# c-zhou/oatk

Hardware: AMD Instinct MI355X
Metric: HiFi Gbases/s through syncasm (syncmer+syncerr) at k=1001 s=31 (higher is better)
Workload: dtype u64

## Files before the change

include/oatk_hip_ec.h:

```cpp
#ifndef OATK_HIP_EC_H
#define OATK_HIP_EC_H

#include "oatk_hip.h"

#ifdef __cplusplus
extern "C" {
#endif

typedef struct {
    uint64_t n_vtx, n_arc;
    const uint64_t *idx_p;
    const uint64_t *idx_n;
    const uint64_t *arc_v;
    const uint64_t *arc_w;
    const uint64_t *arc_ls;
    const uint32_t *arc_cov;
    const uint8_t *arc_del;
} oatk_ec_graph_t;

int oatk_hip_ec(oatk_hip_ctx *ctx, const oatk_ec_graph_t *g, double max_edist, uint32_t err_mer_c, uint32_t max_err_c,
                uint32_t err_arc_c, double max_arc_f);

int oatk_hip_ec_stats(oatk_hip_ctx *ctx, uint64_t *stats12);

int oatk_hip_debug_ec_tiers(oatk_hip_ctx *ctx, int cap_t0, int cap_t1);

int oatk_hip_debug_wf_ed(oatk_hip_ctx *ctx, uint64_t n_jobs, const uint8_t *t_codes, const uint64_t *t_off, const uint8_t *q_codes, const uint64_t *q_off,
                         const int32_t *bw, const int32_t *step_ql, const uint64_t *step_off, int32_t *out3);
int oatk_hip_debug_wf_ed_wg(oatk_hip_ctx *ctx, int R, uint64_t n_jobs, const uint8_t *t_codes, const uint64_t *t_off, const uint8_t *q_codes, const uint64_t *q_off,
                            const int32_t *bw, const int32_t *step_ql, const uint64_t *step_off, int32_t *out3);
int oatk_hip_debug_tables(oatk_hip_ctx *ctx, uint64_t n_jobs, const uint8_t *t_codes, const uint64_t *t_off, const uint8_t *s_codes, const uint64_t *s_off, int32_t *out, const uint64_t *out_off);

enum {
    OATK_BUF_EC_N_SCM = 100, OATK_BUF_EC_SCM_OFF, OATK_BUF_EC_KMER, OATK_BUF_EC_MPOS, OATK_BUF_EC_SMER,
    OATK_BUF_EC_SCM_COV, OATK_BUF_EC_SCM_DEL, OATK_BUF_EC_SCM_OCC_OFF, OATK_BUF_EC_SCM_OCC, OATK_BUF_EC_ERR_DEL,
    OATK_BUF_EC_SCM_FWD,
    OATK_BUF_EC_VTX_SRC,
    OATK_BUF_EC_BLOCK_WORK, OATK_BUF_EC_BLOCK_OUT,
    OATK_BUF_EC_CSEQ_LEN,
    OATK_BUF_EC_CSEQ_OFF,
    OATK_BUF_EC_CSEQ,
    OATK_BUF_EC_BLOCK_QEND
};

int oatk_hip_ec_keep_seq(oatk_hip_ctx *ctx, int on);
int oatk_hip_ec_corrected_reads(oatk_hip_ctx *ctx, uint64_t *n_bases);

int oatk_hip_ec_mark(oatk_hip_ctx *ctx, uint32_t err_mer_c, uint32_t max_err_c, uint32_t err_arc_c, double max_arc_f);
int oatk_hip_ec_correct(oatk_hip_ctx *ctx, double max_edist);

int oatk_hip_ec_graph(oatk_hip_ctx *ctx);
int oatk_hip_ec_graph_light(oatk_hip_ctx *ctx, uint32_t err_mer_c);

int oatk_hip_ec_set_global(oatk_hip_ctx *ctx, uint64_t n_global, const uint32_t *d_l2g, const uint32_t *d_cov, const uint64_t *d_s);
int oatk_hip_ec_pairs(oatk_hip_ctx *ctx, const void **d_keys, const void **d_dist, uint64_t *n_pairs);
int oatk_hip_ec_graph_from_pairs(oatk_hip_ctx *ctx, const uint64_t *d_keys, const uint32_t *d_dist, uint64_t n_pairs);
int oatk_hip_ec_graph_from_segments(oatk_hip_ctx *ctx, const uint64_t *d_keys, const uint64_t *d_val, uint64_t n_seg);
int oatk_hip_ec_export_kmers(oatk_hip_ctx *ctx, const uint32_t *d_ids, uint64_t n, uint8_t *d_out, uint32_t stride, uint8_t *d_rev);
int oatk_hip_ec_import_kmers(oatk_hip_ctx *ctx, const uint32_t *d_ids, const uint8_t *d_rev, const uint8_t *d_kmers, uint64_t n, uint32_t stride);
int oatk_hip_ec_reserve_import(oatk_hip_ctx *ctx, uint64_t bytes);

enum {
    OATK_BUF_EG_IDX_P = 120, OATK_BUF_EG_IDX_N, OATK_BUF_EG_ARC_V, OATK_BUF_EG_ARC_W, OATK_BUF_EG_ARC_LS, OATK_BUF_EG_ARC_COV,
    OATK_BUF_EG_ARC_COMP,
    OATK_BUF_EG_OTHER
};

#ifdef __cplusplus
}
#endif
#endif
```

oatk_amd/_lib.py:

```python
import ctypes as C
import os

HERE = os.path.dirname(os.path.abspath(__file__))
LIB_PATH = os.environ.get("OATK_HIP_LIB") or os.path.join(HERE, "lib", "liboatk_hip.so")
HOST_LIB_PATH = os.path.join(HERE, "lib", "liboatk_host.so")

OK, E_NODEV, E_ARG, E_STATE, E_SMER, E_SPLIT, E_NOMEM = range(7)
READ_ALIGN = 64
BUF = {name: i for i, name in enumerate([
    "HOCO_L", "N_SCM", "N_NN", "N_LRL", "HO_RL", "HOCO_S", "NN_KEY", "LRL_KEY", "LRL_VAL",
    "SCM_OFF", "POS_MPOS", "POS_SMER", "POS_HASH", "POS_KID",
    "SCM_H", "SCM_S", "SCM_COV", "SCM_OCC_OFF", "SCM_OCC"])}
BUF.update({name: 100 + i for i, name in enumerate([
    "EC_N_SCM", "EC_SCM_OFF", "EC_KMER", "EC_MPOS", "EC_SMER", "EC_SCM_COV", "EC_SCM_DEL", "EC_SCM_OCC_OFF", "EC_SCM_OCC", "EC_ERR_DEL",
    "EC_SCM_FWD", "EC_VTX_SRC", "EC_BLOCK_WORK", "EC_BLOCK_OUT", "EC_CSEQ_LEN", "EC_CSEQ_OFF", "EC_CSEQ", "EC_BLOCK_QEND"])})
BUF.update({name: 160 + i for i, name in enumerate(["INGEST_SEQ", "INGEST_OFF", "INGEST_LEN", "INGEST_HDR"])})
FMT_AUTO, FMT_FASTA, FMT_FASTQ = 0, 1, 2
BUF.update({name: 140 + i for i, name in enumerate(["CONS_SEL", "CONS_SLOT", "CONS_RL", "CONS_MSEQ", "CONS_FIRST", "CONS_TOT"])})
BUF.update({name: 200 + i for i, name in enumerate(["RA_ALN_SID", "RA_ALN_OFF", "RA_ALN_S", "RA_FRG_UID", "RA_FRG_UBEG", "RA_FRG_UEND", "RA_FRG_SBEG", "RA_FRG_SEND", "RA_SKIPPED"])})
BUF.update({name: 150 + i for i, name in enumerate(["OVL_KEY", "OVL_OFF", "OVL_DIST", "OVL_CNT", "OVL_TAIL"])})
BUF.update({name: 120 + i for i, name in enumerate([
    "EG_IDX_P", "EG_IDX_N", "EG_ARC_V", "EG_ARC_W", "EG_ARC_LS", "EG_ARC_COV", "EG_ARC_COMP", "EG_OTHER"])})
BUF.update({name: 180 + i for i, name in enumerate([
    "AG_SCM_DEL", "AG_VTX_SCM", "AG_VTX_COV", "AG_IDX_P", "AG_IDX_N", "AG_ARC_V", "AG_ARC_W", "AG_ARC_COV", "AG_ARC_COMP", "AG_ARC_LINK"])})
BUF.update({name: 220 + i for i, name in enumerate(["MG_H", "MG_S", "MG_COV", "MG_L2G", "MG_EC_COV", "MG_EC_DEL", "MG_LCOV"])})
BUF.update({name: 230 + i for i, name in enumerate(["MG_G_H", "MG_G_S", "MG_G_COV", "MG_G_DEL", "MG_G_OCC_OFF", "MG_G_OCC", "MG_POS_GKID"])})
TIMERS = ["hpc", "syncmer", "syncmer_n", "scan_post", "count_place", "count_sort", "count_group", "kmer_hash", "ec_graph", "ec_mark", "ec_solve", "ec_refresh"]

EXPORTS = [
    "oatk_hip_abi_version", "oatk_hip_device_count", "oatk_hip_create", "oatk_hip_destroy", "oatk_hip_last_error",
    "oatk_hip_stream", "oatk_hip_sync", "oatk_hip_max_k", "oatk_hip_scan", "oatk_hip_scan_host", "oatk_hip_count",
    "oatk_comm_unique_id", "oatk_comm_create", "oatk_comm_group_create", "oatk_comm_group_rank", "oatk_comm_group_destroy", "oatk_comm_destroy",
    "oatk_comm_rank", "oatk_comm_size", "oatk_comm_backend", "oatk_comm_traffic", "oatk_hip_merge_counts", "oatk_hip_multi_range", "oatk_hip_ec_sharded",
    "oatk_hip_gather_table", "oatk_hip_asm_graph_sharded", "oatk_hip_consensus_sharded", "oatk_hip_overlap_hist_sharded", "oatk_hip_stat_sharded",
    "oatk_hip_scan_begin", "oatk_hip_scan_reserve", "oatk_hip_scan_append", "oatk_hip_device", "oatk_hip_d2d", "oatk_hip_mem_pool",
    "oatk_hip_info", "oatk_hip_buffer", "oatk_hip_d2h", "oatk_hip_d2h_async", "oatk_hip_h2d_async", "oatk_hip_staging", "oatk_hip_ingest_text_buffer", "oatk_hip_set_timing", "oatk_hip_get_timing",
    "oatk_hip_debug_hash_mask", "oatk_hip_debug_force_general", "oatk_hip_debug_list_cap",
    "oatk_hip_ec_graph", "oatk_hip_ec_graph_light", "oatk_hip_ec", "oatk_hip_ec_stats", "oatk_hip_debug_ec_tiers", "oatk_hip_debug_wf_ed", "oatk_hip_debug_wf_ed_wg", "oatk_hip_ec_mark", "oatk_hip_ec_correct",
    "oatk_hip_ec_set_global", "oatk_hip_ec_pairs", "oatk_hip_ec_graph_from_pairs", "oatk_hip_ec_graph_from_segments", "oatk_hip_ec_export_kmers", "oatk_hip_ec_import_kmers",
    "oatk_hip_ec_reserve_import", "oatk_hip_consensus", "oatk_hip_consensus_ids", "oatk_hip_ingest", "oatk_hip_ingest_host", "oatk_hip_scan_ingested", "oatk_hip_stat", "oatk_hip_stat_keys", "oatk_hip_stat_from_keys",
    "oatk_hip_asm_graph", "oatk_hip_asm_pairs", "oatk_hip_asm_graph_from_pairs", "oatk_hip_overlap_hist", "oatk_hip_overlap_pairs", "oatk_hip_overlap_hist_from_pairs", "oatk_hip_read_alignment", "oatk_hip_debug_align_two_pass",
    "oatk_hip_ra_utg_coverage", "oatk_hip_ra_arc_coverage", "oatk_hip_debug_racov_cap", "oatk_hip_ra_utg_coverage_sharded", "oatk_hip_ra_arc_coverage_sharded",
    "oatk_hip_ra_triplet_scores", "oatk_hip_ra_triplet_scores_sharded",
    "oatk_hip_ec_keep_seq", "oatk_hip_ec_corrected_reads",
    "oatk_hip_inflate_bgzf", "oatk_hip_inflate_bgzf_host", "oatk_hip_inflate_last_byte", "oatk_hip_ingest_names",
    "oatk_hip_ingest_bam", "oatk_hip_ingest_bam_host", "oatk_hip_ingest_bam_stats", "oatk_hip_ingest_bam_times",
]

HOST_EXPORTS = ["oatk_multi_scg_ra_utg_coverage", "oatk_multi_scg_ra_arc_coverage", "oatk_scg_multiplex_plan", "oatk_multi_scg_multiplex_plan",
                "oatk_triplet_table_free", "oatk_multi_read_error_correction_fo", "oatk_bgzf_index", "oatk_host_set_device_inflate", "oatk_host_inflate_counts"]


def load_host():
    H = C.CDLL(HOST_LIB_PATH)
    vp = C.c_void_p
    H.oatk_sr_db_new.restype = vp
    H.oatk_sr_db_new.argtypes = [C.c_int, C.c_int]
    H.oatk_multi_create.restype = vp
    H.oatk_multi_create.argtypes = [C.POINTER(C.c_int), C.c_int]
    H.oatk_multi_destroy.argtypes = [vp]
    H.oatk_multi_ctx.restype = vp
    H.oatk_multi_ctx.argtypes = [vp, C.c_int]
    H.oatk_multi_last_error.restype = C.c_char_p
    H.oatk_multi_last_error.argtypes = [vp]
    H.oatk_multi_range.argtypes = [vp, C.c_int, C.POINTER(C.c_uint64), C.POINTER(C.c_uint64)]
    H.oatk_multi_sr_read_files.argtypes = [vp, vp, C.POINTER(C.c_char_p), C.c_int]
    H.oatk_multi_collect_syncmer_from_reads.restype = vp
    H.oatk_multi_collect_syncmer_from_reads.argtypes = [vp, vp, C.POINTER(C.c_int)]
    H.oatk_multi_read_error_correction.argtypes = [vp, vp, vp, C.c_double, C.c_uint32, C.c_uint32, C.c_uint32, C.c_double, vp]
    H.oatk_multi_read_error_correction_fo.argtypes = [vp, vp, vp, C.c_double, C.c_uint32, C.c_uint32, C.c_uint32, C.c_double, vp, vp]
    H.oatk_multi_make_syncmer_asmg.restype = vp
    H.oatk_multi_make_syncmer_asmg.argtypes = [vp, vp, C.c_uint32, C.c_double, C.POINTER(C.c_int)]
    H.oatk_multi_scg_read_alignment.argtypes = [vp, vp, vp, vp, C.c_int, C.POINTER(C.c_uint64)]
    H.oatk_multi_scg_ra_utg_coverage.argtypes = [vp, vp, vp, vp, C.c_int]
    H.oatk_multi_scg_ra_arc_coverage.argtypes = [vp, vp, vp, vp, C.c_int]
    H.oatk_scg_multiplex_plan.argtypes = [vp, vp, vp, C.c_uint, C.c_uint32, C.c_double, C.c_double, vp, C.POINTER(C.c_int), C.POINTER(TripletTable)]
    H.oatk_multi_scg_multiplex_plan.argtypes = [vp, vp, vp, C.c_uint32, C.c_double, C.c_double, vp, C.POINTER(C.c_int), C.POINTER(TripletTable)]
    H.oatk_triplet_table_free.restype = None
    H.oatk_triplet_table_free.argtypes = [C.POINTER(TripletTable)]
    H.oatk_host_debug_window.argtypes = [C.c_uint64]
    H.oatk_bgzf_index.argtypes = [vp, C.c_uint64, C.c_uint64, C.c_uint64, vp, C.POINTER(C.c_uint64), C.POINTER(C.c_uint64), C.POINTER(C.c_uint64)]
    return H


BGZF_MEMBER = [("in_off", "<u8"), ("in_len", "<u4"), ("out_len", "<u4"), ("out_off", "<u8"), ("crc", "<u4"), ("pad", "<u4")]
INF_OK, INF_STREAM, INF_LENGTH, INF_CRC = range(4)


class TripletTable(C.Structure):
    _fields_ = [("n", C.c_uint64), ("m", C.c_uint64), ("l_in", C.POINTER(C.c_uint64)), ("l_out", C.POINTER(C.c_uint64)), ("val", C.POINTER(C.c_double))]

# ... 60 lines not shown
    L.oatk_hip_last_error.argtypes = [vp]
    L.oatk_hip_stream.restype = vp
    L.oatk_hip_stream.argtypes = [vp]
    L.oatk_hip_sync.argtypes = [vp]
    L.oatk_hip_max_k.restype = C.c_int
    L.oatk_hip_scan.argtypes = [vp, vp, vp, vp, C.c_uint64, C.c_uint64, C.c_uint64, C.c_int, C.c_int]
    L.oatk_hip_scan_host.argtypes = [vp, vp, vp, vp, C.c_uint64, C.c_uint64, C.c_uint64, C.c_int, C.c_int]
    L.oatk_hip_count.argtypes = [vp]
    L.oatk_comm_unique_id.argtypes = [vp]
    L.oatk_comm_create.restype = vp
    L.oatk_comm_create.argtypes = [vp, C.c_int, C.c_int, C.c_int]
    L.oatk_comm_group_create.restype = vp
    L.oatk_comm_group_create.argtypes = [C.c_int]
    L.oatk_comm_group_rank.restype = vp
    L.oatk_comm_group_rank.argtypes = [vp, C.c_int]
    L.oatk_comm_group_destroy.argtypes = [vp]
    L.oatk_comm_destroy.argtypes = [vp]
    L.oatk_comm_rank.argtypes = [vp]
    L.oatk_comm_size.argtypes = [vp]
    L.oatk_comm_backend.restype = C.c_char_p
    L.oatk_comm_backend.argtypes = [vp]
    L.oatk_comm_traffic.restype = None
    L.oatk_comm_traffic.argtypes = [vp, C.POINTER(C.c_uint64), C.c_int]
    L.oatk_hip_merge_counts.argtypes = [vp, vp, C.POINTER(C.c_uint64)]
    L.oatk_hip_multi_range.argtypes = [vp, C.POINTER(C.c_uint64), C.POINTER(C.c_uint64), C.POINTER(C.c_uint64)]
    L.oatk_hip_ec_sharded.argtypes = [vp, vp, C.c_double, C.c_uint32, C.c_uint32, C.c_uint32, C.c_double, vp, C.POINTER(C.c_uint64)]
    L.oatk_hip_gather_table.argtypes = [vp, vp, C.c_int]
    L.oatk_hip_asm_graph_sharded.argtypes = [vp, vp, C.c_uint32, C.c_double, C.POINTER(C.c_uint64), C.POINTER(C.c_uint64)]
    L.oatk_hip_consensus_sharded.argtypes = [vp, vp, C.c_uint32]
    L.oatk_hip_overlap_hist_sharded.argtypes = [vp, vp, C.c_uint32, C.POINTER(C.c_uint64), C.POINTER(C.c_uint64)]
    L.oatk_hip_stat_sharded.argtypes = [vp, vp, C.POINTER(StatRaw)]
    L.oatk_hip_scan_begin.argtypes = [vp, C.c_uint64, C.c_int, C.c_int]
    L.oatk_hip_scan_reserve.argtypes = [vp, C.c_uint64, C.c_uint64, C.c_uint64]
    L.oatk_hip_scan_append.argtypes = [vp, vp]
    L.oatk_hip_device.argtypes = [vp]
    L.oatk_hip_mem_pool.argtypes = [vp, C.c_uint64]
    L.oatk_hip_d2d.argtypes = [vp, vp, vp, C.c_uint64]
    L.oatk_hip_info.argtypes = [vp, C.POINTER(Info)]
    L.oatk_hip_buffer.argtypes = [vp, C.c_int, C.POINTER(vp), C.POINTER(C.c_uint64)]
    L.oatk_hip_d2h.argtypes = [vp, vp, vp, C.c_uint64]
    L.oatk_hip_staging.restype = vp
    L.oatk_hip_staging.argtypes = [vp, C.c_uint64]
    L.oatk_hip_set_timing.argtypes = [vp, C.c_int]
    L.oatk_hip_get_timing.argtypes = [vp, C.POINTER(C.c_float), C.c_int]
    L.oatk_hip_debug_hash_mask.argtypes = [vp, C.c_uint64]
    L.oatk_hip_debug_force_general.argtypes = [vp, C.c_int]
    L.oatk_hip_debug_list_cap.argtypes = [vp, C.c_int]
    L.oatk_hip_ec_graph.argtypes = [vp]
    L.oatk_hip_ec_graph_light.argtypes = [vp, C.c_uint32]
    L.oatk_hip_ec.argtypes = [vp, C.POINTER(EcGraph), C.c_double, C.c_uint32, C.c_uint32, C.c_uint32, C.c_double]
    L.oatk_hip_ec_stats.argtypes = [vp, vp]
    L.oatk_hip_debug_ec_tiers.argtypes = [vp, C.c_int, C.c_int]
    L.oatk_hip_debug_wf_ed.argtypes = [vp, C.c_uint64, vp, vp, vp, vp, vp, vp, vp, vp]
    if hasattr(L, "oatk_hip_debug_wf_ed_wg"):
        L.oatk_hip_debug_wf_ed_wg.argtypes = [vp, C.c_int, C.c_uint64, vp, vp, vp, vp, vp, vp, vp, vp]
    if hasattr(L, "oatk_hip_debug_ed_ab"):
        L.oatk_hip_debug_ed_ab.argtypes = [vp, C.c_int, C.c_uint64, vp, vp, vp, vp, vp, vp, C.POINTER(C.c_float)]
    L.oatk_hip_ec_mark.argtypes = [vp, C.c_uint32, C.c_uint32, C.c_uint32, C.c_double]
    L.oatk_hip_ec_correct.argtypes = [vp, C.c_double]
    L.oatk_hip_ec_keep_seq.argtypes = [vp, C.c_int]
    L.oatk_hip_ec_corrected_reads.argtypes = [vp, C.POINTER(C.c_uint64)]
    L.oatk_hip_ec_set_global.argtypes = [vp, C.c_uint64, vp, vp, vp]
    L.oatk_hip_ec_pairs.argtypes = [vp, C.POINTER(vp), C.POINTER(vp), C.POINTER(C.c_uint64)]
    L.oatk_hip_ec_graph_from_pairs.argtypes = [vp, vp, vp, C.c_uint64]
    L.oatk_hip_ec_graph_from_segments.argtypes = [vp, vp, vp, C.c_uint64]
    L.oatk_hip_ec_export_kmers.argtypes = [vp, vp, C.c_uint64, vp, C.c_uint32, vp]
    L.oatk_hip_ec_import_kmers.argtypes = [vp, vp, vp, vp, C.c_uint64, C.c_uint32]
    L.oatk_hip_ec_reserve_import.argtypes = [vp, C.c_uint64]
    L.oatk_hip_consensus.argtypes = [vp, C.c_uint32]
    L.oatk_hip_consensus_ids.argtypes = [vp, vp, C.c_uint64]
    L.oatk_hip_ingest.argtypes = [vp, vp, C.c_uint64, C.c_int, C.c_int, C.POINTER(C.c_uint64), C.POINTER(C.c_uint64)]
    L.oatk_hip_ingest_host.argtypes = [vp, vp, C.c_uint64, C.c_int, C.c_int, C.POINTER(C.c_uint64), C.POINTER(C.c_uint64)]
    L.oatk_hip_scan_ingested.argtypes = [vp, C.c_uint64, C.c_int, C.c_int]
    L.oatk_hip_ingest_text_buffer.argtypes = [vp, C.c_uint64, C.POINTER(vp)]
    L.oatk_hip_inflate_bgzf.argtypes = [vp, vp, C.c_uint64, vp, C.c_uint64, vp, C.c_uint64, C.POINTER(C.c_uint64), vp]
    L.oatk_hip_inflate_bgzf_host.argtypes = [vp, vp, C.c_uint64, vp, C.c_uint64, vp, C.c_uint64, C.POINTER(C.c_uint64), vp]
    L.oatk_hip_inflate_last_byte.argtypes = [vp]
    L.oatk_hip_ingest_names.argtypes = [vp, vp, C.c_uint64, C.POINTER(vp), C.POINTER(vp), C.POINTER(C.c_uint64)]
    L.oatk_hip_ingest_bam.argtypes = [vp, vp, C.c_uint64, C.c_int, C.c_int, C.POINTER(C.c_uint64), C.POINTER(C.c_uint64)]
    L.oatk_hip_ingest_bam_host.argtypes = [vp, vp, C.c_uint64, C.c_int, C.c_int, C.POINTER(C.c_uint64), C.POINTER(C.c_uint64)]
    L.oatk_hip_ingest_bam_stats.argtypes = [vp, C.POINTER(C.c_uint64)]
    L.oatk_hip_ingest_bam_times.argtypes = [vp, C.POINTER(C.c_float)]
    L.oatk_hip_stat.argtypes = [vp, C.POINTER(StatRaw)]
    L.oatk_hip_stat_keys.argtypes = [vp, C.POINTER(vp), C.POINTER(vp), C.POINTER(C.c_uint64), vp]
    L.oatk_hip_stat_from_keys.argtypes = [vp, vp, vp, C.c_uint64, vp, C.POINTER(StatRaw)]
    L.oatk_hip_debug_align_two_pass.argtypes = [vp, C.c_int]
    L.oatk_hip_read_alignment.argtypes = [vp, C.POINTER(RaGraph), vp, C.POINTER(C.c_uint64), C.POINTER(C.c_uint64), vp]
    L.oatk_hip_ra_utg_coverage.argtypes = [vp, C.POINTER(RacovGraph), C.POINTER(RacovReads), C.POINTER(RacovAln), C.c_int, vp, C.POINTER(C.c_uint64)]
    L.oatk_hip_ra_arc_coverage.argtypes = [vp, C.POINTER(RacovGraph), C.POINTER(RacovAln), vp]
    L.oatk_hip_debug_racov_cap.argtypes = [vp, C.c_uint64]
    L.oatk_hip_ra_utg_coverage_sharded.argtypes = [vp, vp, C.POINTER(RacovGraph), C.POINTER(RacovReads), C.POINTER(RacovAln), C.c_int, vp, C.POINTER(C.c_uint64)]
    L.oatk_hip_ra_arc_coverage_sharded.argtypes = [vp, vp, C.POINTER(RacovGraph), C.POINTER(RacovAln), vp]
    u64p = C.POINTER(C.c_uint64)
    L.oatk_hip_ra_triplet_scores.argtypes = [vp, C.POINTER(RacovGraph), C.POINTER(RacovAln), vp, C.c_uint64, u64p, vp, vp, vp, vp]
    L.oatk_hip_ra_triplet_scores_sharded.argtypes = [vp, vp, C.POINTER(RacovGraph), C.POINTER(RacovAln), vp, C.c_uint64, u64p, vp, vp, vp, vp]
    L.oatk_hip_overlap_pairs.argtypes = [vp, C.POINTER(vp), C.POINTER(vp), C.POINTER(C.c_uint64)]
    L.oatk_hip_overlap_hist_from_pairs.argtypes = [vp, vp, vp, C.c_uint64, C.POINTER(C.c_uint64), C.POINTER(C.c_uint64)]
    L.oatk_hip_overlap_hist.argtypes = [vp, C.POINTER(C.c_uint64), C.POINTER(C.c_uint64)]
    L.oatk_hip_asm_graph.argtypes = [vp, C.c_uint32, C.c_double, C.POINTER(C.c_uint64), C.POINTER(C.c_uint64)]
    L.oatk_hip_asm_pairs.argtypes = [vp, C.POINTER(vp), C.POINTER(C.c_uint64)]
    L.oatk_hip_asm_graph_from_pairs.argtypes = [vp, vp, C.c_uint64, C.c_uint64, vp, vp, C.c_uint32, C.c_double, C.POINTER(C.c_uint64), C.POINTER(C.c_uint64)]
    _lib = L
    return L
```

oatk_amd/csrc/api_ec.inc:

```
#include "../../include/oatk_hip_ec.h"
#include "ec.hpp"
#include "ec_wave.hpp"
#include "ec_heavy.hpp"
#include "ec_fused.hpp"
#include "ecgraph.hpp"
#include "ec_seq.hpp"
#include <rocprim/iterator/counting_iterator.hpp>

struct EcState {
    DevBuf idx_p, idx_n, arc_v, arc_w, arc_ls, arc_cov, arc_del, conv;
    DevBuf scm_del, err_del, vtx_hs_off, vtx_mpos;
    DevBuf copy_n, seg, keep_all, n_blocks, n_blocks64, blk_off, work, out, path_pool, cursor, todo, todo2, slabs, big_slabs, os_slabs;
    DevBuf qkey, qidx, qtmp[4];
    uint64_t n_live = 0, q_used = 0, qk_used = 0;
    DevBuf hyb_slabs[16];
    hipStream_t aux[5] = {nullptr, nullptr, nullptr, nullptr, nullptr};
    hipEvent_t aux_ev[5] = {nullptr, nullptr, nullptr, nullptr, nullptr}, fork_ev = nullptr;
    DevBuf new_n, new_n64, new_off, new_k, new_m, new_s, stats;
    DevBuf live32, live64, live_off, larc, lidx_p, lidx_n;
    DevBuf cov, fwd, key_id, key_sorted, val_occ, occ, occ_off, cov64;
    uint64_t n_vtx = 0, new_tot = 0;
    uint64_t stats_h[12] = {0};
    uint64_t n_work = 0;
    uint32_t staged_over = 0;
// ... 51 lines not shown
        if (which == OATK_BUF_EC_VTX_SRC) *d_ptr = e->vtx_hs_off.p, *bytes = e->n_vtx * 8;
        else *d_ptr = e->err_del.p, *bytes = e->n_vtx;
        return OATK_OK;
    }
    if (!e || !e->done) { ctx->err = "unknown buffer id, or error-correction results requested before oatk_hip_ec"; return OATK_E_STATE; }
    if (which == OATK_BUF_EC_BLOCK_WORK) { *d_ptr = e->work.p, *bytes = e->n_work * sizeof(oatk::EcWork); return OATK_OK; }
    if (which == OATK_BUF_EC_BLOCK_OUT) { *d_ptr = e->out.p, *bytes = e->n_work * sizeof(oatk::EcBlockOut); return OATK_OK; }
    if (which == OATK_BUF_EC_BLOCK_QEND) {
        if (!e->seq_kept) { ctx->err = "EC_BLOCK_QEND: the resident correction was made without oatk_hip_ec_keep_seq"; return OATK_E_STATE; }
        *d_ptr = e->qend.p, *bytes = e->n_work * 4;
        return OATK_OK;
    }
    if (which >= OATK_BUF_EC_CSEQ_LEN && which <= OATK_BUF_EC_CSEQ) {
        if (!e->seq_kept || !e->cseq_done) { ctx->err = "corrected sequences requested before oatk_hip_ec_corrected_reads"; return OATK_E_STATE; }
        if (which == OATK_BUF_EC_CSEQ_LEN) *d_ptr = e->clen.p, *bytes = ctx->n_reads * 4;
        else if (which == OATK_BUF_EC_CSEQ_OFF) *d_ptr = e->coff.p, *bytes = (ctx->n_reads + 1) * 8;
        else *d_ptr = e->cseq.p, *bytes = e->cseq_bytes;
        return OATK_OK;
    }
    const uint64_t n = ctx->n_reads, ns = e->n_vtx, tot = e->new_tot;
    switch (which) {
        case OATK_BUF_EC_N_SCM: *d_ptr = e->new_n.p, *bytes = n * 4; break;
        case OATK_BUF_EC_SCM_OFF: *d_ptr = e->new_off.p, *bytes = (n + 1) * 8; break;
        case OATK_BUF_EC_KMER: *d_ptr = e->new_k.p, *bytes = tot * 8; break;
        case OATK_BUF_EC_MPOS: *d_ptr = e->new_m.p, *bytes = tot * 4; break;
        case OATK_BUF_EC_SMER: *d_ptr = e->new_s.p, *bytes = tot * 8; break;
        case OATK_BUF_EC_SCM_COV: *d_ptr = e->cov.p, *bytes = ns * 4; break;
        case OATK_BUF_EC_SCM_DEL: *d_ptr = e->scm_del.p, *bytes = ns; break;
        case OATK_BUF_EC_SCM_OCC_OFF: *d_ptr = e->occ_off.p, *bytes = (ns + 1) * 8; break;
        case OATK_BUF_EC_SCM_OCC: *d_ptr = e->occ.p, *bytes = tot * 8; break;
        case OATK_BUF_EC_ERR_DEL: *d_ptr = e->err_del.p, *bytes = ns; break;
        case OATK_BUF_EC_SCM_FWD: *d_ptr = e->fwd.p, *bytes = ns * 4; break;
        default: ctx->err = "unknown buffer id"; return OATK_E_ARG;
    }
    return OATK_OK;
}

__global__ void ec_narrow_kernel(const uint64_t *in, uint32_t *out, uint64_t n)
{
    uint64_t i = (uint64_t) blockIdx.x * blockDim.x + threadIdx.x;
    if (i < n) out[i] = (uint32_t) in[i];
}
#define EENSURE(buf, bytes, ...) ENSURE_IN(e, "ec.", buf, bytes, ##__VA_ARGS__)

extern "C" int oatk_hip_debug_ec_tiers(oatk_hip_ctx *ctx, int cap_t0, int cap_t1)
{
    if (!ctx) return OATK_E_NODEV;
    if (cap_t0 < 0 || cap_t1 < 0 || (cap_t0 && cap_t1 && cap_t1 < cap_t0)) { ctx->err = "oatk_hip_debug_ec_tiers: 0 <= cap_t0 <= cap_t1"; return OATK_E_ARG; }
    ctx->ec_cap_t0 = cap_t0, ctx->ec_cap_t1 = cap_t1;
    return OATK_OK;
}

static int debug_ed_impl(oatk_hip_ctx *ctx, uint64_t n_jobs, const uint8_t *t_codes, const uint64_t *t_off, const uint8_t *q_codes, const uint64_t *q_off,
                         const int32_t *bw, const int32_t *step_ql, const uint64_t *step_off, int32_t *out3, bool myers, float *kernel_ms, int wg_R = 0)
{
    using namespace oatk;
    if (!ctx) return OATK_E_NODEV;
    if (n_jobs == 0) return OATK_OK;
    if (n_jobs >= 0x7FFFFFFFULL) { ctx->err = "oatk_hip_debug_wf_ed: too many jobs"; return OATK_E_ARG; }
    CK(hipSetDevice(ctx->device));
    std::vector<uint64_t> tw_off(n_jobs + 1, 0), qw_off(n_jobs + 1, 0), k_off(n_jobs + 1, 0);
    std::vector<int32_t> tl(n_jobs);
    for (uint64_t j = 0; j < n_jobs; ++j) {
        const uint64_t t = t_off[j + 1] - t_off[j], q = q_off[j + 1] - q_off[j];
        if (t == 0 || q == 0 || t > 0x3FFFFFFF || q > 0x3FFFFFFF) { ctx->err = "oatk_hip_debug_wf_ed: empty or oversized string (wf_ed asserts tl > 0 && ql > 0)"; return OATK_E_ARG; }
        for (uint64_t s = step_off[j]; s < step_off[j + 1]; ++s)
            if (step_ql[s] < 1 || (uint64_t) step_ql[s] > q || (s > step_off[j] && step_ql[s] < step_ql[s - 1])) { ctx->err = "oatk_hip_debug_wf_ed: query lengths must ascend within the query"; return OATK_E_ARG; }
        tl[j] = (int32_t) t;
        if (wg_R && (bw[j] >= 0? (uint64_t) 2 * (uint64_t) bw[j] + 3 : t + q + 3) > (wg_R == ECF_NW? (uint64_t) ECF_NW * ECF_OWN : (uint64_t) 64 * ECH_NW * (uint64_t) wg_R)) { ctx->err = "oatk_hip_debug_wf_ed_wg: a job's diagonals do not fit the registers of this variant"; return OATK_E_ARG; }
        tw_off[j + 1] = tw_off[j] + ecw_words((int32_t) t), qw_off[j + 1] = qw_off[j] + ecw_words((int32_t) q);
        k_off[j + 1] = k_off[j] + 2 * (t + q + 8);
    }
    auto pack = [](const uint8_t *codes, const uint64_t *off, const std::vector<uint64_t> &woff, uint64_t n) {
        std::vector<uint32_t> w(woff[n], 0u);
        for (uint64_t j = 0; j < n; ++j)
            for (uint64_t p = 0, len = off[j + 1] - off[j]; p < len; ++p)
                w[woff[j] + (p >> 4)] |= (uint32_t) (codes[off[j] + p] & 3u) << ((p & 15u) << 1);
        return w;
    };
    const std::vector<uint32_t> tw = pack(t_codes, t_off, tw_off, n_jobs), qw = pack(q_codes, q_off, qw_off, n_jobs);
    const uint64_t n_steps = step_off[n_jobs];
    DevBuf d_tw, d_qw, d_two, d_qwo, d_tl, d_bw, d_sq, d_so, d_k, d_ko, d_out, d_slab;
    hipEvent_t ev0 = nullptr, ev1 = nullptr;
    if (kernel_ms) { *kernel_ms = 0.f; (void) hipEventCreate(&ev0); (void) hipEventCreate(&ev1); }
    int32_t max_t = 0;
    for (uint64_t j = 0; j < n_jobs; ++j) if (tl[j] > max_t) max_t = tl[j];
    const uint64_t n_waves = (n_jobs + 63) / 64, slab_words = (uint64_t) 6 * 64 * (uint64_t) ((max_t + 63) / 64 + 1);
    std::vector<int32_t> ql_last(n_jobs);
    for (uint64_t j = 0; j < n_jobs; ++j) ql_last[j] = step_off[j + 1] > step_off[j]? step_ql[step_off[j + 1] - 1] : (int32_t) (q_off[j + 1] - q_off[j]);
    int rc = OATK_OK;
    hipError_t he = hipSuccess;
    auto up = [&](DevBuf &b, const void *src, size_t bytes) {
        if (rc) return;
        if (!b.ensure(bytes + 16, ctx->stream)) { rc = OATK_E_NOMEM; return; }
        if (bytes && (he = hipMemcpyAsync(b.p, src, bytes, hipMemcpyHostToDevice, ctx->stream)) != hipSuccess) rc = OATK_E_NODEV;
    };
    up(d_tw, tw.data(), tw.size() * 4); up(d_qw, qw.data(), qw.size() * 4);
    up(d_two, tw_off.data(), (n_jobs + 1) * 8); up(d_qwo, qw_off.data(), (n_jobs + 1) * 8); up(d_ko, k_off.data(), (n_jobs + 1) * 8);
    up(d_tl, tl.data(), n_jobs * 4); up(d_bw, bw, n_jobs * 4); up(d_sq, step_ql, n_steps * 4); up(d_so, step_off, (n_jobs + 1) * 8);
    if (!rc && (!d_k.ensure(k_off[n_jobs] * 4 + 16, ctx->stream) || !d_out.ensure(n_steps * 12 + 16, ctx->stream))) rc = OATK_E_NOMEM;
    if (!rc && myers) {
        if (!d_slab.ensure(n_waves * slab_words * 8 + 64, ctx->stream) || !d_out.ensure(n_jobs * 12 + 16, ctx->stream)) rc = OATK_E_NOMEM;
        up(d_sq, ql_last.data(), n_jobs * 4);
    }
    if (!rc) {
        if (ev0) (void) hipEventRecord(ev0, ctx->stream);
#ifdef OATK_EXPERIMENTS
        if (myers)
            hipLaunchKernelGGL(myers_ed_kernel, dim3((unsigned) n_waves), dim3(64), 0, ctx->stream, n_jobs, d_tw.as<uint32_t>(), d_two.as<uint64_t>(), d_tl.as<int32_t>(),
                               d_qw.as<uint32_t>(), d_qwo.as<uint64_t>(), d_sq.as<int32_t>(), d_bw.as<int32_t>(), d_slab.as<uint64_t>(), slab_words, d_out.as<int32_t>());
        else
#endif
        if (wg_R) {
            uint64_t cap_words = 0;
            for (uint64_t j = 0; j < n_jobs; ++j) { if (tw_off[j + 1] - tw_off[j] > cap_words) cap_words = tw_off[j + 1] - tw_off[j]; if (qw_off[j + 1] - qw_off[j] > cap_words) cap_words = qw_off[j + 1] - qw_off[j]; }
            const uint64_t lds = ((uint64_t) ech_misc_words(wg_R) + 2 * cap_words) * 4;
            if (lds > 64 * 1024 || (wg_R != 1 && wg_R != 2 && wg_R != 6 && wg_R != ECF_NW)) { ctx->err = "oatk_hip_debug_wf_ed_wg: strings too long for LDS, or no such variant (1, 2, 6, 16)"; rc = OATK_E_ARG; }
            else if (wg_R == ECF_NW) hipLaunchKernelGGL((ecf_wf_ed_kernel<ECF_NW>), dim3((unsigned) n_jobs), dim3(64 * ECF_NW), (unsigned) (((uint64_t) ecf_misc_words(ECF_NW) + 2 * cap_words) * 4), ctx->stream, d_tw.as<uint32_t>(), d_two.as<uint64_t>(), d_tl.as<int32_t>(),
                                                         d_qw.as<uint32_t>(), d_qwo.as<uint64_t>(), d_bw.as<int32_t>(), d_sq.as<int32_t>(), d_so.as<uint64_t>(), d_out.as<int32_t>(), (int32_t) cap_words);
            else if (wg_R == 1) hipLaunchKernelGGL((ech_wf_ed_kernel<ECH_NW, 1>), dim3((unsigned) n_jobs), dim3(64 * ECH_NW), (unsigned) lds, ctx->stream, d_tw.as<uint32_t>(), d_two.as<uint64_t>(), d_tl.as<int32_t>(),
                                                    d_qw.as<uint32_t>(), d_qwo.as<uint64_t>(), d_bw.as<int32_t>(), d_sq.as<int32_t>(), d_so.as<uint64_t>(), d_out.as<int32_t>(), (int32_t) cap_words);
            else if (wg_R == 2) hipLaunchKernelGGL((ech_wf_ed_kernel<ECH_NW, 2>), dim3((unsigned) n_jobs), dim3(64 * ECH_NW), (unsigned) lds, ctx->stream, d_tw.as<uint32_t>(), d_two.as<uint64_t>(), d_tl.as<int32_t>(),
                                                    d_qw.as<uint32_t>(), d_qwo.as<uint64_t>(), d_bw.as<int32_t>(), d_sq.as<int32_t>(), d_so.as<uint64_t>(), d_out.as<int32_t>(), (int32_t) cap_words);
            else hipLaunchKernelGGL((ech_wf_ed_kernel<ECH_NW, 6>), dim3((unsigned) n_jobs), dim3(64 * ECH_NW), (unsigned) lds, ctx->stream, d_tw.as<uint32_t>(), d_two.as<uint64_t>(), d_tl.as<int32_t>(),
                                    d_qw.as<uint32_t>(), d_qwo.as<uint64_t>(), d_bw.as<int32_t>(), d_sq.as<int32_t>(), d_so.as<uint64_t>(), d_out.as<int32_t>(), (int32_t) cap_words);
        } else
        hipLaunchKernelGGL(ecw_wf_ed_kernel, dim3((unsigned) n_jobs), dim3(64), 0, ctx->stream, d_tw.as<uint32_t>(), d_two.as<uint64_t>(), d_tl.as<int32_t>(),
                           d_qw.as<uint32_t>(), d_qwo.as<uint64_t>(), d_bw.as<int32_t>(), d_sq.as<int32_t>(), d_so.as<uint64_t>(), d_k.as<int32_t>(),
                           d_ko.as<uint64_t>(), d_out.as<int32_t>());
        if (ev1) (void) hipEventRecord(ev1, ctx->stream);
        const uint64_t n_out = myers? n_jobs : n_steps;
        if (n_out && (he = hipMemcpyAsync(out3, d_out.p, n_out * 12, hipMemcpyDeviceToHost, ctx->stream)) != hipSuccess) rc = OATK_E_NODEV;
        if ((he = hipStreamSynchronize(ctx->stream)) != hipSuccess) rc = OATK_E_NODEV;
        if (!rc && (he = hipGetLastError()) != hipSuccess) rc = OATK_E_NODEV;
    }
    (void) hipStreamSynchronize(ctx->stream);
    if (ev0 && ev1 && !rc) (void) hipEventElapsedTime(kernel_ms, ev0, ev1);
    if (ev0) (void) hipEventDestroy(ev0);
    if (ev1) (void) hipEventDestroy(ev1);
    if (rc == OATK_E_NODEV) ctx->err = std::string("oatk_hip_debug_wf_ed: ") + hipGetErrorString(he);
    if (rc == OATK_E_NOMEM) ctx->err = "oatk_hip_debug_wf_ed: hipMalloc failed";
    return rc;
}

extern "C" int oatk_hip_debug_wf_ed(oatk_hip_ctx *ctx, uint64_t n_jobs, const uint8_t *t_codes, const uint64_t *t_off, const uint8_t *q_codes, const uint64_t *q_off,
                                    const int32_t *bw, const int32_t *step_ql, const uint64_t *step_off, int32_t *out3)
{
    float ms = 0.f;
    const bool timed = getenv("OATK_DEBUG_ED_TIME") != nullptr;
    const int rc = debug_ed_impl(ctx, n_jobs, t_codes, t_off, q_codes, q_off, bw, step_ql, step_off, out3, false, timed? &ms : nullptr);
    if (timed) fprintf(stderr, "[wf_ed_wg] R 0: %llu jobs, kernel %.3f ms\n", (unsigned long long) n_jobs, ms);
    return rc;
}

extern "C" int oatk_hip_debug_tables(oatk_hip_ctx *ctx, uint64_t n_jobs, const uint8_t *t_codes, const uint64_t *t_off, const uint8_t *s_codes, const uint64_t *s_off, int32_t *out, const uint64_t *out_off)
{
    using namespace oatk;
    if (!ctx) return OATK_E_NODEV;
    if (n_jobs == 0) return OATK_OK;
    if (n_jobs >= 0x7FFFFFFFULL) { ctx->err = "oatk_hip_debug_tables: too many jobs"; return OATK_E_ARG; }
    CK(hipSetDevice(ctx->device));
    std::vector<uint64_t> tw_off(n_jobs + 1, 0), qw_off(n_jobs + 1, 0);
    std::vector<int32_t> tl(n_jobs), ql(n_jobs);
    uint64_t cap_words = 0;
    for (uint64_t j = 0; j < n_jobs; ++j) {
        const uint64_t t = t_off[j + 1] - t_off[j], q = s_off[j + 1] - s_off[j];
        if (t == 0 || q == 0 || t > 0x3FFFFFFF || q > 1024) { ctx->err = "oatk_hip_debug_tables: an empty string, or one of more than 1024 bases"; return OATK_E_ARG; }
        if (out_off[j + 1] - out_off[j] < 2 * (t + 1)) { ctx->err = "oatk_hip_debug_tables: a job's output holds 2 (tl + 1) numbers"; return OATK_E_ARG; }
        tl[j] = (int32_t) t, ql[j] = (int32_t) q;
        tw_off[j + 1] = tw_off[j] + ecw_words((int32_t) t), qw_off[j + 1] = qw_off[j] + ecw_words((int32_t) q);
        if (tw_off[j + 1] - tw_off[j] > cap_words) cap_words = tw_off[j + 1] - tw_off[j];
        if (qw_off[j + 1] - qw_off[j] > cap_words) cap_words = qw_off[j + 1] - qw_off[j];
    }
    if (2 * cap_words * 4 > 64 * 1024) { ctx->err = "oatk_hip_debug_tables: strings too long for LDS"; return OATK_E_ARG; }
    auto pack = [](const uint8_t *codes, const uint64_t *off, const std::vector<uint64_t> &woff, uint64_t n) {
        std::vector<uint32_t> w(woff[n], 0u);
        for (uint64_t j = 0; j < n; ++j)
            for (uint64_t p = 0, len = off[j + 1] - off[j]; p < len; ++p)
                w[woff[j] + (p >> 4)] |= (uint32_t) (codes[off[j] + p] & 3u) << ((p & 15u) << 1);
        return w;
    };
    const std::vector<uint32_t> tw = pack(t_codes, t_off, tw_off, n_jobs), qw = pack(s_codes, s_off, qw_off, n_jobs);
    DevBuf d_tw, d_qw, d_two, d_qwo, d_tl, d_ql, d_oo, d_out;
    int rc = OATK_OK;
    hipError_t he = hipSuccess;
    auto up = [&](DevBuf &b, const void *src, size_t bytes) {
        if (rc) return;
        if (!b.ensure(bytes + 16, ctx->stream)) { rc = OATK_E_NOMEM; return; }
        if (bytes && (he = hipMemcpyAsync(b.p, src, bytes, hipMemcpyHostToDevice, ctx->stream)) != hipSuccess) rc = OATK_E_NODEV;
    };
    up(d_tw, tw.data(), tw.size() * 4); up(d_qw, qw.data(), qw.size() * 4);
    up(d_two, tw_off.data(), (n_jobs + 1) * 8); up(d_qwo, qw_off.data(), (n_jobs + 1) * 8);
    up(d_tl, tl.data(), n_jobs * 4); up(d_ql, ql.data(), n_jobs * 4); up(d_oo, out_off, (n_jobs + 1) * 8);
    const uint64_t n_out = out_off[n_jobs];
    if (!rc && !d_out.ensure(n_out * 4 + 16, ctx->stream)) rc = OATK_E_NOMEM;
    if (!rc) {
        int seg_nw = 1, seg_cut = 0;
        { const char *ev = getenv("OATK_DEBUG_TABLES_SEG"); if (ev && sscanf(ev, "%d:%d", &seg_nw, &seg_cut) != 2) seg_nw = 1, seg_cut = 0; }
        if (n_out && (he = hipMemsetAsync(d_out.p, 0xFF, n_out * 4, ctx->stream)) != hipSuccess) rc = OATK_E_NODEV;
#define OATK_TABLES_LAUNCH(NW) hipLaunchKernelGGL((ecb_tables_kernel<NW>), dim3((unsigned) n_jobs), dim3(64 * NW), (unsigned) (2 * cap_words * 4), ctx->stream, d_tw.as<uint32_t>(), d_two.as<uint64_t>(), d_tl.as<int32_t>(), \
                           d_qw.as<uint32_t>(), d_qwo.as<uint64_t>(), d_ql.as<int32_t>(), d_out.as<int32_t>(), d_oo.as<uint64_t>(), (int32_t) cap_words, (int32_t) seg_cut)
        if (seg_nw == 2) OATK_TABLES_LAUNCH(2); else if (seg_nw == 4) OATK_TABLES_LAUNCH(4); else if (seg_nw == 8) OATK_TABLES_LAUNCH(8); else if (seg_nw == 16) OATK_TABLES_LAUNCH(16); else OATK_TABLES_LAUNCH(1);
#undef OATK_TABLES_LAUNCH
        if (n_out && (he = hipMemcpyAsync(out, d_out.p, n_out * 4, hipMemcpyDeviceToHost, ctx->stream)) != hipSuccess) rc = OATK_E_NODEV;
        if ((he = hipStreamSynchronize(ctx->stream)) != hipSuccess) rc = OATK_E_NODEV;
// ... 313 lines not shown
    CK(hipSetDevice(ctx->device));
    EcState *e = ctx->ec;
    if (n) hipLaunchKernelGGL(ecw_export_kmer_kernel, dim3((unsigned) n), dim3(64), 0, ctx->stream, n, d_ids, e->vtx_hs_off.as<uint64_t>(), e->vtx_mpos.as<uint32_t>(),
                              ctx->hoco_s.as<uint8_t>(), ctx->K, stride, d_out, d_rev);
    CK(hipStreamSynchronize(ctx->stream));
    CK(hipGetLastError());
    return OATK_OK;
}

extern "C" int oatk_hip_ec_import_kmers(oatk_hip_ctx *ctx, const uint32_t *d_ids, const uint8_t *d_rev, const uint8_t *d_kmers, uint64_t n, uint32_t stride)
{
    using namespace oatk;
    if (!ctx) return OATK_E_NODEV;
    if (!ctx->ec || !ctx->ec->marked) { ctx->err = "oatk_hip_ec_import_kmers needs oatk_hip_ec_mark"; return OATK_E_STATE; }
    if (stride % 16 || stride < (uint32_t) ((ctx->K + 3) / 4 + 8)) { ctx->err = "k-mer stride must be a multiple of 16 and hold the k-mer + 8 bytes"; return OATK_E_ARG; }
    CK(hipSetDevice(ctx->device));
    EcState *e = ctx->ec;
    if (n && !ctx->hoco_s.p) { ctx->err = "oatk_hip_ec_import_kmers: this batch has no hoco strings to put k-mers behind"; return OATK_E_STATE; }
    const uint64_t base = ((ctx->seq_bytes / 4 + 128) + 15) & ~15ULL;
    if (e->imp_used + n * stride > ctx->import_reserve) { ctx->err = "imported k-mers exceed the reserve behind the hoco strings (oatk_hip_ec_reserve_import before the scan)"; return OATK_E_NOMEM; }
    if (n) {
        CK(hipMemcpyAsync(ctx->hoco_s.as<uint8_t>() + base + e->imp_used, d_kmers, n * stride, hipMemcpyDeviceToDevice, ctx->stream));
        hipLaunchKernelGGL(ecw_import_kmer_kernel, dim3((unsigned) ((n + 255) / 256)), dim3(256), 0, ctx->stream, n, d_ids, d_rev, base + e->imp_used, stride,
                           e->vtx_hs_off.as<uint64_t>(), e->vtx_mpos.as<uint32_t>());
        e->imp_used += n * stride;
    }
    CK(hipStreamSynchronize(ctx->stream));
    CK(hipGetLastError());
    return OATK_OK;
}

extern "C" int oatk_hip_ec_reserve_import(oatk_hip_ctx *ctx, uint64_t bytes)
{
    if (!ctx) return OATK_E_NODEV;
    ctx->import_reserve = bytes < (1u << 20)? (1u << 20) : (bytes + 15) & ~15ULL;
    return OATK_OK;
}

struct EcKnobs {
    int heavy = -1;
    bool stages = false;
    bool serial_tiers = false;
    int32_t step_budget = 1000;
    int32_t min_nw = 0;
    int32_t heavy_cap2 = 0;
    int32_t heavy_fl = 0;
    int32_t waves = 32;
    bool assemble_walk = false;
    int memo = 2;
    bool queue_sort = true;
    bool list_walk = false;
    bool light_packed = true;
    bool light_pairs = true;
    bool light_wide = false;
};
static EcKnobs ec_knobs_read()
{
    EcKnobs k;
    auto num = [](const char *n, int32_t lo, int32_t dflt) { const char *e = getenv(n); return e && atoi(e) >= lo? (int32_t) atoi(e) : dflt; };
    { const char *e = getenv("OATK_DEBUG_EC_HEAVY"); k.heavy = e && (e[0] == '0' || e[0] == '1') && !e[1]? e[0] - '0' : -1; }
    k.stages = getenv("OATK_DEBUG_EC_STAGES") != nullptr;
    { const char *e = getenv("OATK_DEBUG_EC_SERIAL_TIERS"); k.serial_tiers = e && e[0] == '1'; }
    k.step_budget = num("OATK_DEBUG_EC_STEP_BUDGET", 1, 1000);
    k.min_nw = num("OATK_DEBUG_EC_FUSED_MIN_NW", 2, 0);
    k.heavy_cap2 = num("OATK_DEBUG_EC_HEAVY_CAP2", 1, 0), k.heavy_fl = num("OATK_DEBUG_EC_HEAVY_FL", 64, 0) & ~7;
    k.waves = num("OATK_DEBUG_EC_WAVES", 1, 32);
    { const char *e = getenv("OATK_DEBUG_EC_ASSEMBLE_WALK"); k.assemble_walk = e && e[0] == '1'; }
    { const char *e = getenv("OATK_DEBUG_EC_LIST_WALK"); k.list_walk = e && e[0] == '1'; }
    { const char *e = getenv("OATK_DEBUG_EC_MEMO"); k.memo = e && (e[0] == '0' || e[0] == '1') && !e[1]? e[0] - '0' : 2; }
    { const char *e = getenv("OATK_DEBUG_EC_QUEUE_SORT"); k.queue_sort = !(e && e[0] == '0' && !e[1]); }
    { const char *e = getenv("OATK_DEBUG_EC_LIGHT_PACKED"); k.light_packed = !(e && e[0] == '0' && !e[1]); }
    { const char *e = getenv("OATK_DEBUG_EC_LIGHT_PAIRS"); k.light_pairs = !(e && e[0] == '0' && !e[1]); }
    { const char *e = getenv("OATK_DEBUG_EC_LIGHT_KEYBITS"); k.light_wide = e && !strcmp(e, "64"); }
    return k;
}

static int ec_light_packed(oatk_hip_ctx *ctx, uint32_t c, bool pairs_old, bool force_wide)
{
    using namespace oatk;
    EcState *e = ctx->ec;
    const uint64_t nv = ec_n_vtx(ctx), nr = ctx->n_reads, n = ctx->n_occ, nw = (nv + 63) / 64, nwg = (nr + 255) / 256;
    if (n >= 0xFFFFFFFFULL) { ctx->err = "more than 2^32 adjacent pairs"; return OATK_E_ARG; }
    if (nv >= 0x7FFFFFFFULL) { ctx->err = "too many syncmers for 32-bit oriented vertex ids"; return OATK_E_ARG; }
    EENSURE(g_other, 2 * nv + 8); EENSURE(g_cbits, (nw + 1) * 8); EENSURE(g_wcnt, (nw + 1) * 4); EENSURE(g_wpre, (nw + 1) * 4);
    EENSURE(g_gcnt, (nwg + 1) * 4); EENSURE(g_gpre, (nwg + 1) * 4); EENSURE(g_nruns, 64);
    t_begin(ctx, OATK_T_EC_GRAPH);
    CK(hipMemsetAsync(e->g_other.p, 0, 2 * nv + 8, ctx->stream));
    uint32_t n_cand = 0, nk32 = 0;
    uint64_t nk = 0;
    EgrPacked pk = {nullptr, 1, force_wide, nullptr};
    int rc;
    if (n && nv) {
        const uint64_t *bits = e->g_cbits.as<uint64_t>();
        const uint32_t *wpre = e->g_wpre.as<uint32_t>();
        const uint64_t *scm_off = ctx->scm_off.as<uint64_t>(), *chains = ec_chains(ctx);
        const uint32_t *mpos = ctx->pos_mpos.as<uint32_t>();
        hipLaunchKernelGGL(egr_cand_flag_kernel, grid256(nv), dim3(256), 0, ctx->stream, nv, nw, ctx->scm_cov.as<uint32_t>(), c, e->g_cbits.as<uint64_t>(), e->g_wcnt.as<uint32_t>());
        PRIM(rocprim::exclusive_scan, e->g_wcnt.as<const uint32_t>(), e->g_wpre.as<uint32_t>(), 0u, nw + 1, rocprim::plus<uint32_t>(), ctx->stream);
        CK(hipMemcpyAsync(&n_cand, e->g_wpre.as<uint32_t>() + nw, 4, hipMemcpyDeviceToHost, ctx->stream));
        if (pairs_old) {
            EENSURE(g_keys, (n + 1) * 8); EENSURE(g_dist, (n + 1) * 4); EENSURE(g_keep, n + 8); EENSURE(g_keys2, (n + 1) * 8);
            hipLaunchKernelGGL(egr_pair_light_wave_kernel, dim3((unsigned) ((nr + 3) / 4)), dim3(256), 0, ctx->stream, nr, scm_off, chains, mpos, ctx->scm_cov.as<uint32_t>(), c,
                               e->g_keys.as<uint64_t>(), e->g_dist.as<uint32_t>(), e->g_keep.as<uint8_t>(), e->g_other.as<uint8_t>());
            auto flags = rocprim::make_transform_iterator(e->g_keep.as<uint8_t>(), [] __device__(uint8_t f) -> uint32_t { return f; });
            PRIM(rocprim::exclusive_scan, flags, e->g_keys2.as<uint32_t>(), 0u, n, rocprim::plus<uint32_t>(), ctx->stream);
        } else {
            hipLaunchKernelGGL((egr_pair_entry_kernel<uint32_t, false>), dim3((unsigned) nwg), dim3(256), 0, ctx->stream, nr, scm_off, chains, mpos, bits, wpre, 0u,
                               e->g_gcnt.as<uint32_t>(), (const uint32_t *) nullptr, (uint32_t *) nullptr, (uint32_t *) nullptr, (uint8_t *) nullptr);
            PRIM(rocprim::exclusive_scan, e->g_gcnt.as<const uint32_t>(), e->g_gpre.as<uint32_t>(), 0u, nwg + 1, rocprim::plus<uint32_t>(), ctx->stream);
            CK(hipMemcpyAsync(&nk32, e->g_gpre.as<uint32_t>() + nwg, 4, hipMemcpyDeviceToHost, ctx->stream));
        }
        CK(hipStreamSynchronize(ctx->stream));
        while ((1ULL << pk.B) < 2 * (uint64_t) n_cand) ++pk.B;
        if (2 * pk.B > 64) { ctx->err = "light EC graph: a pair of candidate ranks does not fit a 64-bit key"; return OATK_E_ARG; }
        pk.wide = force_wide || 2 * pk.B > 32;
        const uint64_t cap = pairs_old? n : (uint64_t) nk32;
        EENSURE(g_lkeys, (cap + 1) * (pk.wide? 8 : 4)); EENSURE(g_ldist, (cap + 1) * 4); EENSURE(g_candid, ((uint64_t) n_cand + 1) * 4);
        pk.keys = e->g_lkeys.p, pk.cand_id = e->g_candid.as<uint32_t>();
        if (n_cand) hipLaunchKernelGGL(egr_cand_id_kernel, grid256(nv), dim3(256), 0, ctx->stream, nv, bits, wpre, e->g_candid.as<uint32_t>());
        if (pairs_old) {
            uint64_t *d_cnt = e->g_nruns.as<uint64_t>() + 2;
            if (pk.wide) hipLaunchKernelGGL(egr_compact_pack_kernel<uint64_t>, grid256(n), dim3(256), 0, ctx->stream, n, e->g_keep.as<uint8_t>(), e->g_keys2.as<uint32_t>(), e->g_keys.as<uint64_t>(),
                                            e->g_dist.as<uint32_t>(), bits, wpre, pk.B, e->g_lkeys.as<uint64_t>(), e->g_ldist.as<uint32_t>(), d_cnt);
            else hipLaunchKernelGGL(egr_compact_pack_kernel<uint32_t>, grid256(n), dim3(256), 0, ctx->stream, n, e->g_keep.as<uint8_t>(), e->g_keys2.as<uint32_t>(), e->g_keys.as<uint64_t>(),
                                    e->g_dist.as<uint32_t>(), bits, wpre, pk.B, e->g_lkeys.as<uint32_t>(), e->g_ldist.as<uint32_t>(), d_cnt);
// ... 127 lines not shown
{
    if (!e->aux[0]) {
        int pr_least = 0, pr_greatest = 0;
        CK(hipDeviceGetStreamPriorityRange(&pr_least, &pr_greatest));
        for (int i = 0; i < 5; ++i) { CK(hipStreamCreateWithPriority(&e->aux[i], hipStreamNonBlocking, i < 4? pr_greatest : pr_least)); CK(hipEventCreateWithFlags(&e->aux_ev[i], hipEventDisableTiming)); }
        CK(hipEventCreateWithFlags(&e->fork_ev, hipEventDisableTiming));
    }
    CK(hipEventRecord(e->fork_ev, ctx->stream));
    return OATK_OK;
}

static int ec_route(oatk_hip_ctx *ctx, EcState *e, uint64_t n_work, const EcRoute &rt, unsigned long long *routed, size_t bytes)
{
    hipLaunchKernelGGL(ec_route_kernel, dim3((unsigned) ((n_work + 256 * ECW_ROUTE_ITEMS - 1) / (256 * ECW_ROUTE_ITEMS))), dim3(256), 0, ctx->stream, e->work.as<EcWork>(), n_work, rt);
    CK(hipMemcpyAsync(routed, rt.cnt[0], bytes, hipMemcpyDeviceToHost, ctx->stream));
    CK(hipStreamSynchronize(ctx->stream));
    return OATK_OK;
}

static int ec_sort_longest_first(oatk_hip_ctx *ctx, EcState *e, uint32_t *list, uint64_t n)
{
    uint32_t *k_in = e->todo2.as<uint32_t>(), *k_out = k_in + (n + 1), *v_out = k_out + (n + 1);
    hipLaunchKernelGGL(ec_route_keys_kernel, dim3((unsigned) ((n + 255) / 256)), dim3(256), 0, ctx->stream, e->work.as<EcWork>(), list, n, k_in);
    PRIM(rocprim::radix_sort_pairs, k_in, k_out, list, v_out, n, 0, 32, ctx->stream);
    CK(hipMemcpyAsync(list, v_out, n * 4, hipMemcpyDeviceToDevice, ctx->stream));
    return OATK_OK;
}

static int ec_queue_room(oatk_hip_ctx *ctx, EcState *e, uint64_t n_work)
{
    e->q_used = e->qk_used = 0;
    EENSURE(qkey, (4 * (n_work + 1) + 64) * 4); EENSURE(qidx, 2 * (n_work + 1) * 4);
    return OATK_OK;
}
static int ec_queue_sort(oatk_hip_ctx *ctx, EcState *e, const uint32_t *list, uint64_t n, hipStream_t st, DevBuf &tmp, const uint32_t **sorted)
{
    auto bits = [](uint64_t v) { int b = 1; while (b < 64 && (v >> b)) ++b; return b; };
    const uint64_t end_max = 2 * e->g_n_vtx;
    const uint32_t lp_max = (uint32_t) e->n_live;
    const int lb = bits(lp_max), total = lb + 8 >= 32? 32 : (lb + 8 + 7) & ~7;
    const int eb = bits(end_max) < total - lb? bits(end_max) : total - lb;
    if (e->q_used + n > e->qidx.cap / 4 || e->qk_used + 2 * (n + 1) > e->qkey.cap / 4) { ctx->err = "EC solver: more sorted queues than room for them (internal)"; return OATK_E_STATE; }
    uint32_t *v_out = e->qidx.as<uint32_t>() + e->q_used, *k_in = e->qkey.as<uint32_t>() + e->qk_used, *k_out = k_in + (n + 1);
    e->q_used += n, e->qk_used += 2 * (n + 1);
    hipLaunchKernelGGL(ec_queue_keys_kernel, dim3((unsigned) ((n + 255) / 256)), dim3(256), 0, st, e->work.as<EcWork>(), list, n, lp_max, end_max, eb, k_in);
    if (list) PRIM_IN(tmp, st, "hipMalloc failed (EC queue sort)", rocprim::radix_sort_pairs, k_in, k_out, list, v_out, n, 0, (unsigned) (eb + lb), st);
    else {
        rocprim::counting_iterator<uint32_t> iota(0);
        PRIM_IN(tmp, st, "hipMalloc failed (EC queue sort)", rocprim::radix_sort_pairs, k_in, k_out, iota, v_out, n, 0, (unsigned) (eb + lb), st);
    }
    *sorted = v_out;
    return OATK_OK;
}
static int32_t ec_routed_batch(uint64_t n_todo, uint64_t waves)
{
    const uint64_t b = waves? n_todo / (16 * waves) : 1;
    return (int32_t) (b < 1? 1 : (b > ECW_BATCH? ECW_BATCH : b));
}
struct EcMemoLog { int tier; unsigned long long n; int32_t batch; int slot; };
static int ec_memo_report(oatk_hip_ctx *ctx, EcState *e, const std::vector<EcMemoLog> &log)
{
    if (log.empty()) return OATK_OK;
    unsigned long long c[128];
    CK(hipMemcpyAsync(c, (unsigned long long *) e->cursor.p + 64, sizeof(c), hipMemcpyDeviceToHost, ctx->stream));
    CK(hipStreamSynchronize(ctx->stream));
    for (const EcMemoLog &l : log)
        fprintf(stderr, "[ec stages] wave solver, tier %d, %llu blocks: batch %d, %llu levels reused, %llu blocks started at their sink\n", l.tier, l.n, (int) l.batch, c[2 * l.slot], c[2 * l.slot + 1]);
    return OATK_OK;
}

static int ec_launch_slab_tier(oatk_hip_ctx *ctx, EcState *e, const EcwArgs &base, uint32_t &max_hl, const uint32_t *todo, uint64_t n_todo,
                               unsigned long long *queue, hipStream_t st)
{
    if (max_hl == 0) {
        std::vector<uint32_t> hl(ctx->n_reads);
        CK(hipMemcpy(hl.data(), ctx->hoco_l.p, ctx->n_reads * 4, hipMemcpyDeviceToHost));
        for (uint64_t i = 0; i < ctx->n_reads; ++i) if (hl[i] > max_hl) max_hl = hl[i];
    }
    EcwArgs a = base;
    a.cap_t = (int32_t) max_hl + 64, a.cap_c = ec_cap_c(a.cap_t, ctx->K);
    a.cap_w = 2 * ((int32_t) (max_hl * base.max_edist) + 16) + 16, a.cap_path = ec_cap_c((int32_t) max_hl, ctx->K), a.cap_f = 1 << 22;
    a.todo = todo, a.n_todo = n_todo, a.next = queue, a.skip_l = 0x7FFFFFFF, a.batch = 1;
    a.todo_out = e->todo2.as<uint32_t>(), a.todo_cnt = base.pool_cursor + 63;
    a.slab_bytes = ((uint64_t) ecw_scratch_words(a.cap_t, a.cap_c, a.cap_w, a.cap_path, a.cap_f) * 4 + 63) & ~63ULL;
    uint64_t waves = todo? n_todo : base.n_work;
    if (waves > 1024) waves = 1024;
    if (!waves) return OATK_OK;
    EENSURE(big_slabs, waves * a.slab_bytes);
    a.slabs = e->big_slabs.as<uint8_t>();
    ec_wave_launch<1, 1>(waves, 0, st, a);
    return OATK_OK;
}

static int ec_second_stage(oatk_hip_ctx *ctx, EcState *e, const EcKnobs &kn, const EcwArgs &base, uint32_t *todo, uint64_t nh, uint32_t *todo_out,
                           int &qslot, int &hyb_k, unsigned long long &left)
{
    unsigned long long *cur = base.pool_cursor;
    struct timespec ts0, ts1;
    if (kn.stages) clock_gettime(CLOCK_MONOTONIC, &ts0);
    if (nh > 1 && nh <= (4u << 20)) {
        if (3 * (nh + 1) > base.n_work + 1) EENSURE(todo2, 3 * (nh + 1) * 4);
        int rc = ec_sort_longest_first(ctx, e, todo, nh); if (rc) return rc;
    }
    const int NCLS = 5;
    const int NWS[NCLS] = {16, 8, 4, 2, 1};
    EcwArgs fa[NCLS];
    uint64_t lds[NCLS];
    for (int i = 0; i < NCLS; ++i) {
        const int NW = NWS[i];
        EcwArgs &a = fa[i];
        a = base;
        a.cap_t = ec_band_cap(((NW == 1? 64 : NW * ECF_OWN) - 3) / 2, base.max_edist);
        a.cap_c = ec_cap_c(a.cap_t, ctx->K), a.cap_w = 0, a.cap_path = a.cap_c;
        a.cap_f = kn.heavy_fl? kn.heavy_fl : (NW == 16? 32768 : (NW == 8? 24576 : (NW == 4? 16384 : (NW == 2? 12288 : 8192))));
        a.os_words = 1 << 20;
        lds[i] = (uint64_t) (NW == 1? ech_lds_words(a.cap_t, a.cap_c, a.cap_f, 1) : ecf_lds_words(a.cap_t, a.cap_c, a.cap_f, NW)) * 4;
    }
    int narrowest = NCLS - 1;
    if (kn.min_nw >= 2) narrowest = kn.min_nw >= 16? 0 : (kn.min_nw >= 8? 1 : (kn.min_nw >= 4? 2 : 3));
    while (narrowest > 0 && lds[narrowest] > 64 * 1024) --narrowest;
// ... 94 lines not shown
    const uint64_t t0_waves = T0.usable? ec_tier_waves(T0, kn.waves, ctx->n_cu) : 0;
    EENSURE(os_slabs, (t0_waves + ECW_WPB) * ec_os_words(T0.cap_c) * 4 + 64);
    EENSURE(todo, 4 * (n_work + 1) * 4); EENSURE(todo2, (n_work + 1) * 4);
    uint32_t *list[5] = {nullptr, e->todo.as<uint32_t>(), e->todo.as<uint32_t>() + (n_work + 1), e->todo.as<uint32_t>() + 2 * (n_work + 1), e->todo.as<uint32_t>() + 3 * (n_work + 1)};
    int qslot = 5, hyb_k = 0;
    auto launch_class = [&](int c, const uint32_t *todo, uint64_t n_todo, hipStream_t st) -> int {
        if (!n_todo) return OATK_OK;
        if (qslot >= 60) { ctx->err = "EC solver: more launches than work-queue counters (internal)"; return OATK_E_STATE; }
        const EcClass &h = H[c];
        EcwArgs a = base;
        a.cap_t = h.cap_t, a.cap_c = h.cap_c, a.cap_w = kn.step_budget, a.cap_path = h.cap_c, a.cap_f = h.cap_fl, a.os_words = (uint64_t) h.cap_fh;
        a.todo = todo, a.n_todo = n_todo, a.next = cur + qslot++, a.skip_l = 0x7FFFFFFF, a.batch = 1;
        a.todo_out = list[4], a.todo_cnt = cur + 4;
        uint64_t wgs = (uint64_t) ctx->n_cu * (c < 3? ec_wg_per_cu(h.lds) : 8);
        if (wgs > n_todo) wgs = n_todo;
        while (wgs > (uint64_t) ctx->n_cu && wgs * h.slab > (3ULL << 30)) wgs -= (uint64_t) ctx->n_cu;
        void *p = nullptr;
        { int rc = ec_slab_buf(ctx, e, hyb_k, wgs * h.slab + 64, st, "the workgroup solver", "slabs", &p); if (rc) return rc; }
        a.slabs = (uint8_t *) p, a.slab_bytes = h.slab;
        if (c == 1) ec_heavy_launch<1, 4>(wgs, h.lds, st, a);
        else if (c == 2) ec_heavy_launch<1, 8>(wgs, h.lds, st, a);
        else ec_heavy_launch<ECH_NW, 6>(wgs, h.lds, st, a);
        return OATK_OK;
    };
    EcRoute rt;
    for (int c = 0; c < 4; ++c) rt.list[c] = list[c], rt.cnt[c] = cur + c;
    for (int c = 1; c < 4; ++c) if (!H[c].usable) rt.list[c] = list[4], rt.cnt[c] = cur + 4;
    rt.cap[0] = T0.usable? T0.cap_t : -1, rt.cap[1] = H[1].routes? H[1].cap_t : 0, rt.cap[2] = H[2].routes? H[2].cap_t : 0, rt.cap[3] = 0x7FFFFFFF;
    unsigned long long routed[5] = {0, 0, 0, 0, 0}, cnts[5] = {0, 0, 0, 0, 0};
    if (n_work) { int rc = ec_route(ctx, e, n_work, rt, routed, sizeof(routed)); if (rc) return rc; }
    { int rc = ec_fork_side_streams(ctx, e); if (rc) return rc; }
    {
        unsigned long long mx = routed[1] > routed[2]? routed[1] : routed[2];
        mx = routed[3] > mx? routed[3] : mx;
        if (mx <= (4u << 20) && 3 * (mx + 1) > n_work + 1) EENSURE(todo2, 3 * (mx + 1) * 4);
    }
    int used_aux = 0;
    for (int c = 3; c >= 1; --c) {
        if (!routed[c]) continue;
        if (routed[c] > 1 && routed[c] <= (64u << 10)) {
            int rc = ec_sort_longest_first(ctx, e, list[c], routed[c]); if (rc) return rc;
            CK(hipEventRecord(e->fork_ev, ctx->stream));
        }
        hipStream_t st = e->aux[used_aux];
        CK(hipStreamWaitEvent(st, e->fork_ev, 0));
        { int rc = launch_class(c, list[c], routed[c], st); if (rc) return rc; }
        CK(hipEventRecord(e->aux_ev[used_aux], st));
        ++used_aux;
    }
    std::vector<EcMemoLog> mlog;
    if (T0.usable && n_work) {
        EcwArgs a = base;
        ec_set_caps(a, T0);
        a.todo = nullptr, a.n_todo = 0, a.next = cur + qslot++, a.skip_l = T0.cap_t, a.batch = ECW_BATCH;
        if (kn.queue_sort && n_work > 1) {
            { int rc = ec_queue_room(ctx, e, n_work); if (rc) return rc; }
            { int rc = ec_queue_sort(ctx, e, nullptr, n_work, ctx->stream, ctx->tmp, &a.todo); if (rc) return rc; }
            a.n_todo = n_work;
        }
        if (kn.stages) a.memo_stat = cur + 64 + 2 * mlog.size(), mlog.push_back(EcMemoLog{0, (unsigned long long) n_work, a.batch, (int) mlog.size()});
        a.arc_budget = EC_ARC_BUDGET;
        a.todo_out = list[1], a.todo_cnt = cur + 1;
        a.os_words = ec_os_words(T0.cap_c), a.os_slabs = e->os_slabs.as<uint32_t>();
        uint64_t waves = t0_waves;
        const uint64_t groups = (n_work + (uint64_t) a.batch - 1) / (uint64_t) a.batch;
        if (waves > groups) waves = groups;
        ec_launch_lds_tier(T0, waves, ctx->stream, a);
    }
    CK(hipMemcpyAsync(cnts, cur, sizeof(cnts), hipMemcpyDeviceToHost, ctx->stream));
    CK(hipStreamSynchronize(ctx->stream));
    if (kn.stages) { int rc = ec_memo_report(ctx, e, mlog); if (rc) return rc; }
    if (cnts[1] > routed[1]) { int rc = launch_class(1, list[1] + routed[1], cnts[1] - routed[1], ctx->stream); if (rc) return rc; }
    n_big = cnts[1] + routed[2] + routed[3] + routed[4];
    for (int i = 0; i < used_aux; ++i) CK(hipStreamWaitEvent(ctx->stream, e->aux_ev[i], 0));
    CK(hipMemcpyAsync(cnts, cur, sizeof(cnts), hipMemcpyDeviceToHost, ctx->stream));
    CK(hipStreamSynchronize(ctx->stream));
    if (kn.stages) fprintf(stderr, "[ec stages] first stage done: %llu blocks go on (classes got %llu + %llu + %llu; %llu past a class that does not fit LDS)\n", cnts[4], cnts[1], routed[2], routed[3], routed[4]);
    if (!cnts[4]) return OATK_OK;
    unsigned long long left = 0;
    { int rc = ec_second_stage(ctx, e, kn, base, list[4], cnts[4], list[1], qslot, hyb_k, left); if (rc) return rc; }
    if (!left) return OATK_OK;
    return ec_launch_slab_tier(ctx, e, base, max_hl, list[1], left, cur + qslot++, ctx->stream);
}

static int ec_solve_tiers(oatk_hip_ctx *ctx, EcState *e, const EcKnobs &kn, const EcwArgs &base, uint32_t &max_hl, uint64_t &n_big)
{
    const int LAST = 3;
    const uint64_t n_work = base.n_work;
    unsigned long long *cur = base.pool_cursor;
    const int32_t t_lo = ctx->ec_cap_t0 > 0? ctx->ec_cap_t0 : EC_CAP_T0, t_hi = ctx->ec_cap_t1 > 0? ctx->ec_cap_t1 : EC_CAP_T1;
    EcTier T[LAST + 1];
    T[0] = ec_lds_tier(t_lo, 32, 2048, false, base.max_edist, ctx->K);
    T[1] = ec_lds_tier(2 * t_lo < t_hi? 2 * t_lo : t_hi, 64, 4096, false, base.max_edist, ctx->K);
    T[2] = ec_lds_tier(t_hi, 0, 0, true, base.max_edist, ctx->K);
    T[LAST] = EcTier{}, T[LAST].usable = true;
    uint64_t os_total = 0, os_next = 0;
    for (int t = 0; t < LAST; ++t) if (T[t].usable) os_total += 3 * (ec_tier_waves(T[t], kn.waves, ctx->n_cu) + ECW_WPB) * ec_os_words(T[t].cap_c);
    EENSURE(os_slabs, os_total * 4 + 64);
    EENSURE(todo, 3 * (n_work + 1) * 4); EENSURE(todo2, (n_work + 1) * 4);
    uint32_t *list[4] = {nullptr, e->todo.as<uint32_t>(), e->todo.as<uint32_t>() + (n_work + 1), e->todo.as<uint32_t>() + 2 * (n_work + 1)};
    int qslot = 4, hyb_k = 0;
    std::vector<EcMemoLog> mlog;
    if (kn.queue_sort) { int rc = ec_queue_room(ctx, e, n_work); if (rc) return rc; }
    auto next_usable = [&](int t) { int u = t + 1; while (u < LAST && !T[u].usable) ++u; return u; };
    auto launch = [&](int tier, const uint32_t *todo, uint64_t n_todo, hipStream_t st, bool routed, uint64_t max_waves = 0) -> int {
        if (qslot >= 60) { ctx->err = "EC solver: more rounds of left-overs than queue counters (internal)"; return OATK_E_STATE; }
        unsigned long long *queue = cur + qslot++;
        if (kn.stages) fprintf(stderr, "[ec stages] tier %d: %llu blocks%s\n", tier, (unsigned long long) (todo? n_todo : n_work), todo? (routed? " routed by length" : " left over") : "");
        if (tier == LAST) return ec_launch_slab_tier(ctx, e, base, max_hl, todo, n_todo, queue, st);
        const EcTier &t = T[tier];
        EcwArgs a = base;
        ec_set_caps(a, t);
        a.todo = todo, a.n_todo = n_todo, a.next = queue;
        a.skip_l = routed && tier == 0? t.cap_t : 0x7FFFFFFF;
        a.batch = ECW_BATCH;
        const int nx = tier < LAST - 1 && T[LAST - 1].usable? LAST - 1 : next_usable(tier);
        a.todo_out = list[nx], a.todo_cnt = cur + nx;
        uint64_t waves = ec_tier_waves(t, kn.waves, ctx->n_cu);
        a.os_words = ec_os_words(t.cap_c);
        if ((os_next + waves * a.os_words) * 4 > e->os_slabs.cap) { ctx->err = "EC solver: more launches than optimum-consensus slabs (internal)"; return OATK_E_STATE; }
        a.os_slabs = e->os_slabs.as<uint32_t>() + os_next;
        os_next += waves * a.os_words;
        const uint64_t n_items = todo? n_todo : n_work;
        if (tier > 0) {
            uint64_t w1 = waves < n_items? waves : n_items;
            if (max_waves && w1 > max_waves) w1 = max_waves;
            a.batch = ec_routed_batch(n_items, w1);
        }
        if (kn.queue_sort && (todo? routed : true) && n_items > 1 && a.batch > 1) {
            DevBuf *tmp = &ctx->tmp;
            for (int i = 0; i < 4; ++i) if (st == e->aux[i]) tmp = &e->qtmp[i];
            { int rc = ec_queue_sort(ctx, e, todo, n_items, st, *tmp, &a.todo); if (rc) return rc; }
            a.n_todo = n_items;
        }
        const uint64_t groups = (n_items + (uint64_t) a.batch - 1) / (uint64_t) a.batch;
        if (waves > groups) waves = groups;
        if (max_waves && waves > max_waves) waves = max_waves;
        if (!waves) return OATK_OK;
        if (kn.stages && mlog.size() < 64) a.memo_stat = cur + 64 + 2 * mlog.size(), mlog.push_back(EcMemoLog{tier, (unsigned long long) n_items, a.batch, (int) mlog.size()});
        if (t.hybrid) {
            void *p = nullptr;
            int rc = ec_slab_buf(ctx, e, hyb_k, (waves + ECW_WPB) * t.slab + 64, st, "the hybrid tier", "slabs", &p); if (rc) return rc;
            a.slabs = (uint8_t *) p, a.slab_bytes = t.slab;
        }
        ec_launch_lds_tier(t, waves, st, a);
        return OATK_OK;
    };
    EcRoute rt;
    for (int t = 0; t <= LAST; ++t) rt.cap[t] = T[t].usable? T[t].cap_t : 0, rt.list[t] = list[t], rt.cnt[t] = cur + t;
    rt.cap[LAST] = 0x7FFFFFFF;
    const bool side_by_side = T[0].usable && !kn.serial_tiers && n_work;
    unsigned long long routed[4] = {0, 0, 0, 0}, done[4] = {0, 0, 0, 0}, cnts[4] = {0, 0, 0, 0};
    int used_aux = 0;
    if (side_by_side) {
        { int rc = ec_route(ctx, e, n_work, rt, routed, sizeof(routed)); if (rc) return rc; }
        { int rc = ec_fork_side_streams(ctx, e); if (rc) return rc; }
        for (int tier = LAST - 1; tier >= 1; --tier) {
            if (!T[tier].usable || !routed[tier]) continue;
            hipStream_t st = e->aux[used_aux];
            CK(hipStreamWaitEvent(st, e->fork_ev, 0));
            { int rc = launch(tier, list[tier], routed[tier], st, true, tier == 1? 2 * (uint64_t) ctx->n_cu : 0); if (rc) return rc; }
            CK(hipEventRecord(e->aux_ev[used_aux], st));
            ++used_aux;
            done[tier] = routed[tier];
        }
    }
    const int first_tier = side_by_side || T[0].usable? 0 : next_usable(0);
    { int rc = launch(first_tier, nullptr, 0, ctx->stream, side_by_side); if (rc) return rc; }
    bool waited_aux = used_aux == 0;
    for (int round = 0; ; ++round) {
        CK(hipMemcpyAsync(cnts, cur, sizeof(cnts), hipMemcpyDeviceToHost, ctx->stream));
        CK(hipStreamSynchronize(ctx->stream));
        if (round == 0) n_big = cnts[1] + cnts[2] + routed[3];
        bool any = false;
        for (int tier = first_tier + 1; tier <= LAST; ++tier) {
            if (!T[tier].usable || cnts[tier] <= done[tier]) continue;
            { int rc = launch(tier, list[tier] + done[tier], cnts[tier] - done[tier], ctx->stream, false); if (rc) return rc; }
            done[tier] = cnts[tier];
            any = true;
        }
        if (!any && waited_aux) break;
        if (!waited_aux) { for (int i = 0; i < used_aux; ++i) CK(hipStreamWaitEvent(ctx->stream, e->aux_ev[i], 0)); waited_aux = true; }
    }
    if (kn.stages) { int rc = ec_memo_report(ctx, e, mlog); if (rc) return rc; }
    return OATK_OK;
}

}

extern "C" int oatk_hip_ec_correct(oatk_hip_ctx *ctx, double max_edist)
{
    using namespace oatk;
// ... 16 lines not shown
        if (na) hipLaunchKernelGGL(ec_live_flag_kernel, grid256(na), dim3(256), 0, ctx->stream, na, (const uint8_t *) e->arc_del.p, e->live32.as<uint32_t>());
        { int rc = prim_scan_total_u32(ctx, e->live32, e->live64, e->live_off, na, &n_live); if (rc) return rc; }
        if (n_live >= 0xFFFFFFFFULL) { ctx->err = "error correction: more than 2^32 live arcs"; return OATK_E_ARG; }
        EENSURE(larc, (n_live + 1) * sizeof(EcLiveArc));
        e->n_live = n_live;
        hipLaunchKernelGGL(ec_live_idx_kernel, grid256(2 * nv), dim3(256), 0, ctx->stream, 2 * nv, e->idx_p.as<uint64_t>(), e->idx_n.as<uint32_t>(),
                           e->live_off.as<uint64_t>(), e->lidx_p.as<uint32_t>(), e->lidx_n.as<uint32_t>(), e->g_flags.as<uint32_t>() + 9);
        if (na) hipLaunchKernelGGL(ec_live_arc_kernel, grid256(na), dim3(256), 0, ctx->stream, na, (const uint8_t *) e->arc_del.p, e->live_off.as<uint64_t>(),
                                   e->arc_w.as<uint64_t>(), e->arc_ls.as<uint32_t>(), e->vtx_hs_off.as<uint64_t>(), e->vtx_mpos.as<uint32_t>(),
                                   e->lidx_p.as<uint32_t>(), e->lidx_n.as<uint32_t>(), e->larc.as<EcLiveArc>(), e->g_flags.as<uint32_t>() + 8);
        uint32_t fl[2] = {0, 0};
        CK(hipMemcpyAsync(fl, e->g_flags.as<uint32_t>() + 8, 8, hipMemcpyDeviceToHost, ctx->stream));
        CK(hipStreamSynchronize(ctx->stream));
        const uint32_t no_src = fl[0];
        graph_branches = fl[1] != 0;
        if (no_src && ctx->n_occ) { ctx->err = "error correction: a live vertex has no k-mer on this shard (import it: oatk_hip_ec_import_kmers)"; return OATK_E_STATE; }
        lv.idx_p = e->lidx_p.as<uint32_t>(), lv.idx_n = e->lidx_n.as<uint32_t>(), lv.arc = e->larc.as<EcLiveArc>();
    }

    EENSURE(n_blocks, (nr + 1) * 4);
    const dim3 rblocks((unsigned) ((nr + ECR_READS_PER_BLOCK - 1) / ECR_READS_PER_BLOCK > 0? (nr + ECR_READS_PER_BLOCK - 1) / ECR_READS_PER_BLOCK : 1));
    EENSURE(new_n, (nr + 1) * 4); EENSURE(copy_n, (nr + 1) * 4); EENSURE(keep_all, nr + 1);
    const uint64_t stage_cap = nocc + nr + 1;
    e->staged_over = 0;
    if (kn.list_walk) hipLaunchKernelGGL(ec_count_blocks_wave_kernel, rblocks, dim3(256), 0, ctx->stream, rd, (const uint8_t *) e->scm_del.p, e->n_blocks.as<uint32_t>());
    else {
        static_assert(sizeof(EcSeg) == 8, "a staging entry is one val_occ entry");
        EENSURE(val_occ, stage_cap * sizeof(EcSeg));
        hipLaunchKernelGGL(ec_stage_blocks_wave_kernel, rblocks, dim3(256), 0, ctx->stream, rd, (const uint8_t *) e->scm_del.p, e->n_blocks.as<uint32_t>(), e->copy_n.as<uint32_t>(),
                           e->keep_all.as<uint8_t>(), e->val_occ.as<EcSeg>(), stage_cap, e->g_flags.as<uint32_t>() + 10);
        CK(hipMemcpyAsync(&e->staged_over, e->g_flags.as<uint32_t>() + 10, 4, hipMemcpyDeviceToHost, ctx->stream));
    }
    uint64_t n_work = 0;
    { int rc = prim_scan_total_u32(ctx, e->n_blocks, e->n_blocks64, e->blk_off, nr, &n_work); if (rc) return rc; }
    if (e->staged_over) { ctx->err = "error correction: a read has more error blocks than syncmers + 1 (the block walk's staging array)"; return OATK_E_STATE; }
    EENSURE(work, (n_work + 1) * sizeof(EcWork)); EENSURE(out, (n_work + 1) * sizeof(EcBlockOut));
    e->n_work = n_work;
    EENSURE(seg, (n_work + 1) * sizeof(EcSeg));
    if (kn.list_walk) hipLaunchKernelGGL(ec_list_blocks_wave_kernel, rblocks, dim3(256), 0, ctx->stream, rd, lv, (const uint8_t *) e->scm_del.p, e->blk_off.as<uint64_t>(), e->work.as<EcWork>(),
                                         e->copy_n.as<uint32_t>(), e->seg.as<EcSeg>(), e->keep_all.as<uint8_t>());
    else hipLaunchKernelGGL(ec_fill_work_kernel, grid256(nr), dim3(256), 0, ctx->stream, rd, lv, e->blk_off.as<uint64_t>(), (const EcSeg *) e->val_occ.as<EcSeg>(), e->work.as<EcWork>(), e->seg.as<EcSeg>());
    if (keep_seq) {
        uint64_t slot_words = 0;
        EENSURE(slot_w, (n_work + 1) * 4); EENSURE(qend, (n_work + 1) * 4);
        if (n_work) hipLaunchKernelGGL(ec_slot_words_kernel, grid256(n_work), dim3(256), 0, ctx->stream, e->work.as<EcWork>(), n_work, max_edist, e->slot_w.as<uint32_t>());
        { int rc = prim_scan_total_u32(ctx, e->slot_w, e->slot_w64, e->slot_off, n_work, &slot_words); if (rc) return rc; }
        EENSURE(slots, (slot_words + 4) * 4);
    }
    t_end(ctx, OATK_T_EC_MARK);
    t_begin(ctx, OATK_T_EC_SOLVE);

    const bool heavy = kn.heavy < 0? graph_branches : kn.heavy != 0;
    uint64_t pool_cap = 2 * nocc + (uint64_t) 16384 * ECW_POOL_CHUNK + 4096;
    EENSURE(cursor, 512 + 128 * 8); EENSURE(stats, 16 * 8);
    uint64_t n_big = 0;
    uint32_t max_hl = 0;
    for (;;) {
        EENSURE(path_pool, pool_cap * 8);
        CK(hipMemsetAsync(e->cursor.p, 0, 512 + 128 * 8, ctx->stream));
        EcwArgs base = {};
        base.lv = lv, base.rd = rd, base.work = e->work.as<EcWork>(), base.n_work = n_work, base.max_edist = max_edist;
        base.out = e->out.as<EcBlockOut>(), base.path_pool = e->path_pool.as<uint64_t>(), base.pool_cap = pool_cap;
        base.memo = kn.memo;
        base.pool_cursor = (unsigned long long *) e->cursor.p;
        if (keep_seq) {
            CK(hipMemsetAsync(e->qend.p, 0, (n_work + 1) * 4, ctx->stream));
            base.seq_qend = e->qend.as<uint32_t>(), base.seq_slots = e->slots.as<uint32_t>(), base.seq_slot_off = e->slot_off.as<uint64_t>();
        }
        if (kn.stages) fprintf(stderr, "[ec stages] the live graph %s: %s\n", graph_branches? "branches" : "does not branch", heavy? "classes with budgets, second stage" : "round 4's tiers");
        { int rc = heavy? ec_solve_classes(ctx, e, kn, base, max_hl, n_big) : ec_solve_tiers(ctx, e, kn, base, max_hl, n_big); if (rc) return rc; }
        unsigned long long fin = 0, used = 0;
        CK(hipMemcpyAsync(&fin, base.pool_cursor + 63, 8, hipMemcpyDeviceToHost, ctx->stream));
        CK(hipStreamSynchronize(ctx->stream));
        if (fin) { ctx->err = "error correction: a block outgrew the large scratch slab (DFS deeper than 4 MiB of frames)"; return OATK_E_NOMEM; }
        CK(hipMemcpyAsync(&used, e->cursor.p, 8, hipMemcpyDeviceToHost, ctx->stream));
        CK(hipStreamSynchronize(ctx->stream));
        if (used <= pool_cap) break;
        pool_cap = used + used / 4 + 4096;
    }

    t_end(ctx, OATK_T_EC_SOLVE);
    t_begin(ctx, OATK_T_EC_REFRESH);
    EENSURE(new_n, (nr + 1) * 4);
    CK(hipMemsetAsync(e->stats.p, 0, 16 * 8, ctx->stream));
    EcAssembleArgs aa;
    aa.rd = rd, aa.scm_del = (const uint8_t *) e->scm_del.p, aa.scm_s = g.scm_s, aa.blk_off = e->blk_off.as<uint64_t>();
    aa.out = e->out.as<EcBlockOut>(), aa.path_pool = e->path_pool.as<uint64_t>(), aa.new_n = e->new_n.as<uint32_t>(), aa.new_off = nullptr;
    aa.new_k_mer = nullptr, aa.new_s_mer = nullptr, aa.new_m_pos = nullptr, aa.old_s_mer = ctx->pos_smer.as<uint64_t>();
    aa.stats = (unsigned long long *) e->stats.p, aa.pass = 1, aa.seg = e->seg.as<EcSeg>(), aa.keep_all = e->keep_all.as<uint8_t>();
    if (n_work) hipLaunchKernelGGL(ec_block_stats_kernel, dim3((unsigned) (n_work / 256 + 1 < 512? n_work / 256 + 1 : 512)), dim3(256), 0, ctx->stream, e->work.as<EcWork>(),
                                   e->out.as<EcBlockOut>(), n_work, (unsigned long long *) e->stats.p);
    if (kn.assemble_walk) hipLaunchKernelGGL(ec_new_n_kernel, grid256(nr), dim3(256), 0, ctx->stream, nr, e->copy_n.as<uint32_t>(), e->blk_off.as<uint64_t>(), e->work.as<EcWork>(), e->out.as<EcBlockOut>(), e->new_n.as<uint32_t>());
    else hipLaunchKernelGGL(ec_new_n_seg_kernel, grid256(nr), dim3(256), 0, ctx->stream, nr, e->copy_n.as<uint32_t>(), e->blk_off.as<uint64_t>(), e->seg.as<EcSeg>(), e->out.as<EcBlockOut>(), e->new_n.as<uint32_t>());
    uint64_t tot = 0;
    { int rc = prim_scan_total_u32(ctx, e->new_n, e->new_n64, e->new_off, nr, &tot); if (rc) return rc; }
    e->new_tot = tot;
    EENSURE(new_k, (tot + 1) * 8); EENSURE(new_m, (tot + 1) * 4); EENSURE(new_s, (tot + 1) * 8);
    EENSURE(key_id, (tot + 1) * 4); EENSURE(key_sorted, (tot + 1) * 4); EENSURE(val_occ, (tot + 1) * 8); EENSURE(occ, (tot + 1) * 8);
    aa.new_off = e->new_off.as<uint64_t>(), aa.new_k_mer = e->new_k.as<uint64_t>(), aa.new_m_pos = e->new_m.as<uint32_t>(), aa.new_s_mer = e->new_s.as<uint64_t>();
    aa.key_id = e->key_id.as<uint32_t>(), aa.val_occ = e->val_occ.as<uint64_t>(), aa.sid0 = ctx->sid0;
    if (kn.assemble_walk) hipLaunchKernelGGL(ec_assemble_wave_kernel<1>, rblocks, dim3(256), 0, ctx->stream, aa);
    else hipLaunchKernelGGL(ec_assemble_seg_kernel, rblocks, dim3(256), 0, ctx->stream, aa);

    EENSURE(cov, (nv + 1) * 4); EENSURE(fwd, (nv + 1) * 4);
    CK(hipMemsetAsync(e->cov.p, 0, (nv + 1) * 4, ctx->stream));
    CK(hipMemsetAsync(e->fwd.p, 0, (nv + 1) * 4, ctx->stream));
    if (tot) {
        unsigned id_bits = 1;
        while (id_bits < 32 && (nv - 1) >> id_bits) ++id_bits;
        PRIM(rocprim::radix_sort_pairs, e->key_id.as<uint32_t>(), e->key_sorted.as<uint32_t>(), e->val_occ.as<uint64_t>(), e->occ.as<uint64_t>(), tot, 0, id_bits, ctx->stream);
        hipLaunchKernelGGL(ec_fwd_flag_kernel, grid256(tot), dim3(256), 0, ctx->stream, tot, e->occ.as<uint64_t>(), e->key_id.as<uint32_t>());
        PRIM(rocprim::inclusive_scan, e->key_id.as<uint32_t>(), e->key_id.as<uint32_t>(), tot, rocprim::plus<uint32_t>(), ctx->stream);
        hipLaunchKernelGGL(ec_cov_sorted_kernel, grid256(tot), dim3(256), 0, ctx->stream, tot, e->key_sorted.as<uint32_t>(), e->key_id.as<uint32_t>(),
                           e->cov.as<uint32_t>(), e->fwd.as<uint32_t>());
    }
    hipLaunchKernelGGL(ec_del_kernel, grid256(nv), dim3(256), 0, ctx->stream, nv, e->fwd.as<uint32_t>(), e->scm_del.as<uint8_t>());
    uint64_t chk = 0;
    { int rc = prim_scan_total_u32(ctx, e->cov, e->cov64, e->occ_off, nv, &chk); if (rc) return rc; }
    unsigned long long st[16];
    CK(hipMemcpyAsync(st, e->stats.p, sizeof(st), hipMemcpyDeviceToHost, ctx->stream));
    t_end(ctx, OATK_T_EC_REFRESH);
    CK(hipStreamSynchronize(ctx->stream));
    CK(hipGetLastError());
    t_collect(ctx, OATK_T_EC_MARK, OATK_T_EC_REFRESH);
    for (int i = 0; i < 11; ++i) e->stats_h[i] = st[i];
    e->stats_h[11] = n_big;
    if (chk != tot) { ctx->err = "error correction: coverage does not add up"; return OATK_E_STATE; }
    e->done = true, e->seq_kept = keep_seq, e->seq_global = e->global;
    return OATK_OK;
}

extern "C" int oatk_hip_ec_keep_seq(oatk_hip_ctx *ctx, int on)
{
    if (!ctx) return OATK_E_NODEV;
    if (!ctx->ec) ctx->ec = new EcState();
    ctx->ec->keep_seq = on != 0;
    return OATK_OK;
}

extern "C" int oatk_hip_ec_corrected_reads(oatk_hip_ctx *ctx, uint64_t *n_bases)
{
    using namespace oatk;
    if (!ctx) return OATK_E_NODEV;
    EcState *e = ctx->ec;
    if (e && e->seq_kept && e->seq_global != e->global) {
        ctx->err = e->global? "oatk_hip_ec_corrected_reads: the resident correction was made on one handle's ids and the handle is sharded now (correct again: oatk_hip_ec_sharded)"
                            : "oatk_hip_ec_corrected_reads: the resident correction was made on sharded reads (global ids) and the handle is not sharded any more (correct again)";
        return OATK_E_STATE;
    }
    if (!e || !e->done || !e->seq_kept || !ctx->scanned) { ctx->err = "oatk_hip_ec_corrected_reads needs a correction of the resident batch made with oatk_hip_ec_keep_seq"; return OATK_E_STATE; }
    CK(hipSetDevice(ctx->device));
    e->cseq_done = false;
    EC_VIEWS();
    (void) g;
    const uint64_t n_work = e->n_work;
    const bool stages = getenv("OATK_DEBUG_EC_STAGES") != nullptr;
    hipEvent_t ev[3] = {nullptr, nullptr, nullptr};
    if (stages) for (int i = 0; i < 3; ++i) CK(hipEventCreate(&ev[i]));
    EENSURE(sblk, (n_work + nr + 1) * sizeof(EcSeqBlk)); EENSURE(clen, (nr + 1) * 4); EENSURE(cbytes, (nr + 1) * 4);
    if (stages) CK(hipEventRecord(ev[0], ctx->stream));
    if (nr) hipLaunchKernelGGL(ec_cseq_len_kernel, grid256(nr), dim3(256), 0, ctx->stream, rd, e->blk_off.as<uint64_t>(), e->work.as<EcWork>(), e->out.as<EcBlockOut>(), e->qend.as<uint32_t>(),
                               e->sblk.as<EcSeqBlk>(), e->clen.as<uint32_t>(), e->cbytes.as<uint32_t>());
    uint64_t bytes = 0;
    { int rc = prim_scan_total_u32(ctx, e->cbytes, e->cbytes64, e->coff, nr, &bytes); if (rc) return rc; }
    EENSURE(cseq, bytes + 16);
    if (stages) CK(hipEventRecord(ev[1], ctx->stream));
    EcSeqArgs sa;
// ... 58 lines not shown
```

oatk_amd/csrc/ec.hpp:

```cpp
#pragma once
#include "common.hpp"

namespace oatk {

#define EC_FAILURE 0
#define EC_SUCCESS 1
#define EC_AMBISNQ 2
#define EC_AMBISEQ 3
#define EC_MAX_DFS_PATH 10000
#define EC_MIN_ERR_SEQ_LEN 10
#define EC_MIN_ERR_BASE 6
#define EC_NONE 0xFFFFFFFFFFFFFFFFULL

struct EcGraph {
    uint64_t n_vtx, n_arc;
    const uint64_t *idx_p;
    const uint32_t *idx_n;
    const uint64_t *arc_v, *arc_w;
    const uint32_t *arc_ls, *arc_cov;
    uint8_t *arc_del;
    uint8_t *scm_del;
    const uint32_t *scm_cov;
    const uint64_t *scm_s;
    const uint64_t *vtx_hs_off;
// ... 605 lines not shown
                    int32_t c;
                    if (b.r) c = np >= 1? np - 1 : 0;
                    else c = (np >= 2? np - 2 : 0) + (b.end_utg == EC_NONE && np > 1? 1 : 0);
                    if (PASS) {
                        for (int32_t t = lane; t < c; t += 64) {
                            const uint64_t p = b.r? path[np - 1 - t] : path[1 + t];
                            const uint64_t kk = (p & ~1ULL) | 1ULL;
                            write(wpos + (uint32_t) t, kk, b.r? 0xFFFFFFFFu ^ (uint32_t) (p & 1ULL) : 0xFFFFFFFEu | (uint32_t) (p & 1ULL), a.scm_s[kk >> 1]);
                        }
                    }
                    wpos += (uint32_t) c;
                } else if (b.r) {
                    copy(0, b.beg);
                } else if (b.beg + 1 < n) {
                    copy(b.beg + 1, b.end < n? b.end : n);
                }
            },
            copy);
        if (nb < 0) {
            wpos = w0;
            if (PASS && lane < n) write(w0 + (uint32_t) lane, km, mp, my_s);
            wpos += (uint32_t) n;
        }
        if (!PASS && lane == 0) a.new_n[x.r] = (uint32_t) (wpos - w0);
    }
}

__global__ __launch_bounds__(256) void ec_new_n_seg_kernel(uint64_t n_reads, const uint32_t *copy_n, const uint64_t *blk_off, const EcSeg *seg, const EcBlockOut *out, uint32_t *new_n)
{
    const uint64_t r = (uint64_t) blockIdx.x * blockDim.x + threadIdx.x;
    if (r >= n_reads) return;
    const uint64_t b0 = blk_off[r], b1 = blk_off[r + 1];
    if (b0 == b1) { new_n[r] = copy_n[r]; return; }
    uint32_t s = 0, prev_end = 0;
    for (uint64_t i = b0; i < b1; ++i) {
        const EcSeg d = seg[i];
        s += ec_seg_front(d, prev_end) + ec_seg_body(d, out[i].status, out[i].np);
        prev_end = d.end_fl >> 2;
    }
    new_n[r] = s;
}

__device__ __forceinline__ uint32_t ecr_incl_sum(uint32_t v)
{
    v += (uint32_t) __builtin_amdgcn_update_dpp(0, (int32_t) v, 0x111, 0xf, 0xf, false);
    v += (uint32_t) __builtin_amdgcn_update_dpp(0, (int32_t) v, 0x112, 0xf, 0xf, false);
    v += (uint32_t) __builtin_amdgcn_update_dpp(0, (int32_t) v, 0x114, 0xf, 0xf, false);
    v += (uint32_t) __builtin_amdgcn_update_dpp(0, (int32_t) v, 0x118, 0xf, 0xf, false);
    v += (uint32_t) __builtin_amdgcn_update_dpp(0, (int32_t) v, 0x142, 0xa, 0xf, false);
    v += (uint32_t) __builtin_amdgcn_update_dpp(0, (int32_t) v, 0x143, 0xc, 0xf, false);
    return v;
}

__global__ __launch_bounds__(256) void ec_assemble_seg_kernel(EcAssembleArgs a)
{
    const uint64_t r0 = ((uint64_t) blockIdx.x * 4 + (threadIdx.x >> 6)) * ECR_RPW;
    const int lane = threadIdx.x & 63;
    if (r0 >= a.rd.n_reads) return;
#pragma unroll
    for (int k = 0; k < ECR_RPW; ++k) {
        const uint64_t r = r0 + k;
        if (r >= a.rd.n_reads) break;
        const uint64_t o = a.rd.scm_off[r], b0 = a.blk_off[r], w0 = a.new_off[r];
        const int32_t n = ecr_s((int32_t) (a.rd.scm_off[r + 1] - o));
        const uint64_t nb64 = a.blk_off[r + 1] - b0;
        const int32_t nb = ecr_s(nb64 > 64? 65 : (int32_t) nb64);
        const uint32_t room = (uint32_t) ecr_s((int32_t) (uint32_t) (a.new_off[r + 1] - w0));
        const bool keep_all = ecr_s((int32_t) a.keep_all[r]) != 0;
        if (n > 64 || nb > 64 || (nb == 0 && !keep_all)) {
            if (lane == 0) ec_assemble_read_serial(a, r);
            continue;
        }
        const bool in = lane < n;
        const uint64_t km = in? a.rd.k_mer[o + lane] : 0;
        const uint32_t mp = in? a.rd.m_pos[o + lane] : 0;
        const uint64_t my_s = in? a.old_s_mer[o + lane] : 0;
        const uint64_t sid = (a.sid0 + r) << 32;
        auto write = [&](uint32_t idx, uint64_t kk, uint32_t m, uint64_t sv) {
            if (idx >= room) return;
            const uint64_t w = w0 + idx;
            a.new_k_mer[w] = kk, a.new_m_pos[w] = m, a.new_s_mer[w] = sv;
            a.key_id[w] = (uint32_t) (kk >> 1), a.val_occ[w] = sid | (uint64_t) idx << 1 | (m & 1u);
        };
        if (nb == 0) {
            if (in) write((uint32_t) lane, km, mp, my_s);
            continue;
        }
        const bool isb = lane < nb;
        EcSeg d;
        d.beg = 0, d.end_fl = 0;
        uint32_t status = EC_FAILURE, np = 0;
        uint64_t path_off = 0;
        if (isb) d = a.seg[b0 + lane], status = a.out[b0 + lane].status, np = a.out[b0 + lane].np, path_off = a.out[b0 + lane].path_off;
        const uint32_t end = d.end_fl >> 2, prev = wave_prev(end), prev_end = lane == 0? 0u : prev;
        const bool solved = isb && status == EC_SUCCESS;
        const uint32_t front = isb? ec_seg_front(d, prev_end) : 0u, body = isb? ec_seg_body(d, status, np) : 0u, pc = solved? body : 0u;
        const uint32_t at_incl = ecr_incl_sum(front + body), pt_incl = ecr_incl_sum(pc);
        const uint32_t at = at_incl - (front + body), pt = pt_incl - pc;
        const uint32_t n_path = ecr_u32(pt_incl, 63);
        {
            const uint32_t meta = d.beg | (d.end_fl & EC_SEG_R) << 8 | (uint32_t) solved << 9;
            const uint32_t base = at - prev_end;
            uint32_t my_meta = 0, my_base = 0;
            for (int32_t i = 0; i < nb; ++i) {
                const uint32_t pe = ecr_u32(prev_end, i), mi = ecr_u32(meta, i), bi = ecr_u32(base, i);
                if ((uint32_t) lane >= pe) my_meta = mi, my_base = bi;
            }
            const bool stays = !(my_meta >> 9 & 1u) || (!(my_meta >> 8 & 1u) && (uint32_t) lane <= (my_meta & 0xFFu));
            if (in && stays) write(my_base + (uint32_t) lane, km, mp, my_s);
        }
        for (uint32_t t0 = 0; t0 < n_path; t0 += 64) {
            const uint32_t t = t0 + (uint32_t) lane;
            int32_t bi = 0;
            for (int32_t i = 0; i < nb; ++i) if (t >= ecr_u32(pt, i)) bi = i;
            const uint32_t q = t - (uint32_t) __shfl((int32_t) pt, bi), dst = (uint32_t) __shfl((int32_t) (at + front), bi);
            const int32_t bnp = __shfl((int32_t) np, bi);
            const bool br = __shfl((int32_t) (d.end_fl & EC_SEG_R), bi) != 0;
            const uint64_t poff = (uint64_t) (uint32_t) __shfl((int32_t) (uint32_t) (path_off >> 32), bi) << 32 | (uint32_t) __shfl((int32_t) (uint32_t) path_off, bi);
            if (t < n_path) {
                const uint64_t p = br? a.path_pool[poff + (uint32_t) (bnp - 1) - q] : a.path_pool[poff + 1 + q];
                const uint64_t kk = (p & ~1ULL) | 1ULL;
                write(dst + q, kk, br? 0xFFFFFFFFu ^ (uint32_t) (p & 1ULL) : 0xFFFFFFFEu | (uint32_t) (p & 1ULL), a.scm_s[kk >> 1]);
            }
        }
    }
}

__global__ void ec_fwd_flag_kernel(uint64_t tot, const uint64_t *occ, uint32_t *flag)
{
    uint64_t i = (uint64_t) blockIdx.x * blockDim.x + threadIdx.x;
    if (i < tot) flag[i] = !(occ[i] & 1ULL);
}
__global__ void ec_cov_sorted_kernel(uint64_t tot, const uint32_t *key_sorted, const uint32_t *fwd_incl, uint32_t *cov, uint32_t *fwd)
{
    uint64_t i = (uint64_t) blockIdx.x * blockDim.x + threadIdx.x;
    if (i >= tot) return;
    const uint32_t k = key_sorted[i];
    if (i + 1 < tot && key_sorted[i + 1] == k) return;
    uint64_t lo = 0, hi = i;
    while (lo < hi) {
        const uint64_t mid = (lo + hi) >> 1;
        if (key_sorted[mid] < k) lo = mid + 1; else hi = mid;
    }
    cov[k] = (uint32_t) (i - lo + 1);
    fwd[k] = fwd_incl[i] - (lo? fwd_incl[lo - 1] : 0u);
}

__global__ void ec_del_kernel(uint64_t n, const uint32_t *fwd, uint8_t *del)
{
    uint64_t i = (uint64_t) blockIdx.x * blockDim.x + threadIdx.x;
    if (i < n) del[i] = !fwd[i];
}

}
```

oatk_amd/csrc/ec_wave.hpp:

```cpp
#pragma once
#include <type_traits>
#include "ec.hpp"

namespace oatk {

__device__ __forceinline__ uint32_t ecw_rev_in_bytes(uint32_t x)
{
    x = ((x >> 2) & 0x33333333u) | ((x & 0x33333333u) << 2);
    return ((x >> 4) & 0x0F0F0F0Fu) | ((x & 0x0F0F0F0Fu) << 4);
}
__device__ __forceinline__ uint32_t ecw_rev16(uint32_t x)
{
    x = __builtin_bitreverse32(x);
    return ((x >> 1) & 0x55555555u) | ((x & 0x55555555u) << 1);
}
__device__ __forceinline__ uint32_t ecw_src16(const uint8_t *hs, uint32_t p)
{
    const uint32_t *w = (const uint32_t *) hs + (p >> 4);
    const uint64_t v = (uint64_t) ecw_rev_in_bytes(w[1]) << 32 | ecw_rev_in_bytes(w[0]);
    return (uint32_t) (v >> ((p & 15u) << 1));
}
__device__ __forceinline__ uint32_t ecw_gather16(const uint8_t *hs, int64_t start, bool desc)
{
    if (!desc) return start >= 0? ecw_src16(hs, (uint32_t) start) : ecw_src16(hs, 0) << ((uint32_t) (-start) << 1);
// ... 10 lines not shown
    const uint64_t v = (uint64_t) ecw_rev_in_bytes(w1) << 32 | ecw_rev_in_bytes(w0);
    const uint32_t x = (uint32_t) (v >> ((p & 15u) << 1));
    if (!desc) return start >= 0? x : x << ((uint32_t) (-start) << 1);
    const int64_t lo = start - 15;
    return ~(lo >= 0? ecw_rev16(x) : ecw_rev16(x) >> ((uint32_t) (-lo) << 1));
}
__device__ __forceinline__ uint32_t ecw_win16(const uint32_t *W, int32_t p)
{
    const int32_t i = p >> 4;
    return (uint32_t) (((uint64_t) W[i + 1] << 32 | W[i]) >> ((p & 15) << 1));
}
__device__ __forceinline__ void ecw_sync()
{
    __builtin_amdgcn_fence(__ATOMIC_RELEASE, "workgroup");
    __builtin_amdgcn_wave_barrier();
    __builtin_amdgcn_fence(__ATOMIC_ACQUIRE, "workgroup");
}
__device__ __forceinline__ int32_t ecw_uni(int32_t v) { return __builtin_amdgcn_readfirstlane(v); }
__device__ __forceinline__ uint32_t ecw_uniu(uint32_t v) { return (uint32_t) __builtin_amdgcn_readfirstlane((int32_t) v); }
__device__ __forceinline__ uint32_t ecw_lane(uint32_t v, int l) { return (uint32_t) __builtin_amdgcn_readlane((int32_t) v, l); }
__device__ __forceinline__ uint64_t ecw_uni64(uint64_t v) { return (uint64_t) ecw_uniu((uint32_t) (v >> 32)) << 32 | ecw_uniu((uint32_t) v); }

__global__ __launch_bounds__(64) void ecw_export_kmer_kernel(uint64_t n, const uint32_t *ids, const uint64_t *vtx_hs_off, const uint32_t *vtx_mpos,
                                                             const uint8_t *hoco_s, int K, uint32_t stride, uint8_t *out, uint8_t *rev)
{
    const uint64_t i = blockIdx.x;
    if (i >= n) return;
    const uint32_t v = ids[i];
    const uint64_t src = vtx_hs_off[v];
    uint32_t *o = (uint32_t *) (out + i * stride);
    const uint32_t mp = vtx_mpos[v];
    for (uint32_t wi = threadIdx.x; wi < stride / 4; wi += 64)
        o[wi] = src != EC_NO_SRC && (int) (wi << 4) < K? ecw_rev_in_bytes(ecw_src16(hoco_s + src, (mp >> 1) + (wi << 4))) : 0u;
    if (threadIdx.x == 0) rev[i] = src != EC_NO_SRC? (uint8_t) (mp & 1u) : (uint8_t) 0xFF;
}
__global__ void ecw_import_kmer_kernel(uint64_t n, const uint32_t *ids, const uint8_t *rev, uint64_t base_off, uint32_t stride, uint64_t *vtx_hs_off, uint32_t *vtx_mpos)
{
    uint64_t i = (uint64_t) blockIdx.x * blockDim.x + threadIdx.x;
    if (i >= n) return;
    vtx_hs_off[ids[i]] = base_off + i * stride;
    vtx_mpos[ids[i]] = rev[i] & 1u;
}

#define ECW_LIKELY(x) __builtin_expect(!!(x), 1)
#define ECW_RARE(x) __builtin_expect(!!(x), 0)

struct EcwScratch {
    uint32_t *ts, *cs, *os;
    int32_t *ka, *kb;
    uint64_t *c_path, *o_path;
    uint8_t *frames;
    int32_t cap_t, cap_c, cap_w, cap_path, cap_f;
    int32_t arc_budget;
};

struct EcwFrame {
    uint32_t arc_i, arc_end;
    int32_t l0, score, t_end, q_end, n, d0, prev_off, depth;
};

struct EcwWave {
    int32_t *k, *spare;
    int32_t n, d0;
};

__device__ int ecw_step(const uint32_t *ts, int32_t tl, const uint32_t *qs, int32_t ql, int32_t bw, EcwWave &wv, int32_t *buf_a, int32_t *buf_b,
                        int32_t &t_end, int32_t &q_end)
{
    const int lane = threadIdx.x & 63;
    const int32_t n = wv.n, d0 = wv.d0;
    int32_t *k = wv.k;
    t_end = q_end = -1;
    int lg = 0;
    if (n <= 32) lg = n <= 1? 6 : __builtin_clz((uint32_t) (n - 1)) - 26;
    const int G = 1 << lg, c = lane & (G - 1), gbase = lane & ~(G - 1);
    const uint64_t gmask = G == 64? ~0ULL : (1ULL << G) - 1ULL;
    if (n > 64) {
        for (int32_t base = 0; base < n; base += 256) {
            int32_t kk[4], dd[4], lim[4];
            bool a0[4], act[4];
#pragma unroll
            for (int u = 0; u < 4; ++u) {
                const int32_t j = base + 64 * u + lane;
                const bool valid = j < n;
                kk[u] = valid? k[j] : 0, dd[u] = valid? d0 + j : 0;
                a0[u] = valid && !(kk[u] >= tl || kk[u] + dd[u] >= ql);
                act[u] = a0[u];
                lim[u] = (ql - dd[u] < tl? ql - dd[u] : tl) - 1;
            }
            while (__ballot(act[0] | act[1] | act[2] | act[3])) {
#pragma unroll
                for (int u = 0; u < 4; ++u) {
                    const int32_t r = lim[u] - kk[u];
                    const uint32_t x = ecw_win16(ts, kk[u] + 1) ^ ecw_win16(qs, kk[u] + dd[u] + 1);
                    int32_t m = x? __builtin_ctz(x) >> 1 : 16;
                    m = m < r? m : r;
                    m = act[u] && r > 0? m : 0;
                    kk[u] += m;
                    act[u] = act[u] && m == 16;
                }
            }
#pragma unroll
            for (int u = 0; u < 4; ++u) {
                const int32_t j = base + 64 * u + lane;
                const bool reached = a0[u] && (kk[u] + dd[u] == ql - 1 || kk[u] == tl - 1);
                const uint64_t rmask = __ballot(reached);
                if (rmask) {
                    const int fl = __builtin_ctzll(rmask);
                    if (a0[u] && lane < fl) k[j] = kk[u];
                    t_end = (int32_t) ecw_lane((uint32_t) kk[u], fl);
                    q_end = t_end + d0 + base + 64 * u + fl;
                    ecw_sync();
                    return 1;
                }
                if (a0[u]) k[j] = kk[u];
            }
        }
    } else
    for (int32_t base = 0; base < n; base += 64) {
        const int32_t j = base + (lane >> lg);
        const bool valid = j < n;
        int32_t kk = valid? k[j] : 0;
        const int32_t dd = valid? d0 + j : 0;
        const bool act0 = valid && !(kk >= tl || kk + dd >= ql);
        bool act = act0;
        const int32_t lim = (ql - dd < tl? ql - dd : tl) - 1;
        if (__ballot(act)) {
            const int32_t o = c << 4;
            for (;;) {
                const int32_t r = lim - kk - o;
                const int32_t oo = r > 0? o : 0;
                const uint32_t x = ecw_win16(ts, kk + 1 + oo) ^ ecw_win16(qs, kk + dd + 1 + oo);
                int32_t m = x? __builtin_ctz(x) >> 1 : 16;
                m = m < r? m : r;
                m = act && r > 0? m : 0;
                const uint64_t gb = (__ballot(m != 16) >> gbase) & gmask;
                const int first = gb? __builtin_ctzll(gb) : 0;
                const int32_t mm = __shfl(m, gbase + first);
                const int32_t adv = gb? (first << 4) + mm : G << 4;
                kk += act? adv : 0;
                act = act && gb == 0;
                if (!__ballot(act)) break;
            }
        }
        const bool reached = act0 && (kk + dd == ql - 1 || kk == tl - 1);
        const uint64_t rmask = __ballot(reached && c == 0);
        if (rmask) {
            const int fl = __builtin_ctzll(rmask);
            const int32_t jf = base + (fl >> lg);
            if (act0 && c == 0 && j < jf) k[j] = kk;
            t_end = (int32_t) ecw_lane((uint32_t) kk, fl);
            q_end = t_end + d0 + jf;
            ecw_sync();
            return 1;
        }
        if (act0 && c == 0) k[j] = kk;
    }
    ecw_sync();
    int32_t *__restrict__ nk = wv.spare;
#pragma unroll 4
    for (int32_t ib = 0; ib < n + 2; ib += 64) {
        const int32_t i = ib + lane, jj = i - 1;
        const int32_t ja = jj - 1 < 0? 0 : (jj - 1 < n? jj - 1 : n - 1), jb = jj < 0? 0 : (jj < n? jj : n - 1), jc = jj + 1 < n? jj + 1 : n - 1;
        const int32_t ka = k[ja], kb = k[jb], kc = k[jc];
        int32_t v = jj - 1 >= 0? ka : INT32_MIN;
        const int32_t ub = kb + 1, uc = kc + 1;
        v = jj >= 0 && jj < n && ub > v? ub : v;
        v = jj + 1 < n && uc > v? uc : v;
        if (i < n + 2) nk[i] = v;
    }
    int32_t st = 0, en = n + 2;
    const int32_t nd0 = d0 - 1;
    if (ECW_LIKELY(bw < 0 || n < 2 * bw + 1)) {
        if (nd0 < -tl) ++st;
        if (nd0 + n + 1 > ql) --en;
    } else {
        const int32_t lo = -bw > -tl? -bw : -tl, hi = bw > ql? bw : ql;
        while (nd0 + st < lo) ++st;
        while (nd0 + en - 1 > hi) --en;
    }
    wv.n = en - st, wv.d0 = nd0 + st;
    wv.k = nk + st;
    wv.spare = nk == buf_a? buf_b : buf_a;
    ecw_sync();
    return 0;
}

__global__ __launch_bounds__(64) void ecw_wf_ed_kernel(const uint32_t *tw, const uint64_t *tw_off, const int32_t *tl, const uint32_t *qw, const uint64_t *qw_off,
                                                       const int32_t *bw, const int32_t *step_ql, const uint64_t *step_off, int32_t *kbuf, const uint64_t *k_off,
                                                       int32_t *out3)
{
    const uint64_t j = blockIdx.x;
    const uint32_t *ts = tw + tw_off[j], *qs = qw + qw_off[j];
    int32_t *ka = kbuf + k_off[j], *kb = ka + (k_off[j + 1] - k_off[j]) / 2;
    const int32_t tlen = tl[j], band = bw[j];
    EcwWave wv;
    wv.k = ka, wv.spare = kb, wv.n = 1, wv.d0 = 0;
    if (threadIdx.x == 0) ka[0] = -1;
    ecw_sync();
    int32_t score = 0, t_end = -1, q_end = -1;
    for (uint64_t s = step_off[j]; s < step_off[j + 1]; ++s) {
        const int32_t ql = step_ql[s];
        for (;;) {
            if (ecw_step(ts, tlen, qs, ql, band, wv, ka, kb, t_end, q_end)) break;
            ++score;
            if (band >= 0 && score > band) break;
        }
        if (threadIdx.x == 0) out3[3 * s] = score, out3[3 * s + 1] = t_end + 1, out3[3 * s + 2] = q_end + 1;
    }
}

#ifdef OATK_EXPERIMENTS
__global__ __launch_bounds__(64) void myers_ed_kernel(uint64_t n_jobs, const uint32_t *tw, const uint64_t *tw_off, const int32_t *tl, const uint32_t *qw, const uint64_t *qw_off,
                                                      const int32_t *ql_, const int32_t *bw, uint64_t *slab, uint64_t slab_words, int32_t *out3)
{
    const uint64_t j = (uint64_t) blockIdx.x * 64 + threadIdx.x;
    if (j >= n_jobs) return;
    const uint32_t lane = threadIdx.x;
    const uint32_t *ts = tw + tw_off[j], *qs = qw + qw_off[j];
    const int32_t T = tl[j], Q = ql_[j], nw = (T + 63) >> 6;
    uint64_t *S = slab + (uint64_t) blockIdx.x * slab_words;
    auto at = [&](int32_t plane, int32_t w) -> uint64_t & { return S[((uint64_t) plane * (uint64_t) (slab_words / (6 * 64)) + (uint64_t) w) * 64 + lane]; };
    for (int32_t w = 0; w < nw; ++w) {
        uint64_t eq[4] = {0, 0, 0, 0};
        for (int32_t b = 0; b < 64 && 64 * w + b < T; ++b) {
            const int32_t p = 64 * w + b;
            eq[(ts[p >> 4] >> ((p & 15) << 1)) & 3u] |= 1ULL << b;
        }
        for (int c = 0; c < 4; ++c) at(c, w) = eq[c];
        at(4, w) = ~0ULL, at(5, w) = 0ULL;
    }
    const int32_t lastw = nw - 1;
    const uint64_t lastbit = 1ULL << ((T - 1) & 63);
    int32_t score = T, best = T, bi = T, bj = 0;
    for (int32_t col = 0; col < Q; ++col) {
        const uint32_t c = (qs[col >> 4] >> ((col & 15) << 1)) & 3u;
        int hin = 1;
        for (int32_t w = 0; w < nw; ++w) {
            uint64_t Eq = at((int32_t) c, w), Pv = at(4, w), Mv = at(5, w);
            const uint64_t Xv = Eq | Mv;
            if (hin < 0) Eq |= 1ULL;
            const uint64_t Xh = (((Eq & Pv) + Pv) ^ Pv) | Eq;
            uint64_t Ph = Mv | ~(Xh | Pv), Mh = Pv & Xh;
            const uint64_t top = w == lastw? lastbit : 1ULL << 63;
            const int hout = (Ph & top? 1 : 0) - (Mh & top? 1 : 0);
            Ph <<= 1, Mh <<= 1;
            if (hin < 0) Mh |= 1ULL; else if (hin > 0) Ph |= 1ULL;
            at(4, w) = Mh | ~(Xv | Ph);
            at(5, w) = Ph & Xv;
            hin = hout;
        }
        score += hin;
        if (score < best) best = score, bi = T, bj = col + 1;
    }
    int32_t v = score;
    for (int32_t i = T - 1; i >= 0; --i) {
        const uint64_t bit = 1ULL << (i & 63);
        v -= (at(4, i >> 6) & bit? 1 : 0) - (at(5, i >> 6) & bit? 1 : 0);
        if (v < best) best = v, bi = i, bj = Q;
    }
    const int32_t band = bw[j];
    if (band >= 0 && best > band) best = band + 1, bi = 0, bj = 0;
    out3[3 * j] = best, out3[3 * j + 1] = bi, out3[3 * j + 2] = bj;
}
#endif


struct EcwArcRegs {
    uint4 a;
    uint2 b;
};
__device__ __forceinline__ EcwArcRegs ecw_arc_load(const EcLiveArc *arc, uint32_t i)
{
    EcwArcRegs r;
    const uint4 *q = (const uint4 *) (arc + i);
    r.a = q[0];
    r.b = *(const uint2 *) (q + 1);
    return r;
}

struct EcwMemo {
    uint64_t src, ff_end;
    int32_t depth;
    int32_t ff_d;
    uint32_t ff_arc;
    int32_t ff_cl0, ff_clp;
    int32_t mode;
    uint32_t n_reuse, n_ff;
    __device__ __forceinline__ void reset() { src = ff_end = EC_NONE, depth = 0, ff_d = 0, ff_arc = 0, ff_cl0 = ff_clp = 0; }
};

template <bool KEEP = false>
__device__ bool ecw_solve_block(const EcLive &lv, const EcReads &rd, const EcWork &wk, const EcwScratch &s, double max_edist, EcwMemo &mm,
                                uint32_t &status_out, uint32_t &np_out, uint32_t &tried_out, uint32_t &n_path_out, uint32_t &wf_steps_out, uint32_t &wf_diag_out, uint32_t &olen_out)
{
    const int lane = threadIdx.x & 63;
    const int K = rd.K;
    const int32_t tl = wk.l;
    int32_t bw = (int32_t) ceil((double) tl * max_edist);
    if (bw < EC_MIN_ERR_BASE) bw = EC_MIN_ERR_BASE;
    if (ECW_RARE(tl > s.cap_t || 2 * bw + 8 > s.cap_w)) return false;
    bool m_live = false;
    if (mm.mode) {
        if (ECW_LIKELY(wk.ln == 1)) {
            if (wk.beg_utg != mm.src) mm.reset(), mm.src = wk.beg_utg;
            m_live = true;
        } else mm.reset();
    }
    const bool ff = mm.mode > 1 && m_live && mm.ff_d > 0 && wk.end_utg == mm.ff_end && mm.depth >= mm.ff_d && mm.ff_cl0 >= bw + 3 && mm.ff_clp - K <= tl + bw;
    bool ff_walk = mm.mode > 1 && m_live && wk.end_utg != EC_NONE;
    int32_t cl0 = ff? mm.ff_cl0 : 0;
    const uint32_t arc0 = ff? mm.ff_arc : wk.lp;
    EcwArcRegs pre;
    pre.a = make_uint4(0, 0, 0, 0), pre.b = make_uint2(0, 0);
    uint32_t pre_idx = 0xFFFFFFFFu;
    if (wk.ln) pre = ecw_arc_load(lv.arc, arc0), pre_idx = arc0;
    const uint8_t *hs = rd.hoco_s + ((uint64_t) wk.hs16 << 4);
    auto gather_target = [&](auto nwin, auto rev, int32_t wb) __attribute__((always_inline)) {
        constexpr int NW = decltype(nwin)::value;
        constexpr bool R = decltype(rev)::value;
        uint32_t w0[NW], w1[NW], pp[NW];
#pragma unroll
        for (int u = 0; u < NW; ++u) {
            const int32_t wi = wb + lane + 64 * u;
            const int64_t start = R? (int64_t) wk.beg_pos + tl - 1 - (wi << 4) : (int64_t) wk.beg_pos + (wi << 4);
            pp[u] = ecw_gather16_at(start, R);
            w0[u] = w1[u] = 0;
            if ((wi << 4) < tl) { const uint32_t *q = (const uint32_t *) hs + (pp[u] >> 4); w0[u] = q[0], w1[u] = q[1]; }
        }
#pragma unroll
        for (int u = 0; u < NW; ++u) {
            const int32_t wi = wb + lane + 64 * u;
            const int64_t start = R? (int64_t) wk.beg_pos + tl - 1 - (wi << 4) : (int64_t) wk.beg_pos + (wi << 4);
            if ((wi << 4) < tl) s.ts[wi] = ecw_gather16_fin(w0[u], w1[u], pp[u], start, R);
        }
    };
    auto gather_all = [&](auto rev) __attribute__((always_inline)) {
        if (tl <= 1024) gather_target(std::integral_constant<int, 1>(), rev, 0);
        else if (tl <= 2048) gather_target(std::integral_constant<int, 2>(), rev, 0);
        else for (int32_t wb = 0; (wb << 4) < tl; wb += 256) gather_target(std::integral_constant<int, 4>(), rev, wb);
    };
// ... 53 lines not shown
                continue;
            }
            if (lane == 0) f->arc_i = a + 1;
            depth = ecw_uni(f->depth);
            c_len = ecw_uni(f->l0), score = ecw_uni(f->score), t_end = ecw_uni(f->t_end), q_end = ecw_uni(f->q_end);
            wv.n = ecw_uni(f->n), wv.d0 = ecw_uni(f->d0), wv.k = s.ka, wv.spare = s.kb;
            const int32_t *sv = (const int32_t *) (f + 1);
            for (int32_t j = lane; j < wv.n; j += 64) s.ka[j] = sv[j];
        }
        ++tried;
        if (ECW_RARE(s.arc_budget > 0 && (tried > (uint32_t) s.arc_budget || wf_steps > 2u * (uint32_t) s.arc_budget))) return false;
        if (ECW_RARE(pre_idx != a)) pre = ecw_arc_load(lv.arc, a);
        const uint64_t w = ecw_uniu(pre.a.x);
        const int32_t ls = (int32_t) ecw_uniu(pre.a.y), ext = K - ls;
        const uint32_t w_hs16 = ecw_uniu(pre.a.z), w_mpos = ecw_uniu(pre.a.w), w_lp = ecw_uniu(pre.b.x), w_ln = ecw_uniu(pre.b.y);
        const int32_t t_end0 = t_end;
        if (ECW_RARE(depth + 2 > s.cap_path || c_len + ext > s.cap_c)) return false;
        if (lane == 0) s.c_path[depth + 1] = w;
        int32_t cn = depth + 2;
        pre_idx = 0xFFFFFFFFu;
        if (ECW_LIKELY(w_ln)) pre = ecw_arc_load(lv.arc, w_lp), pre_idx = w_lp;
        if (ECW_LIKELY(m_live && depth < mm.depth)) {
            c_len += ext;
            ++mm.n_reuse;
        } else {
            const uint8_t *vs = rd.hoco_s + ((uint64_t) w_hs16 << 4);
            const uint32_t pos = w_mpos >> 1;
            const bool asc = (uint32_t) (w & 1ULL) == (w_mpos & 1u);
            const int32_t w0 = c_len >> 4, w1 = (c_len + ext - 1) >> 4;
            for (int32_t wb = w0; wb <= w1; wb += 64) {
                const int32_t wi = wb + lane;
                if (wi > w1) continue;
                const int32_t t0 = (wi << 4) - c_len;
                uint32_t x = asc? ecw_gather16(vs, (int64_t) pos + ls + t0, false) : ecw_gather16(vs, (int64_t) pos + K - 1 - ls - t0, true);
                if (t0 < 0) {
                    const uint32_t keep = (1u << ((uint32_t) (-t0) << 1)) - 1u;
                    x = (s.cs[wi] & keep) | (x & ~keep);
                }
                s.cs[wi] = x;
            }
            c_len += ext;
            if (m_live && depth == mm.depth) ++mm.depth;
            ecw_sync();
        }
        if (depth == 0) cl0 = c_len;
        if (ff_walk && w == wk.end_utg && depth > 0) mm.ff_end = wk.end_utg, mm.ff_d = depth, mm.ff_arc = a, mm.ff_cl0 = cl0, mm.ff_clp = c_len - ext;
        if (edist == INT32_MAX && wk.end_utg != EC_NONE && wk.end_utg != w && w_ln == 1 && n_path < EC_MAX_DFS_PATH && c_len - K <= tl + bw && c_len >= bw + 3) {
            vpend = true, v_arc = w_lp, v_depth = depth + 1;
            continue;
        }
        ff_walk = false;
        for (;;) {
            ++wf_steps, wf_diag += (uint64_t) wv.n;
            if (ecw_step(s.ts, tl, s.cs, c_len, bw, wv, s.ka, s.kb, t_end, q_end)) break;
            ++score;
            if (ECW_RARE(score > bw)) break;
        }
        t_end += 1, q_end += 1;
        const int32_t ql = c_len;
        const int32_t sc = score + tl - t_end;
        bool new_opt = false;
        if (sc <= bw && (wk.end_utg == EC_NONE || wk.end_utg == w)) {
            status = EC_SUCCESS;
            if (sc <= edist) {
                if (t_end > t_end0) s_edist = edist;
                edist = sc;
                if (wk.end_utg == EC_NONE && q_end < ql) --cn;
                if (ECW_RARE(edist == s_edist)) {
                    bool diff = q_end != o_len;
                    if (!diff) {
                        bool d = false;
                        const int32_t nw = (q_end + 15) >> 4;
                        for (int32_t wi = lane; wi < nw; wi += 64) {
                            uint32_t x = s.cs[wi] ^ s.os[wi];
                            if (wi == nw - 1 && (q_end & 15)) x &= (1u << ((q_end & 15) << 1)) - 1u;
                            d |= x != 0;
                        }
                        diff = __ballot(d) != 0;
                    }
                    if (diff) status = EC_AMBISEQ;
                    if (status == EC_SUCCESS) {
                        bool pd = cn != np;
                        if (!pd) {
                            bool d = false;
                            for (int32_t i = lane; i < cn; i += 64) d |= s.c_path[i] != s.o_path[i];
                            pd = __ballot(d) != 0;
                        }
                        if (pd) status = EC_AMBISNQ;
                    }
                }
                ecw_sync();
                new_opt = true;
                o_len = q_end;
                for (int32_t i = lane; i < cn; i += 64) s.o_path[i] = s.c_path[i];
                np = cn;
            } else if (sc < s_edist) {
                s_edist = sc;
            }
        }
        if (score <= bw && ql - K <= tl + bw && ((wk.end_utg != EC_NONE && wk.end_utg != w) || t_end < tl)) {
            if (n_path < EC_MAX_DFS_PATH) {
                if (ECW_LIKELY(w_ln == 1)) vpend = true, v_arc = w_lp, v_depth = depth + 1;
                else if (w_ln > 1 && !push_frame(w_lp, w_ln, depth + 1)) return false;
            }
        } else {
            ++n_path;
        }
        if (new_opt && (KEEP || nfr > 0 || vpend)) {
            for (int32_t wi = lane; wi < ((o_len + 15) >> 4); wi += 64) s.os[wi] = s.cs[wi];
        }
    }
    ecw_sync();
    if (KEEP) olen_out = (uint32_t) o_len;
    status_out = (uint32_t) status, np_out = (uint32_t) np, tried_out = tried, n_path_out = (uint32_t) n_path, wf_steps_out = wf_steps, wf_diag_out = (uint32_t) (wf_diag >> 6);
    return true;
}

#ifndef ECW_WPB
#define ECW_WPB 2
#endif
#ifndef ECW_BATCH
#define ECW_BATCH 16
#endif
#define ECW_POOL_CHUNK 512

struct EcwArgs {
    EcLive lv;
    EcReads rd;
    const EcWork *work;
    uint64_t n_work;
    const uint32_t *todo;
    uint64_t n_todo;
    double max_edist;
    uint8_t *slabs;
    uint64_t slab_bytes;
    uint32_t *os_slabs;
    uint64_t os_words;
    int32_t cap_t, cap_c, cap_w, cap_path, cap_f;
    EcBlockOut *out;
    uint64_t *path_pool;
    uint64_t pool_cap;
    unsigned long long *pool_cursor;
    unsigned long long *next;
    uint32_t *todo_out;
    unsigned long long *todo_cnt;
    int32_t skip_l;
    int32_t batch;
    int32_t arc_budget;
    int32_t memo;
    unsigned long long *memo_stat;
    uint32_t *seq_qend;
    uint32_t *seq_slots;
    const uint64_t *seq_slot_off;
};

__host__ __device__ inline uint32_t ec_slot_words(int32_t l, double max_edist)
{
    if (l < EC_MIN_ERR_SEQ_LEN) return 0u;
    int32_t bw = (int32_t) ceil((double) l * max_edist);
    if (bw < EC_MIN_ERR_BASE) bw = EC_MIN_ERR_BASE;
    return (uint32_t) ((l + bw + 15) / 16);
}
__device__ __forceinline__ void ec_keep_seq(const EcwArgs &a, uint64_t wi, uint32_t status, uint32_t o_len, const uint32_t *os, int t, int T)
{
    if (status != EC_SUCCESS && status != EC_AMBISNQ) return;
    const uint64_t s0 = a.seq_slot_off[wi];
    uint32_t nw = (o_len + 15u) >> 4;
    const uint32_t room = (uint32_t) (a.seq_slot_off[wi + 1] - s0);
    if (nw > room) nw = room;
    for (uint32_t j = (uint32_t) t; j < nw; j += (uint32_t) T) a.seq_slots[s0 + j] = os[j];
    if (t == 0) a.seq_qend[wi] = o_len;
}

struct EcRoute {
    int32_t cap[4];
    uint32_t *list[4];
    unsigned long long *cnt[4];
};
#define ECW_ROUTE_ITEMS 8
__global__ void ec_route_keys_kernel(const EcWork *work, const uint32_t *list, uint64_t n, uint32_t *keys)
{
    const uint64_t i = (uint64_t) blockIdx.x * blockDim.x + threadIdx.x;
    if (i < n) keys[i] = ~(uint32_t) work[list[i]].l;
}
__global__ void ec_queue_keys_kernel(const EcWork *work, const uint32_t *list, uint64_t n, uint32_t lp_max, uint64_t end_max, int eb, uint32_t *keys)
{
    const uint64_t i = (uint64_t) blockIdx.x * blockDim.x + threadIdx.x;
    if (i >= n) return;
    const EcWork *w = work + (list? list[i] : i);
    const uint32_t lp = w->lp < lp_max? w->lp : lp_max;
    const uint64_t en = w->end_utg < end_max? w->end_utg : end_max;
    keys[i] = (uint32_t) ((uint64_t) lp << eb | (en & ((1ULL << eb) - 1ULL)));
}
__global__ void ec_route_longer_kernel(const EcWork *work, const uint32_t *list, uint64_t n, int32_t cap, unsigned long long *cnt)
{
    const uint64_t i = (uint64_t) blockIdx.x * blockDim.x + threadIdx.x;
    const uint64_t b = __ballot(i < n && work[list[i]].l > cap);
    if ((threadIdx.x & 63) == 0 && b) atomicAdd(cnt, (unsigned long long) __builtin_popcountll(b));
}
__global__ __launch_bounds__(256) void ec_route_kernel(const EcWork *work, uint64_t n_work, EcRoute rt)
{
    __shared__ uint32_t cnt[4], base_lo[4], base_hi[4];
    __shared__ uint32_t stage[4][256 * ECW_ROUTE_ITEMS / 2];
    constexpr uint32_t CAP = 256 * ECW_ROUTE_ITEMS / 2;
    if (threadIdx.x < 4) cnt[threadIdx.x] = 0;
    __syncthreads();
    const uint64_t i0 = (uint64_t) blockIdx.x * (256 * ECW_ROUTE_ITEMS);
#pragma unroll
    for (int k = 0; k < ECW_ROUTE_ITEMS; ++k) {
        const uint64_t i = i0 + (uint64_t) k * 256 + threadIdx.x;
        if (i >= n_work) continue;
        const int32_t l = work[i].l;
        int t = 0;
        while (t < 3 && l > rt.cap[t]) ++t;
        if (t == 0) continue;
        const uint32_t at = atomicAdd(&cnt[t], 1u);
        if (at < CAP) stage[t][at] = (uint32_t) i;
        else rt.list[t][atomicAdd(rt.cnt[t], 1ULL)] = (uint32_t) i;
    }
    __syncthreads();
    if (threadIdx.x >= 1 && threadIdx.x <= 3) {
        const uint32_t n = cnt[threadIdx.x] < CAP? cnt[threadIdx.x] : CAP;
        const unsigned long long b = n? atomicAdd(rt.cnt[threadIdx.x], (unsigned long long) n) : 0ULL;
        base_lo[threadIdx.x] = (uint32_t) b, base_hi[threadIdx.x] = (uint32_t) (b >> 32);
    }
    __syncthreads();
    for (int t = 1; t <= 3; ++t) {
        const uint32_t n = cnt[t] < CAP? cnt[t] : CAP;
        const uint64_t b = (uint64_t) base_hi[t] << 32 | base_lo[t];
        for (uint32_t j = threadIdx.x; j < n; j += 256) rt.list[t][b + j] = stage[t][j];
    }
}

__host__ __device__ inline uint32_t ecw_words(int32_t bases) { return (uint32_t) ((bases + 15) / 16 + 2); }
__host__ __device__ inline uint32_t ecw_lds_words_hybrid(int32_t cap_t, int32_t cap_c, int32_t cap_w)
{
    return (ecw_words(cap_t) + ecw_words(cap_c) + 2u * (uint32_t) (cap_w + 2) + 1u) & ~1u;
}
__host__ __device__ inline uint64_t ecw_slab_bytes_hybrid(int32_t cap_path, int32_t cap_f) { return ((uint64_t) 16 * (uint64_t) cap_path + (uint64_t) cap_f + 63) & ~63ULL; }
__host__ __device__ inline uint32_t ecw_scratch_words(int32_t cap_t, int32_t cap_c, int32_t cap_w, int32_t cap_path, int32_t cap_f, bool os_too = true)
{
    return ((ecw_words(cap_t) + (os_too? 2u : 1u) * ecw_words(cap_c) + 2u * (uint32_t) (cap_w + 2) + 1u) & ~1u) + 4u * (uint32_t) cap_path + (uint32_t) cap_f / 4u;
}

template <int MODE, int WPB = 1, bool KEEP = false>
__global__ __launch_bounds__(64 * WPB) void ec_wave_kernel(EcwArgs a)
{
    constexpr bool BIG = MODE == 1;
    extern __shared__ uint32_t ecw_lds[];
    const int lane = threadIdx.x & 63;
    const uint32_t wave = blockIdx.x * (uint32_t) WPB + ecw_uniu(threadIdx.x >> 6);
    EcwScratch s;
    s.cap_t = a.cap_t, s.cap_c = a.cap_c, s.cap_w = a.cap_w, s.cap_path = a.cap_path, s.cap_f = a.cap_f;
    s.arc_budget = MODE == 0? a.arc_budget : 0;
    uint32_t *const p0 = BIG? (uint32_t *) (a.slabs + (uint64_t) wave * a.slab_bytes)
                            : ecw_lds + (WPB > 1? ecw_uniu(threadIdx.x >> 6) * (MODE == 2? ecw_lds_words_hybrid(a.cap_t, a.cap_c, a.cap_w)
                                                                                                      : ecw_scratch_words(a.cap_t, a.cap_c, a.cap_w, a.cap_path, a.cap_f, false)) : 0u);
    uint32_t *p = p0;
    s.ts = p, p += ecw_words(a.cap_t);
    s.cs = p, p += ecw_words(a.cap_c);
    if (BIG) s.os = p, p += ecw_words(a.cap_c);
    else s.os = a.os_slabs + (uint64_t) wave * a.os_words;
    s.ka = (int32_t *) p, p += a.cap_w + 2;
    s.kb = (int32_t *) p, p += a.cap_w + 2;
    p += (p - p0) & 1;
    if (MODE == 2) p = (uint32_t *) (a.slabs + (uint64_t) wave * a.slab_bytes);
    s.c_path = (uint64_t *) p, p += 2 * a.cap_path;
    s.o_path = (uint64_t *) p, p += 2 * a.cap_path;
    s.frames = (uint8_t *) p;
    const uint64_t total = a.todo? a.n_todo : a.n_work;
    uint64_t pool_at = 0, pool_end = 0;
    EcwMemo mm;
    mm.mode = a.memo, mm.n_reuse = mm.n_ff = 0;
    for (;;) {
        unsigned long long t0 = 0;
        if (lane == 0) t0 = atomicAdd(a.next, (unsigned long long) a.batch);
        t0 = ecw_uni64(t0);
        if (t0 >= total) break;
        mm.reset();
        const int cnt = total - t0 < (uint64_t) a.batch? (int) (total - t0) : a.batch;
        uint64_t my_wi = 0;
        uint4 m0 = make_uint4(0, 0, 0, 0), m1 = m0, m2 = m0;
        if (lane < cnt) {
            my_wi = a.todo? a.todo[t0 + lane] : t0 + lane;
            const uint4 *q = (const uint4 *) (a.work + my_wi);
            m0 = q[0], m1 = q[1], m2 = q[2];
        }
        for (int i = 0; i < cnt; ++i) {
            EcWork wk;
            const uint64_t wi = (uint64_t) ecw_lane((uint32_t) (my_wi >> 32), i) << 32 | ecw_lane((uint32_t) my_wi, i);
            wk.beg_utg = (uint64_t) ecw_lane(m0.y, i) << 32 | ecw_lane(m0.x, i);
            wk.end_utg = (uint64_t) ecw_lane(m0.w, i) << 32 | ecw_lane(m0.z, i);
            wk.read = ecw_lane(m1.x, i), wk.beg_pos = ecw_lane(m1.y, i);
            wk.l = (int32_t) ecw_lane(m1.z, i), wk.r = (int32_t) ecw_lane(m1.w, i);
            wk.hs16 = ecw_lane(m2.x, i), wk.lp = ecw_lane(m2.y, i), wk.ln = ecw_lane(m2.z, i), wk.pad = 0;
            if (ECW_RARE(wk.l > a.skip_l)) continue;
            EcBlockOut o;
            o.status = EC_FAILURE, o.np = 0, o.path_off = 0, o.flags = 0, o.short_block = 0, o.tried = 0, o.n_path = 0, o.wf_steps = 0, o.wf_diag = 0, o.tier = (uint32_t) MODE;
            const uint64_t tick0 = MODE != 0? __builtin_amdgcn_s_memrealtime() : 0;
            if (ECW_RARE(wk.l < EC_MIN_ERR_SEQ_LEN)) {
                o.short_block = 1;
            } else {
                uint32_t st = 0, np = 0, o_len = 0;
                if (ECW_RARE(!ecw_solve_block<KEEP>(a.lv, a.rd, wk, s, a.max_edist, mm, st, np, o.tried, o.n_path, o.wf_steps, o.wf_diag, o_len))) {
                    o.flags = 1;
                    if (lane == 0) a.todo_out[atomicAdd(a.todo_cnt, 1ULL)] = (uint32_t) wi;
                } else {
                    o.status = st, o.np = np;
                    if (KEEP) ec_keep_seq(a, wi, st, o_len, s.os, lane, 64);
                    if (st == EC_SUCCESS && np) {
                        if (ECW_RARE(pool_at + np > pool_end)) {
                            const unsigned long long want = np > ECW_POOL_CHUNK? np : ECW_POOL_CHUNK;
                            unsigned long long off = 0;
                            if (lane == 0) off = atomicAdd(a.pool_cursor, want);
                            pool_at = ecw_uni64(off), pool_end = pool_at + want;
                        }
                        o.path_off = pool_at;
                        if (pool_at + np <= a.pool_cap) for (uint32_t j = lane; j < np; j += 64) a.path_pool[pool_at + j] = s.o_path[j];
                        pool_at += np;
                    }
                }
            }
            o.ticks = MODE != 0? (uint32_t) (__builtin_amdgcn_s_memrealtime() - tick0) : 0u;
            if (lane == 0) a.out[wi] = o;
            ecw_sync();
        }
    }
    if (a.memo_stat && lane == 0 && (mm.n_reuse | mm.n_ff)) {
        atomicAdd(a.memo_stat, (unsigned long long) mm.n_reuse);
        atomicAdd(a.memo_stat + 1, (unsigned long long) mm.n_ff);
    }
}

}
```

oatk_amd/device.py:

```python
import os
import ctypes as C

import numpy as np

from . import _lib

_DTYPES = {
    "HOCO_L": np.uint32, "N_SCM": np.uint32, "N_NN": np.uint32, "N_LRL": np.uint32, "HO_RL": np.uint8, "HOCO_S": np.uint8,
    "NN_KEY": np.uint64, "LRL_KEY": np.uint64, "LRL_VAL": np.uint32, "SCM_OFF": np.uint64, "POS_MPOS": np.uint32,
    "POS_SMER": np.uint64, "POS_HASH": np.uint64, "POS_KID": np.uint64, "SCM_H": np.uint64, "SCM_S": np.uint64,
    "SCM_COV": np.uint32, "SCM_OCC_OFF": np.uint64, "SCM_OCC": np.uint64,
    "EC_N_SCM": np.uint32, "EC_SCM_OFF": np.uint64, "EC_KMER": np.uint64, "EC_MPOS": np.uint32, "EC_SMER": np.uint64,
    "EC_SCM_COV": np.uint32, "EC_SCM_DEL": np.uint8, "EC_SCM_OCC_OFF": np.uint64, "EC_SCM_OCC": np.uint64, "EC_ERR_DEL": np.uint8,
    "EC_SCM_FWD": np.uint32, "EC_VTX_SRC": np.uint64, "EC_BLOCK_WORK": np.uint32, "EC_BLOCK_OUT": np.uint32,
    "EC_CSEQ_LEN": np.uint32, "EC_CSEQ_OFF": np.uint64, "EC_CSEQ": np.uint8, "EC_BLOCK_QEND": np.uint32,
    "INGEST_SEQ": np.uint8, "INGEST_OFF": np.uint64, "INGEST_LEN": np.uint32, "INGEST_HDR": np.uint64,
    "CONS_SEL": np.uint32, "CONS_SLOT": np.uint32, "CONS_RL": np.uint32, "CONS_MSEQ": np.uint32, "CONS_FIRST": np.uint64, "CONS_TOT": np.uint64,
    "EG_IDX_P": np.uint64, "EG_IDX_N": np.uint32, "EG_ARC_V": np.uint64, "EG_ARC_W": np.uint64, "EG_ARC_LS": np.uint32,
    "EG_ARC_COV": np.uint32, "EG_ARC_COMP": np.uint8, "EG_OTHER": np.uint8,
    "RA_ALN_SID": np.uint32, "RA_ALN_OFF": np.uint64, "RA_ALN_S": np.float64, "RA_FRG_UID": np.uint64, "RA_FRG_UBEG": np.uint32,
    "RA_FRG_UEND": np.uint32, "RA_FRG_SBEG": np.uint32, "RA_FRG_SEND": np.uint32, "RA_SKIPPED": np.uint32,
    "OVL_KEY": np.uint64, "OVL_OFF": np.uint64, "OVL_DIST": np.int32, "OVL_CNT": np.uint32, "OVL_TAIL": np.uint8,
    "MG_G_H": np.uint64, "MG_G_S": np.uint64, "MG_G_COV": np.uint32, "MG_G_DEL": np.uint8, "MG_G_OCC_OFF": np.uint64, "MG_G_OCC": np.uint64, "MG_POS_GKID": np.uint64,
    "MG_H": np.uint64, "MG_S": np.uint64, "MG_COV": np.uint32, "MG_L2G": np.uint32, "MG_EC_COV": np.uint32, "MG_EC_DEL": np.uint8, "MG_LCOV": np.uint32,
# ... 138 lines not shown
    def overlap_hist_sharded(self, comm, min_cov=0):
        np_, ne = C.c_uint64(), C.c_uint64()
        self._check(self.L.oatk_hip_overlap_hist_sharded(self.h, comm, int(min_cov), C.byref(np_), C.byref(ne)), "oatk_hip_overlap_hist_sharded")
        return int(np_.value), int(ne.value)

    def stat_sharded(self, comm):
        r = _lib.StatRaw()
        self._check(self.L.oatk_hip_stat_sharded(self.h, comm, C.byref(r)), "oatk_hip_stat_sharded")
        return self._stat_dict(r)

    def ra_utg_coverage_sharded(self, comm, graph, aln=None, chains=None, verbose=0):
        g, keep_g = self._racov_graph(graph)
        a, keep_a = self._racov_aln(aln)
        r = None
        if chains is not None:
            keep_r = [np.ascontiguousarray(chains[0], dtype=np.uint64), np.ascontiguousarray(chains[1], dtype=np.uint64)]
            r = _lib.RacovReads(len(keep_r[0]) - 1, keep_r[0].ctypes.data, keep_r[1].ctypes.data)
        out = np.zeros(max(g.n_utg, 1), np.float64)
        it = C.c_uint64(0)
        self._check(self.L.oatk_hip_ra_utg_coverage_sharded(self.h, comm, C.byref(g), None if r is None else C.byref(r), None if a is None else C.byref(a),
                                                            verbose, out.ctypes.data, C.byref(it)), "oatk_hip_ra_utg_coverage_sharded")
        return out[:g.n_utg], int(it.value)

    def ra_arc_coverage_sharded(self, comm, graph, aln=None):
        g, keep_g = self._racov_graph(graph)
        a, keep_a = self._racov_aln(aln)
        out = np.zeros(max(g.n_arc, 1), np.float64)
        self._check(self.L.oatk_hip_ra_arc_coverage_sharded(self.h, comm, C.byref(g), None if a is None else C.byref(a), out.ctypes.data),
                    "oatk_hip_ra_arc_coverage_sharded")
        return out[:g.n_arc]

    def ec_graph(self, light_c=0):
        if light_c:
            self._check(self.L.oatk_hip_ec_graph_light(self.h, int(light_c)), "oatk_hip_ec_graph_light")
        else:
            self._check(self.L.oatk_hip_ec_graph(self.h), "oatk_hip_ec_graph")

    def ec(self, max_edist, c, a, graph=None, keep_seq=False):
        self.ec_keep_seq(keep_seq)
        if graph is None:
            rc = self.L.oatk_hip_ec(self.h, None, max_edist, c, 10 * c, c, a)
        else:
            keep = {k: np.ascontiguousarray(graph[k], dtype=dt) for k, dt in
                    (("idx_p", np.uint64), ("idx_n", np.uint64), ("arc_v", np.uint64), ("arc_w", np.uint64), ("arc_ls", np.uint64),
                     ("arc_cov", np.uint32), ("arc_del", np.uint8))}
            g = _lib.EcGraph(int(graph["n_vtx"]), int(graph["n_arc"]), *[keep[k].ctypes.data for k in
                             ("idx_p", "idx_n", "arc_v", "arc_w", "arc_ls", "arc_cov", "arc_del")])
            rc = self.L.oatk_hip_ec(self.h, C.byref(g), max_edist, c, 10 * c, c, a)
        self._check(rc, "oatk_hip_ec")
        st = np.zeros(12, np.uint64)
        self._check(self.L.oatk_hip_ec_stats(self.h, st.ctypes.data), "oatk_hip_ec_stats")
        return st

    def wf_ed(self, jobs, wg=0):
        code = np.full(256, 255, np.uint8)
        for i, ch in enumerate(b"ACGT"):
            code[ch] = code[ch + 32] = i
        t_off, q_off, s_off = np.zeros(len(jobs) + 1, np.uint64), np.zeros(len(jobs) + 1, np.uint64), np.zeros(len(jobs) + 1, np.uint64)
        for j, (t, q, _, steps) in enumerate(jobs):
            t_off[j + 1], q_off[j + 1], s_off[j + 1] = t_off[j] + len(t), q_off[j] + len(q), s_off[j] + len(steps)
        tc = code[np.frombuffer(b"".join(j[0] for j in jobs), np.uint8)] if jobs else np.zeros(0, np.uint8)
        qc = code[np.frombuffer(b"".join(j[1] for j in jobs), np.uint8)] if jobs else np.zeros(0, np.uint8)
        if (tc == 255).any() or (qc == 255).any():
            raise ValueError("wf_ed: the device alphabet is the 2-bit one of sr_t.hoco_s (ACGT)")
        bw = np.array([j[2] for j in jobs], np.int32)
        ql = np.array([x for j in jobs for x in j[3]], np.int32)
        out = np.zeros((len(ql), 3), np.int32)
        tc, qc = np.ascontiguousarray(tc), np.ascontiguousarray(qc)
        if wg:
            self._check(self.L.oatk_hip_debug_wf_ed_wg(self.h, wg, len(jobs), tc.ctypes.data, t_off.ctypes.data, qc.ctypes.data, q_off.ctypes.data, bw.ctypes.data,
                                                       ql.ctypes.data, s_off.ctypes.data, out.ctypes.data), "oatk_hip_debug_wf_ed_wg")
        else:
            self._check(self.L.oatk_hip_debug_wf_ed(self.h, len(jobs), tc.ctypes.data, t_off.ctypes.data, qc.ctypes.data, q_off.ctypes.data, bw.ctypes.data,
                                                    ql.ctypes.data, s_off.ctypes.data, out.ctypes.data), "oatk_hip_debug_wf_ed")
        return [[tuple(int(v) for v in out[s]) for s in range(int(s_off[j]), int(s_off[j + 1]))] for j in range(len(jobs))]

    def tables(self, jobs):
        code = np.full(256, 255, np.uint8)
        for i, ch in enumerate(b"ACGT"):
            code[ch] = code[ch + 32] = i
        t_off, s_off, o_off = np.zeros(len(jobs) + 1, np.uint64), np.zeros(len(jobs) + 1, np.uint64), np.zeros(len(jobs) + 1, np.uint64)
        for j, (t, q) in enumerate(jobs):
            t_off[j + 1], s_off[j + 1], o_off[j + 1] = t_off[j] + len(t), s_off[j] + len(q), o_off[j] + 2 * (len(t) + 1)
        tc = np.ascontiguousarray(code[np.frombuffer(b"".join(j[0] for j in jobs), np.uint8)])
        sc = np.ascontiguousarray(code[np.frombuffer(b"".join(j[1] for j in jobs), np.uint8)])
        out = np.zeros(int(o_off[-1]), np.int32)
        self.L.oatk_hip_debug_tables.argtypes = [C.c_void_p] + [C.c_uint64] + [C.c_void_p] * 6
        self._check(self.L.oatk_hip_debug_tables(self.h, len(jobs), tc.ctypes.data, t_off.ctypes.data, sc.ctypes.data, s_off.ctypes.data, out.ctypes.data, o_off.ctypes.data), "oatk_hip_debug_tables")
        res = []
        for j, (t, _) in enumerate(jobs):
            a = int(o_off[j])
            res.append((out[a:a + len(t) + 1].copy(), out[a + len(t) + 1:a + 2 * (len(t) + 1)].copy()))
        return res

    def ed_ab(self, pairs, myers):
        code = np.full(256, 255, np.uint8)
        for i, ch in enumerate(b"ACGT"):
            code[ch] = code[ch + 32] = i
        n = len(pairs)
        t_off, q_off = np.zeros(n + 1, np.uint64), np.zeros(n + 1, np.uint64)
        t_off[1:] = np.cumsum([len(p[0]) for p in pairs])
        q_off[1:] = np.cumsum([len(p[1]) for p in pairs])
        tc = np.ascontiguousarray(code[np.frombuffer(b"".join(p[0] for p in pairs), np.uint8)])
        qc = np.ascontiguousarray(code[np.frombuffer(b"".join(p[1] for p in pairs), np.uint8)])
        if (tc == 255).any() or (qc == 255).any():
            raise ValueError("ed_ab: the device alphabet is ACGT")
        bw = np.array([p[2] for p in pairs], np.int32)
        out = np.zeros((n, 3), np.int32)
        ms = C.c_float()
        self._check(self.L.oatk_hip_debug_ed_ab(self.h, 1 if myers else 0, n, tc.ctypes.data, t_off.ctypes.data, qc.ctypes.data, q_off.ctypes.data, bw.ctypes.data,
                                                out.ctypes.data, C.byref(ms)), "oatk_hip_debug_ed_ab")
        return [tuple(int(v) for v in r) for r in out], float(ms.value)

    def ec_stats(self):
        st = np.zeros(12, np.uint64)
        self._check(self.L.oatk_hip_ec_stats(self.h, st.ctypes.data), "oatk_hip_ec_stats")
        return st

    def ec_keep_seq(self, on):
        self._check(self.L.oatk_hip_ec_keep_seq(self.h, 1 if on else 0), "oatk_hip_ec_keep_seq")

    def corrected_reads(self):
        n = C.c_uint64(0)
        self._check(self.L.oatk_hip_ec_corrected_reads(self.h, C.byref(n)), "oatk_hip_ec_corrected_reads")
# ... 323 lines not shown
```

Measured before the change: 394.6.

## Regroup lone wavefront extensions, raise EC batch, add pair assembly and run-based coverage

The wavefront edit-distance step now detects when only one diagonal in a subgroup is still extending and hands it to the whole 64-lane wave, which strides 1024 bases per turn. This targets long single-diagonal match runs that would otherwise leave most lanes idle. The default work batch rises from 16 to 32, and new defaults route assembly through a pair kernel and coverage refresh through a run-based kernel. Extension-turn counters and debug entry points are added. The larger batch may worsen load balance, and the extra counters add a little per-step overhead.

```diff
diff --git a/include/oatk_hip_ec.h b/include/oatk_hip_ec.h
--- a/include/oatk_hip_ec.h
+++ b/include/oatk_hip_ec.h
@@ -27,6 +27,9 @@
 
 int oatk_hip_debug_wf_ed(oatk_hip_ctx *ctx, uint64_t n_jobs, const uint8_t *t_codes, const uint64_t *t_off, const uint8_t *q_codes, const uint64_t *q_off,
                          const int32_t *bw, const int32_t *step_ql, const uint64_t *step_off, int32_t *out3);
+int oatk_hip_debug_wf_ed_turns(oatk_hip_ctx *ctx, int regroup, uint64_t n_jobs, const uint8_t *t_codes, const uint64_t *t_off, const uint8_t *q_codes, const uint64_t *q_off,
+                               const int32_t *bw, const int32_t *step_ql, const uint64_t *step_off, int32_t *out3, uint32_t *turns);
+int oatk_hip_debug_cov_runs(oatk_hip_ctx *ctx, int runs, uint64_t n, const uint32_t *key_sorted, const uint64_t *occ, uint64_t nv, uint32_t *cov, uint32_t *fwd, uint8_t *del);
 int oatk_hip_debug_wf_ed_wg(oatk_hip_ctx *ctx, int R, uint64_t n_jobs, const uint8_t *t_codes, const uint64_t *t_off, const uint8_t *q_codes, const uint64_t *q_off,
                             const int32_t *bw, const int32_t *step_ql, const uint64_t *step_off, int32_t *out3);
 int oatk_hip_debug_tables(oatk_hip_ctx *ctx, uint64_t n_jobs, const uint8_t *t_codes, const uint64_t *t_off, const uint8_t *s_codes, const uint64_t *s_off, int32_t *out, const uint64_t *out_off);
diff --git a/oatk_amd/_lib.py b/oatk_amd/_lib.py
--- a/oatk_amd/_lib.py
+++ b/oatk_amd/_lib.py
@@ -36,7 +36,7 @@
     "oatk_hip_scan_begin", "oatk_hip_scan_reserve", "oatk_hip_scan_append", "oatk_hip_device", "oatk_hip_d2d", "oatk_hip_mem_pool",
     "oatk_hip_info", "oatk_hip_buffer", "oatk_hip_d2h", "oatk_hip_d2h_async", "oatk_hip_h2d_async", "oatk_hip_staging", "oatk_hip_ingest_text_buffer", "oatk_hip_set_timing", "oatk_hip_get_timing",
     "oatk_hip_debug_hash_mask", "oatk_hip_debug_force_general", "oatk_hip_debug_list_cap",
-    "oatk_hip_ec_graph", "oatk_hip_ec_graph_light", "oatk_hip_ec", "oatk_hip_ec_stats", "oatk_hip_debug_ec_tiers", "oatk_hip_debug_wf_ed", "oatk_hip_debug_wf_ed_wg", "oatk_hip_ec_mark", "oatk_hip_ec_correct",
+    "oatk_hip_ec_graph", "oatk_hip_ec_graph_light", "oatk_hip_ec", "oatk_hip_ec_stats", "oatk_hip_debug_ec_tiers", "oatk_hip_debug_wf_ed", "oatk_hip_debug_wf_ed_turns", "oatk_hip_debug_cov_runs", "oatk_hip_debug_wf_ed_wg", "oatk_hip_ec_mark", "oatk_hip_ec_correct",
     "oatk_hip_ec_set_global", "oatk_hip_ec_pairs", "oatk_hip_ec_graph_from_pairs", "oatk_hip_ec_graph_from_segments", "oatk_hip_ec_export_kmers", "oatk_hip_ec_import_kmers",
     "oatk_hip_ec_reserve_import", "oatk_hip_consensus", "oatk_hip_consensus_ids", "oatk_hip_ingest", "oatk_hip_ingest_host", "oatk_hip_scan_ingested", "oatk_hip_stat", "oatk_hip_stat_keys", "oatk_hip_stat_from_keys",
     "oatk_hip_asm_graph", "oatk_hip_asm_pairs", "oatk_hip_asm_graph_from_pairs", "oatk_hip_overlap_hist", "oatk_hip_overlap_pairs", "oatk_hip_overlap_hist_from_pairs", "oatk_hip_read_alignment", "oatk_hip_debug_align_two_pass",
@@ -203,6 +203,10 @@
     L.oatk_hip_ec_stats.argtypes = [vp, vp]
     L.oatk_hip_debug_ec_tiers.argtypes = [vp, C.c_int, C.c_int]
     L.oatk_hip_debug_wf_ed.argtypes = [vp, C.c_uint64, vp, vp, vp, vp, vp, vp, vp, vp]
+    if hasattr(L, "oatk_hip_debug_wf_ed_turns"):
+        L.oatk_hip_debug_wf_ed_turns.argtypes = [vp, C.c_int, C.c_uint64, vp, vp, vp, vp, vp, vp, vp, vp, vp]
+    if hasattr(L, "oatk_hip_debug_cov_runs"):
+        L.oatk_hip_debug_cov_runs.argtypes = [vp, C.c_int, C.c_uint64, vp, vp, C.c_uint64, vp, vp, vp]
     if hasattr(L, "oatk_hip_debug_wf_ed_wg"):
         L.oatk_hip_debug_wf_ed_wg.argtypes = [vp, C.c_int, C.c_uint64, vp, vp, vp, vp, vp, vp, vp, vp]
     if hasattr(L, "oatk_hip_debug_ed_ab"):
diff --git a/oatk_amd/csrc/api_ec.inc b/oatk_amd/csrc/api_ec.inc
--- a/oatk_amd/csrc/api_ec.inc
+++ b/oatk_amd/csrc/api_ec.inc
@@ -127,7 +127,8 @@
 }
 
 static int debug_ed_impl(oatk_hip_ctx *ctx, uint64_t n_jobs, const uint8_t *t_codes, const uint64_t *t_off, const uint8_t *q_codes, const uint64_t *q_off,
-                         const int32_t *bw, const int32_t *step_ql, const uint64_t *step_off, int32_t *out3, bool myers, float *kernel_ms, int wg_R = 0)
+                         const int32_t *bw, const int32_t *step_ql, const uint64_t *step_off, int32_t *out3, bool myers, float *kernel_ms, int wg_R = 0,
+                         int regroup = 1, uint32_t *turns = nullptr)
 {
     using namespace oatk;
     if (!ctx) return OATK_E_NODEV;
@@ -155,7 +156,7 @@
     };
     const std::vector<uint32_t> tw = pack(t_codes, t_off, tw_off, n_jobs), qw = pack(q_codes, q_off, qw_off, n_jobs);
     const uint64_t n_steps = step_off[n_jobs];
-    DevBuf d_tw, d_qw, d_two, d_qwo, d_tl, d_bw, d_sq, d_so, d_k, d_ko, d_out, d_slab;
+    DevBuf d_tw, d_qw, d_two, d_qwo, d_tl, d_bw, d_sq, d_so, d_k, d_ko, d_out, d_slab, d_turns;
     hipEvent_t ev0 = nullptr, ev1 = nullptr;
     if (kernel_ms) { *kernel_ms = 0.f; (void) hipEventCreate(&ev0); (void) hipEventCreate(&ev1); }
     int32_t max_t = 0;
@@ -174,6 +175,7 @@
     up(d_two, tw_off.data(), (n_jobs + 1) * 8); up(d_qwo, qw_off.data(), (n_jobs + 1) * 8); up(d_ko, k_off.data(), (n_jobs + 1) * 8);
     up(d_tl, tl.data(), n_jobs * 4); up(d_bw, bw, n_jobs * 4); up(d_sq, step_ql, n_steps * 4); up(d_so, step_off, (n_jobs + 1) * 8);
     if (!rc && (!d_k.ensure(k_off[n_jobs] * 4 + 16, ctx->stream) || !d_out.ensure(n_steps * 12 + 16, ctx->stream))) rc = OATK_E_NOMEM;
+    if (!rc && turns && !d_turns.ensure(n_jobs * 4 + 16, ctx->stream)) rc = OATK_E_NOMEM;
     if (!rc && myers) {
         if (!d_slab.ensure(n_waves * slab_words * 8 + 64, ctx->stream) || !d_out.ensure(n_jobs * 12 + 16, ctx->stream)) rc = OATK_E_NOMEM;
         up(d_sq, ql_last.data(), n_jobs * 4);
@@ -202,10 +204,11 @@
         } else
         hipLaunchKernelGGL(ecw_wf_ed_kernel, dim3((unsigned) n_jobs), dim3(64), 0, ctx->stream, d_tw.as<uint32_t>(), d_two.as<uint64_t>(), d_tl.as<int32_t>(),
                            d_qw.as<uint32_t>(), d_qwo.as<uint64_t>(), d_bw.as<int32_t>(), d_sq.as<int32_t>(), d_so.as<uint64_t>(), d_k.as<int32_t>(),
-                           d_ko.as<uint64_t>(), d_out.as<int32_t>());
+                           d_ko.as<uint64_t>(), d_out.as<int32_t>(), (int32_t) regroup, turns? d_turns.as<uint32_t>() : (uint32_t *) nullptr);
         if (ev1) (void) hipEventRecord(ev1, ctx->stream);
         const uint64_t n_out = myers? n_jobs : n_steps;
         if (n_out && (he = hipMemcpyAsync(out3, d_out.p, n_out * 12, hipMemcpyDeviceToHost, ctx->stream)) != hipSuccess) rc = OATK_E_NODEV;
+        if (!rc && turns && (he = hipMemcpyAsync(turns, d_turns.p, n_jobs * 4, hipMemcpyDeviceToHost, ctx->stream)) != hipSuccess) rc = OATK_E_NODEV;
         if ((he = hipStreamSynchronize(ctx->stream)) != hipSuccess) rc = OATK_E_NODEV;
         if (!rc && (he = hipGetLastError()) != hipSuccess) rc = OATK_E_NODEV;
     }
@@ -226,6 +229,42 @@
     const int rc = debug_ed_impl(ctx, n_jobs, t_codes, t_off, q_codes, q_off, bw, step_ql, step_off, out3, false, timed? &ms : nullptr);
     if (timed) fprintf(stderr, "[wf_ed_wg] R 0: %llu jobs, kernel %.3f ms\n", (unsigned long long) n_jobs, ms);
     return rc;
+}
+
+extern "C" int oatk_hip_debug_wf_ed_turns(oatk_hip_ctx *ctx, int regroup, uint64_t n_jobs, const uint8_t *t_codes, const uint64_t *t_off, const uint8_t *q_codes, const uint64_t *q_off,
+                                          const int32_t *bw, const int32_t *step_ql, const uint64_t *step_off, int32_t *out3, uint32_t *turns)
+{
+    if (!turns) { if (ctx) ctx->err = "oatk_hip_debug_wf_ed_turns: turns is null"; return OATK_E_ARG; }
+    return debug_ed_impl(ctx, n_jobs, t_codes, t_off, q_codes, q_off, bw, step_ql, step_off, out3, false, nullptr, 0, regroup != 0, turns);
+}
+
+extern "C" int oatk_hip_debug_cov_runs(oatk_hip_ctx *ctx, int runs, uint64_t n, const uint32_t *key_sorted, const uint64_t *occ, uint64_t nv, uint32_t *cov, uint32_t *fwd, uint8_t *del)
+{
+    using namespace oatk;
+    if (!ctx) return OATK_E_NODEV;
+    if (!nv || n >= 0xFFFFFFFFULL) { ctx->err = "oatk_hip_debug_cov_runs: no keys, or too many entries"; return OATK_E_ARG; }
+    for (uint64_t i = 0; i < n; ++i)
+        if (key_sorted[i] >= nv || (i && key_sorted[i] < key_sorted[i - 1])) { ctx->err = "oatk_hip_debug_cov_runs: keys must ascend and lie below nv"; return OATK_E_ARG; }
+    CK(hipSetDevice(ctx->device));
+    DevBuf d_key, d_occ, d_flag, d_cov, d_fwd, d_del;
+    if (!d_key.ensure(n * 4 + 16, ctx->stream) || !d_occ.ensure(n * 8 + 16, ctx->stream) || !d_flag.ensure(n * 4 + 16, ctx->stream) || !d_cov.ensure(nv * 4 + 16, ctx->stream) ||
+        !d_fwd.ensure(nv * 4 + 16, ctx->stream) || !d_del.ensure(nv + 16, ctx->stream)) { ctx->err = "oatk_hip_debug_cov_runs: hipMalloc failed"; return OATK_E_NOMEM; }
+    if (n) { CK(hipMemcpyAsync(d_key.p, key_sorted, n * 4, hipMemcpyHostToDevice, ctx->stream)); CK(hipMemcpyAsync(d_occ.p, occ, n * 8, hipMemcpyHostToDevice, ctx->stream)); }
+    CK(hipMemsetAsync(d_cov.p, 0, nv * 4, ctx->stream));
+    CK(hipMemsetAsync(d_fwd.p, 0, nv * 4, ctx->stream));
+    if (n && runs) hipLaunchKernelGGL(ec_cov_runs_kernel, grid256(n), dim3(256), 0, ctx->stream, n, d_key.as<uint32_t>(), d_occ.as<uint64_t>(), d_cov.as<uint32_t>(), d_fwd.as<uint32_t>());
+    else if (n) {
+        hipLaunchKernelGGL(ec_fwd_flag_kernel, grid256(n), dim3(256), 0, ctx->stream, n, d_occ.as<uint64_t>(), d_flag.as<uint32_t>());
+        PRIM(rocprim::inclusive_scan, d_flag.as<uint32_t>(), d_flag.as<uint32_t>(), n, rocprim::plus<uint32_t>(), ctx->stream);
+        hipLaunchKernelGGL(ec_cov_sorted_kernel, grid256(n), dim3(256), 0, ctx->stream, n, d_key.as<uint32_t>(), d_flag.as<uint32_t>(), d_cov.as<uint32_t>(), d_fwd.as<uint32_t>());
+    }
+    hipLaunchKernelGGL(ec_del_kernel, grid256(nv), dim3(256), 0, ctx->stream, nv, d_fwd.as<uint32_t>(), d_del.as<uint8_t>());
+    CK(hipMemcpyAsync(cov, d_cov.p, nv * 4, hipMemcpyDeviceToHost, ctx->stream));
+    CK(hipMemcpyAsync(fwd, d_fwd.p, nv * 4, hipMemcpyDeviceToHost, ctx->stream));
+    CK(hipMemcpyAsync(del, d_del.p, nv, hipMemcpyDeviceToHost, ctx->stream));
+    CK(hipStreamSynchronize(ctx->stream));
+    CK(hipGetLastError());
+    return OATK_OK;
 }
 
 extern "C" int oatk_hip_debug_tables(oatk_hip_ctx *ctx, uint64_t n_jobs, const uint8_t *t_codes, const uint64_t *t_off, const uint8_t *s_codes, const uint64_t *s_off, int32_t *out, const uint64_t *out_off)
@@ -645,6 +684,10 @@
     bool list_walk = false;
     bool light_packed = true;
     bool light_pairs = true;
+    bool regroup = true;
+    int32_t batch = ECW_BATCH;
+    bool assemble_pairs = true;
+    bool refresh_runs = true;
     bool light_wide = false;
 };
 static EcKnobs ec_knobs_read()
@@ -664,6 +707,11 @@
     { const char *e = getenv("OATK_DEBUG_EC_QUEUE_SORT"); k.queue_sort = !(e && e[0] == '0' && !e[1]); }
     { const char *e = getenv("OATK_DEBUG_EC_LIGHT_PACKED"); k.light_packed = !(e && e[0] == '0' && !e[1]); }
     { const char *e = getenv("OATK_DEBUG_EC_LIGHT_PAIRS"); k.light_pairs = !(e && e[0] == '0' && !e[1]); }
+    { const char *e = getenv("OATK_DEBUG_EC_REGROUP"); k.regroup = !(e && e[0] == '0' && !e[1]); }
+    k.batch = num("OATK_DEBUG_EC_BATCH", 1, ECW_BATCH);
+    if (k.batch > 64) k.batch = 64;
+    { const char *e = getenv("OATK_DEBUG_EC_ASSEMBLE_PAIRS"); k.assemble_pairs = !(e && e[0] == '0' && !e[1]); }
+    { const char *e = getenv("OATK_DEBUG_EC_REFRESH_RUNS"); k.refresh_runs = !(e && e[0] == '0' && !e[1]); }
     { const char *e = getenv("OATK_DEBUG_EC_LIGHT_KEYBITS"); k.light_wide = e && !strcmp(e, "64"); }
     return k;
 }
@@ -897,20 +945,20 @@
     *sorted = v_out;
     return OATK_OK;
 }
-static int32_t ec_routed_batch(uint64_t n_todo, uint64_t waves)
+static int32_t ec_routed_batch(uint64_t n_todo, uint64_t waves, int32_t cap)
 {
     const uint64_t b = waves? n_todo / (16 * waves) : 1;
-    return (int32_t) (b < 1? 1 : (b > ECW_BATCH? ECW_BATCH : b));
+    return (int32_t) (b < 1? 1 : (b > (uint64_t) cap? (uint64_t) cap : b));
 }
 struct EcMemoLog { int tier; unsigned long long n; int32_t batch; int slot; };
 static int ec_memo_report(oatk_hip_ctx *ctx, EcState *e, const std::vector<EcMemoLog> &log)
 {
     if (log.empty()) return OATK_OK;
-    unsigned long long c[128];
+    unsigned long long c[192];
     CK(hipMemcpyAsync(c, (unsigned long long *) e->cursor.p + 64, sizeof(c), hipMemcpyDeviceToHost, ctx->stream));
     CK(hipStreamSynchronize(ctx->stream));
     for (const EcMemoLog &l : log)
-        fprintf(stderr, "[ec stages] wave solver, tier %d, %llu blocks: batch %d, %llu levels reused, %llu blocks started at their sink\n", l.tier, l.n, (int) l.batch, c[2 * l.slot], c[2 * l.slot + 1]);
+        fprintf(stderr, "[ec stages] wave solver, tier %d, %llu blocks: batch %d, %llu levels reused, %llu blocks started at their sink, %llu extension turns\n", l.tier, l.n, (int) l.batch, c[3 * l.slot], c[3 * l.slot + 1], c[3 * l.slot + 2]);
     return OATK_OK;
 }
 
@@ -1111,13 +1159,13 @@
     if (T0.usable && n_work) {
         EcwArgs a = base;
         ec_set_caps(a, T0);
-        a.todo = nullptr, a.n_todo = 0, a.next = cur + qslot++, a.skip_l = T0.cap_t, a.batch = ECW_BATCH;
+        a.todo = nullptr, a.n_todo = 0, a.next = cur + qslot++, a.skip_l = T0.cap_t, a.batch = kn.batch;
         if (kn.queue_sort && n_work > 1) {
             { int rc = ec_queue_room(ctx, e, n_work); if (rc) return rc; }
             { int rc = ec_queue_sort(ctx, e, nullptr, n_work, ctx->stream, ctx->tmp, &a.todo); if (rc) return rc; }
             a.n_todo = n_work;
         }
-        if (kn.stages) a.memo_stat = cur + 64 + 2 * mlog.size(), mlog.push_back(EcMemoLog{0, (unsigned long long) n_work, a.batch, (int) mlog.size()});
+        if (kn.stages) a.memo_stat = cur + 64 + 3 * mlog.size(), mlog.push_back(EcMemoLog{0, (unsigned long long) n_work, a.batch, (int) mlog.size()});
         a.arc_budget = EC_ARC_BUDGET;
         a.todo_out = list[1], a.todo_cnt = cur + 1;
         a.os_words = ec_os_words(T0.cap_c), a.os_slabs = e->os_slabs.as<uint32_t>();
@@ -1172,7 +1220,7 @@
         ec_set_caps(a, t);
         a.todo = todo, a.n_todo = n_todo, a.next = queue;
         a.skip_l = routed && tier == 0? t.cap_t : 0x7FFFFFFF;
-        a.batch = ECW_BATCH;
+        a.batch = kn.batch;
         const int nx = tier < LAST - 1 && T[LAST - 1].usable? LAST - 1 : next_usable(tier);
         a.todo_out = list[nx], a.todo_cnt = cur + nx;
         uint64_t waves = ec_tier_waves(t, kn.waves, ctx->n_cu);
@@ -1184,7 +1232,7 @@
         if (tier > 0) {
             uint64_t w1 = waves < n_items? waves : n_items;
             if (max_waves && w1 > max_waves) w1 = max_waves;
-            a.batch = ec_routed_batch(n_items, w1);
+            a.batch = ec_routed_batch(n_items, w1, kn.batch);
         }
         if (kn.queue_sort && (todo? routed : true) && n_items > 1 && a.batch > 1) {
             DevBuf *tmp = &ctx->tmp;
@@ -1196,7 +1244,7 @@
         if (waves > groups) waves = groups;
         if (max_waves && waves > max_waves) waves = max_waves;
         if (!waves) return OATK_OK;
-        if (kn.stages && mlog.size() < 64) a.memo_stat = cur + 64 + 2 * mlog.size(), mlog.push_back(EcMemoLog{tier, (unsigned long long) n_items, a.batch, (int) mlog.size()});
+        if (kn.stages && mlog.size() < 64) a.memo_stat = cur + 64 + 3 * mlog.size(), mlog.push_back(EcMemoLog{tier, (unsigned long long) n_items, a.batch, (int) mlog.size()});
         if (t.hybrid) {
             void *p = nullptr;
             int rc = ec_slab_buf(ctx, e, hyb_k, (waves + ECW_WPB) * t.slab + 64, st, "the hybrid tier", "slabs", &p); if (rc) return rc;
@@ -1319,16 +1367,16 @@
 
     const bool heavy = kn.heavy < 0? graph_branches : kn.heavy != 0;
     uint64_t pool_cap = 2 * nocc + (uint64_t) 16384 * ECW_POOL_CHUNK + 4096;
-    EENSURE(cursor, 512 + 128 * 8); EENSURE(stats, 16 * 8);
+    EENSURE(cursor, 512 + 192 * 8); EENSURE(stats, 16 * 8);
     uint64_t n_big = 0;
     uint32_t max_hl = 0;
     for (;;) {
         EENSURE(path_pool, pool_cap * 8);
-        CK(hipMemsetAsync(e->cursor.p, 0, 512 + 128 * 8, ctx->stream));
+        CK(hipMemsetAsync(e->cursor.p, 0, 512 + 192 * 8, ctx->stream));
         EcwArgs base = {};
         base.lv = lv, base.rd = rd, base.work = e->work.as<EcWork>(), base.n_work = n_work, base.max_edist = max_edist;
         base.out = e->out.as<EcBlockOut>(), base.path_pool = e->path_pool.as<uint64_t>(), base.pool_cap = pool_cap;
-        base.memo = kn.memo;
+        base.memo = kn.memo, base.regroup = kn.regroup;
         base.pool_cursor = (unsigned long long *) e->cursor.p;
         if (keep_seq) {
             CK(hipMemsetAsync(e->qend.p, 0, (n_work + 1) * 4, ctx->stream));
@@ -1367,6 +1415,7 @@
     aa.new_off = e->new_off.as<uint64_t>(), aa.new_k_mer = e->new_k.as<uint64_t>(), aa.new_m_pos = e->new_m.as<uint32_t>(), aa.new_s_mer = e->new_s.as<uint64_t>();
     aa.key_id = e->key_id.as<uint32_t>(), aa.val_occ = e->val_occ.as<uint64_t>(), aa.sid0 = ctx->sid0;
     if (kn.assemble_walk) hipLaunchKernelGGL(ec_assemble_wave_kernel<1>, rblocks, dim3(256), 0, ctx->stream, aa);
+    else if (kn.assemble_pairs) hipLaunchKernelGGL(ec_assemble_pair_kernel, dim3((unsigned) ((nr + 7) / 8 > 0? (nr + 7) / 8 : 1)), dim3(256), 0, ctx->stream, aa);
     else hipLaunchKernelGGL(ec_assemble_seg_kernel, rblocks, dim3(256), 0, ctx->stream, aa);
 
     EENSURE(cov, (nv + 1) * 4); EENSURE(fwd, (nv + 1) * 4);
@@ -1376,10 +1425,13 @@
         unsigned id_bits = 1;
         while (id_bits < 32 && (nv - 1) >> id_bits) ++id_bits;
         PRIM(rocprim::radix_sort_pairs, e->key_id.as<uint32_t>(), e->key_sorted.as<uint32_t>(), e->val_occ.as<uint64_t>(), e->occ.as<uint64_t>(), tot, 0, id_bits, ctx->stream);
+        if (kn.refresh_runs) hipLaunchKernelGGL(ec_cov_runs_kernel, grid256(tot), dim3(256), 0, ctx->stream, tot, e->key_sorted.as<uint32_t>(), e->occ.as<uint64_t>(), e->cov.as<uint32_t>(), e->fwd.as<uint32_t>());
+        else {
         hipLaunchKernelGGL(ec_fwd_flag_kernel, grid256(tot), dim3(256), 0, ctx->stream, tot, e->occ.as<uint64_t>(), e->key_id.as<uint32_t>());
         PRIM(rocprim::inclusive_scan, e->key_id.as<uint32_t>(), e->key_id.as<uint32_t>(), tot, rocprim::plus<uint32_t>(), ctx->stream);
         hipLaunchKernelGGL(ec_cov_sorted_kernel, grid256(tot), dim3(256), 0, ctx->stream, tot, e->key_sorted.as<uint32_t>(), e->key_id.as<uint32_t>(),
                            e->cov.as<uint32_t>(), e->fwd.as<uint32_t>());
+        }
     }
     hipLaunchKernelGGL(ec_del_kernel, grid256(nv), dim3(256), 0, ctx->stream, nv, e->fwd.as<uint32_t>(), e->scm_del.as<uint8_t>());
     uint64_t chk = 0;
diff --git a/oatk_amd/csrc/ec.hpp b/oatk_amd/csrc/ec.hpp
--- a/oatk_amd/csrc/ec.hpp
+++ b/oatk_amd/csrc/ec.hpp
@@ -681,6 +681,71 @@
     return v;
 }
 
+__device__ __forceinline__ void ec_assemble_seg_read(const EcAssembleArgs &a, uint64_t r, int lane)
+{
+    const uint64_t o = a.rd.scm_off[r], b0 = a.blk_off[r], w0 = a.new_off[r];
+    const int32_t n = ecr_s((int32_t) (a.rd.scm_off[r + 1] - o));
+    const uint64_t nb64 = a.blk_off[r + 1] - b0;
+    const int32_t nb = ecr_s(nb64 > 64? 65 : (int32_t) nb64);
+    const uint32_t room = (uint32_t) ecr_s((int32_t) (uint32_t) (a.new_off[r + 1] - w0));
+    const bool keep_all = ecr_s((int32_t) a.keep_all[r]) != 0;
+    if (n > 64 || nb > 64 || (nb == 0 && !keep_all)) {
+        if (lane == 0) ec_assemble_read_serial(a, r);
+        return;
+    }
+    const bool in = lane < n;
+    const uint64_t km = in? a.rd.k_mer[o + lane] : 0;
+    const uint32_t mp = in? a.rd.m_pos[o + lane] : 0;
+    const uint64_t my_s = in? a.old_s_mer[o + lane] : 0;
+    const uint64_t sid = (a.sid0 + r) << 32;
+    auto write = [&](uint32_t idx, uint64_t kk, uint32_t m, uint64_t sv) {
+        if (idx >= room) return;
+        const uint64_t w = w0 + idx;
+        a.new_k_mer[w] = kk, a.new_m_pos[w] = m, a.new_s_mer[w] = sv;
+        a.key_id[w] = (uint32_t) (kk >> 1), a.val_occ[w] = sid | (uint64_t) idx << 1 | (m & 1u);
+    };
+    if (nb == 0) {
+        if (in) write((uint32_t) lane, km, mp, my_s);
+        return;
+    }
+    const bool isb = lane < nb;
+    EcSeg d;
+    d.beg = 0, d.end_fl = 0;
+    uint32_t status = EC_FAILURE, np = 0;
+    uint64_t path_off = 0;
+    if (isb) d = a.seg[b0 + lane], status = a.out[b0 + lane].status, np = a.out[b0 + lane].np, path_off = a.out[b0 + lane].path_off;
+    const uint32_t end = d.end_fl >> 2, prev = wave_prev(end), prev_end = lane == 0? 0u : prev;
+    const bool solved = isb && status == EC_SUCCESS;
+    const uint32_t front = isb? ec_seg_front(d, prev_end) : 0u, body = isb? ec_seg_body(d, status, np) : 0u, pc = solved? body : 0u;
+    const uint32_t at_incl = ecr_incl_sum(front + body), pt_incl = ecr_incl_sum(pc);
+    const uint32_t at = at_incl - (front + body), pt = pt_incl - pc;
+    const uint32_t n_path = ecr_u32(pt_incl, 63);
+    {
+        const uint32_t meta = d.beg | (d.end_fl & EC_SEG_R) << 8 | (uint32_t) solved << 9;
+        const uint32_t base = at - prev_end;
+        uint32_t my_meta = 0, my_base = 0;
+        for (int32_t i = 0; i < nb; ++i) {
+            const uint32_t pe = ecr_u32(prev_end, i), mi = ecr_u32(meta, i), bi = ecr_u32(base, i);
+            if ((uint32_t) lane >= pe) my_meta = mi, my_base = bi;
+        }
+        const bool stays = !(my_meta >> 9 & 1u) || (!(my_meta >> 8 & 1u) && (uint32_t) lane <= (my_meta & 0xFFu));
+        if (in && stays) write(my_base + (uint32_t) lane, km, mp, my_s);
+    }
+    for (uint32_t t0 = 0; t0 < n_path; t0 += 64) {
+        const uint32_t t = t0 + (uint32_t) lane;
+        int32_t bi = 0;
+        for (int32_t i = 0; i < nb; ++i) if (t >= ecr_u32(pt, i)) bi = i;
+        const uint32_t q = t - (uint32_t) __shfl((int32_t) pt, bi), dst = (uint32_t) __shfl((int32_t) (at + front), bi);
+        const int32_t bnp = __shfl((int32_t) np, bi);
+        const bool br = __shfl((int32_t) (d.end_fl & EC_SEG_R), bi) != 0;
+        const uint64_t poff = (uint64_t) (uint32_t) __shfl((int32_t) (uint32_t) (path_off >> 32), bi) << 32 | (uint32_t) __shfl((int32_t) (uint32_t) path_off, bi);
+        if (t < n_path) {
+            const uint64_t p = br? a.path_pool[poff + (uint32_t) (bnp - 1) - q] : a.path_pool[poff + 1 + q];
+            const uint64_t kk = (p & ~1ULL) | 1ULL;
+            write(dst + q, kk, br? 0xFFFFFFFFu ^ (uint32_t) (p & 1ULL) : 0xFFFFFFFEu | (uint32_t) (p & 1ULL), a.scm_s[kk >> 1]);
+        }
+    }
+}
 __global__ __launch_bounds__(256) void ec_assemble_seg_kernel(EcAssembleArgs a)
 {
     const uint64_t r0 = ((uint64_t) blockIdx.x * 4 + (threadIdx.x >> 6)) * ECR_RPW;
@@ -690,67 +755,95 @@
     for (int k = 0; k < ECR_RPW; ++k) {
         const uint64_t r = r0 + k;
         if (r >= a.rd.n_reads) break;
-        const uint64_t o = a.rd.scm_off[r], b0 = a.blk_off[r], w0 = a.new_off[r];
-        const int32_t n = ecr_s((int32_t) (a.rd.scm_off[r + 1] - o));
-        const uint64_t nb64 = a.blk_off[r + 1] - b0;
-        const int32_t nb = ecr_s(nb64 > 64? 65 : (int32_t) nb64);
-        const uint32_t room = (uint32_t) ecr_s((int32_t) (uint32_t) (a.new_off[r + 1] - w0));
-        const bool keep_all = ecr_s((int32_t) a.keep_all[r]) != 0;
-        if (n > 64 || nb > 64 || (nb == 0 && !keep_all)) {
-            if (lane == 0) ec_assemble_read_serial(a, r);
-            continue;
-        }
-        const bool in = lane < n;
-        const uint64_t km = in? a.rd.k_mer[o + lane] : 0;
-        const uint32_t mp = in? a.rd.m_pos[o + lane] : 0;
-        const uint64_t my_s = in? a.old_s_mer[o + lane] : 0;
-        const uint64_t sid = (a.sid0 + r) << 32;
-        auto write = [&](uint32_t idx, uint64_t kk, uint32_t m, uint64_t sv) {
-            if (idx >= room) return;
-            const uint64_t w = w0 + idx;
-            a.new_k_mer[w] = kk, a.new_m_pos[w] = m, a.new_s_mer[w] = sv;
-            a.key_id[w] = (uint32_t) (kk >> 1), a.val_occ[w] = sid | (uint64_t) idx << 1 | (m & 1u);
-        };
-        if (nb == 0) {
-            if (in) write((uint32_t) lane, km, mp, my_s);
-            continue;
-        }
-        const bool isb = lane < nb;
-        EcSeg d;
-        d.beg = 0, d.end_fl = 0;
-        uint32_t status = EC_FAILURE, np = 0;
-        uint64_t path_off = 0;
-        if (isb) d = a.seg[b0 + lane], status = a.out[b0 + lane].status, np = a.out[b0 + lane].np, path_off = a.out[b0 + lane].path_off;
-        const uint32_t end = d.end_fl >> 2, prev = wave_prev(end), prev_end = lane == 0? 0u : prev;
-        const bool solved = isb && status == EC_SUCCESS;
-        const uint32_t front = isb? ec_seg_front(d, prev_end) : 0u, body = isb? ec_seg_body(d, status, np) : 0u, pc = solved? body : 0u;
-        const uint32_t at_incl = ecr_incl_sum(front + body), pt_incl = ecr_incl_sum(pc);
-        const uint32_t at = at_incl - (front + body), pt = pt_incl - pc;
-        const uint32_t n_path = ecr_u32(pt_incl, 63);
-        {
-            const uint32_t meta = d.beg | (d.end_fl & EC_SEG_R) << 8 | (uint32_t) solved << 9;
-            const uint32_t base = at - prev_end;
-            uint32_t my_meta = 0, my_base = 0;
-            for (int32_t i = 0; i < nb; ++i) {
-                const uint32_t pe = ecr_u32(prev_end, i), mi = ecr_u32(meta, i), bi = ecr_u32(base, i);
-                if ((uint32_t) lane >= pe) my_meta = mi, my_base = bi;
-            }
-            const bool stays = !(my_meta >> 9 & 1u) || (!(my_meta >> 8 & 1u) && (uint32_t) lane <= (my_meta & 0xFFu));
-            if (in && stays) write(my_base + (uint32_t) lane, km, mp, my_s);
-        }
-        for (uint32_t t0 = 0; t0 < n_path; t0 += 64) {
-            const uint32_t t = t0 + (uint32_t) lane;
-            int32_t bi = 0;
-            for (int32_t i = 0; i < nb; ++i) if (t >= ecr_u32(pt, i)) bi = i;
-            const uint32_t q = t - (uint32_t) __shfl((int32_t) pt, bi), dst = (uint32_t) __shfl((int32_t) (at + front), bi);
-            const int32_t bnp = __shfl((int32_t) np, bi);
-            const bool br = __shfl((int32_t) (d.end_fl & EC_SEG_R), bi) != 0;
-            const uint64_t poff = (uint64_t) (uint32_t) __shfl((int32_t) (uint32_t) (path_off >> 32), bi) << 32 | (uint32_t) __shfl((int32_t) (uint32_t) path_off, bi);
-            if (t < n_path) {
-                const uint64_t p = br? a.path_pool[poff + (uint32_t) (bnp - 1) - q] : a.path_pool[poff + 1 + q];
-                const uint64_t kk = (p & ~1ULL) | 1ULL;
-                write(dst + q, kk, br? 0xFFFFFFFFu ^ (uint32_t) (p & 1ULL) : 0xFFFFFFFEu | (uint32_t) (p & 1ULL), a.scm_s[kk >> 1]);
-            }
+        ec_assemble_seg_read(a, r, lane);
+    }
+}
+
+__device__ __forceinline__ uint32_t ecr_incl_sum32(uint32_t v)
+{
+    v += (uint32_t) __builtin_amdgcn_update_dpp(0, (int32_t) v, 0x111, 0xf, 0xf, false);
+    v += (uint32_t) __builtin_amdgcn_update_dpp(0, (int32_t) v, 0x112, 0xf, 0xf, false);
+    v += (uint32_t) __builtin_amdgcn_update_dpp(0, (int32_t) v, 0x114, 0xf, 0xf, false);
+    v += (uint32_t) __builtin_amdgcn_update_dpp(0, (int32_t) v, 0x118, 0xf, 0xf, false);
+    v += (uint32_t) __builtin_amdgcn_update_dpp(0, (int32_t) v, 0x142, 0xa, 0xf, false);
+    return v;
+}
+
+__global__ __launch_bounds__(256) void ec_assemble_pair_kernel(EcAssembleArgs a)
+{
+    const uint64_t rp = ((uint64_t) blockIdx.x * 4 + (threadIdx.x >> 6)) * 2;
+    const int lane = threadIdx.x & 63, h = lane >> 5, l = lane & 31;
+    if (rp >= a.rd.n_reads) return;
+    bool ok = rp + 1 < a.rd.n_reads;
+    if (ok) {
+#pragma unroll
+        for (int k = 0; k < 2; ++k) {
+            const uint64_t n64 = a.rd.scm_off[rp + k + 1] - a.rd.scm_off[rp + k], nb64 = a.blk_off[rp + k + 1] - a.blk_off[rp + k];
+            ok = ok && n64 <= 32 && nb64 <= 32 && (nb64 > 0 || a.keep_all[rp + k] != 0);
+        }
+    }
+    if (!ecr_s((int32_t) ok)) {
+        ec_assemble_seg_read(a, rp, lane);
+        if (rp + 1 < a.rd.n_reads) ec_assemble_seg_read(a, rp + 1, lane);
+        return;
+    }
+    const uint64_t r = rp + (uint64_t) h;
+    const uint64_t o = a.rd.scm_off[r], b0 = a.blk_off[r], w0 = a.new_off[r];
+    const int32_t n = (int32_t) (a.rd.scm_off[r + 1] - o), nb = (int32_t) (a.blk_off[r + 1] - b0);
+    const uint32_t room = (uint32_t) (a.new_off[r + 1] - w0);
+    const int32_t nb_max = ecr_s(__builtin_amdgcn_readlane(nb, 0) > __builtin_amdgcn_readlane(nb, 32)? __builtin_amdgcn_readlane(nb, 0) : __builtin_amdgcn_readlane(nb, 32));
+    const bool in = l < n;
+    const uint64_t km = in? a.rd.k_mer[o + l] : 0;
+    const uint32_t mp = in? a.rd.m_pos[o + l] : 0;
+    const uint64_t my_s = in? a.old_s_mer[o + l] : 0;
+    const uint64_t sid = (a.sid0 + r) << 32;
+    auto write = [&](uint32_t idx, uint64_t kk, uint32_t m, uint64_t sv) {
+        if (idx >= room) return;
+        const uint64_t w = w0 + idx;
+        a.new_k_mer[w] = kk, a.new_m_pos[w] = m, a.new_s_mer[w] = sv;
+        a.key_id[w] = (uint32_t) (kk >> 1), a.val_occ[w] = sid | (uint64_t) idx << 1 | (m & 1u);
+    };
+    const bool isb = l < nb;
+    EcSeg d;
+    d.beg = 0, d.end_fl = 0;
+    uint32_t status = EC_FAILURE, np = 0;
+    uint64_t path_off = 0;
+    if (isb) d = a.seg[b0 + l], status = a.out[b0 + l].status, np = a.out[b0 + l].np, path_off = a.out[b0 + l].path_off;
+    const uint32_t end = d.end_fl >> 2, prev = wave_prev(end), prev_end = l == 0? 0u : prev;
+    const bool solved = isb && status == EC_SUCCESS;
+    const uint32_t front = isb? ec_seg_front(d, prev_end) : 0u, body = isb? ec_seg_body(d, status, np) : 0u, pc = solved? body : 0u;
+    const uint32_t at_incl = ecr_incl_sum32(front + body), pt_incl = ecr_incl_sum32(pc);
+    const uint32_t at = at_incl - (front + body), pt = pt_incl - pc;
+    const uint32_t np0 = ecr_u32(pt_incl, 31), np1 = ecr_u32(pt_incl, 63);
+    const uint32_t n_path = h? np1 : np0, n_path_max = np0 > np1? np0 : np1;
+    {
+        const uint32_t meta = d.beg | (d.end_fl & EC_SEG_R) << 8 | (uint32_t) solved << 9;
+        const uint32_t base = at - prev_end;
+        uint32_t my_meta = 0, my_base = 0;
+        for (int32_t i = 0; i < nb_max; ++i) {
+            const uint32_t pe = h? ecr_u32(prev_end, 32 + i) : ecr_u32(prev_end, i), mi = h? ecr_u32(meta, 32 + i) : ecr_u32(meta, i),
+                           bi = h? ecr_u32(base, 32 + i) : ecr_u32(base, i);
+            if (i < nb && (uint32_t) l >= pe) my_meta = mi, my_base = bi;
+        }
+        const bool stays = !(my_meta >> 9 & 1u) || (!(my_meta >> 8 & 1u) && (uint32_t) l <= (my_meta & 0xFFu));
+        if (in && stays) write(my_base + (uint32_t) l, km, mp, my_s);
+    }
+    for (uint32_t t0 = 0; t0 < n_path_max; t0 += 32) {
+        const uint32_t t = t0 + (uint32_t) l;
+        int32_t bi = 0;
+        for (int32_t i = 0; i < nb_max; ++i) {
+            const uint32_t pti = h? ecr_u32(pt, 32 + i) : ecr_u32(pt, i);
+            if (i < nb && t >= pti) bi = i;
+        }
+        const int src = (h << 5) + bi;
+        const uint32_t q = t - (uint32_t) __shfl((int32_t) pt, src), dst = (uint32_t) __shfl((int32_t) (at + front), src);
+        const int32_t bnp = __shfl((int32_t) np, src);
+        const bool br = __shfl((int32_t) (d.end_fl & EC_SEG_R), src) != 0;
+        const uint64_t poff = (uint64_t) (uint32_t) __shfl((int32_t) (uint32_t) (path_off >> 32), src) << 32 | (uint32_t) __shfl((int32_t) (uint32_t) path_off, src);
+        if (t < n_path) {
+            const uint64_t p = br? a.path_pool[poff + (uint32_t) (bnp - 1) - q] : a.path_pool[poff + 1 + q];
+            const uint64_t kk = (p & ~1ULL) | 1ULL;
+            write(dst + q, kk, br? 0xFFFFFFFFu ^ (uint32_t) (p & 1ULL) : 0xFFFFFFFEu | (uint32_t) (p & 1ULL), a.scm_s[kk >> 1]);
         }
     }
 }
@@ -775,6 +868,25 @@
     fwd[k] = fwd_incl[i] - (lo? fwd_incl[lo - 1] : 0u);
 }
 
+__global__ __launch_bounds__(256) void ec_cov_runs_kernel(uint64_t tot, const uint32_t *key_sorted, const uint64_t *occ, uint32_t *cov, uint32_t *fwd)
+{
+    const uint64_t i = (uint64_t) blockIdx.x * 256 + threadIdx.x;
+    const int lane = threadIdx.x & 63;
+    const bool valid = i < tot;
+    const uint32_t k = valid? key_sorted[i] : 0u;
+    const bool f = valid && !(occ[valid? i : 0] & 1ULL);
+    const uint32_t prev = (uint32_t) __shfl_up((int) k, 1);
+    const bool head = valid && (lane == 0 || prev != k);
+    const uint64_t heads = __ballot(head), fw = __ballot(f), vm = __ballot(valid);
+    if (!head) return;
+    const uint64_t above = lane == 63? 0ULL : heads & ~((2ULL << lane) - 1ULL);
+    const int end = above? __builtin_ctzll(above) : __builtin_popcountll(vm);
+    const uint64_t m = (end == 64? ~0ULL : (1ULL << end) - 1ULL) & ~((1ULL << lane) - 1ULL);
+    const uint32_t c = (uint32_t) (end - lane), fc = (uint32_t) __builtin_popcountll(fw & m);
+    if (lane > 0 && above) cov[k] = c, fwd[k] = fc;
+    else atomicAdd(cov + k, c), atomicAdd(fwd + k, fc);
+}
+
 __global__ void ec_del_kernel(uint64_t n, const uint32_t *fwd, uint8_t *del)
 {
     uint64_t i = (uint64_t) blockIdx.x * blockDim.x + threadIdx.x;
diff --git a/oatk_amd/csrc/ec_wave.hpp b/oatk_amd/csrc/ec_wave.hpp
--- a/oatk_amd/csrc/ec_wave.hpp
+++ b/oatk_amd/csrc/ec_wave.hpp
@@ -86,6 +86,7 @@
     uint8_t *frames;
     int32_t cap_t, cap_c, cap_w, cap_path, cap_f;
     int32_t arc_budget;
+    int32_t regroup;
 };
 
 struct EcwFrame {
@@ -99,7 +100,7 @@
 };
 
 __device__ int ecw_step(const uint32_t *ts, int32_t tl, const uint32_t *qs, int32_t ql, int32_t bw, EcwWave &wv, int32_t *buf_a, int32_t *buf_b,
-                        int32_t &t_end, int32_t &q_end)
+                        int32_t &t_end, int32_t &q_end, int32_t regroup, uint32_t &turns)
 {
     const int lane = threadIdx.x & 63;
     const int32_t n = wv.n, d0 = wv.d0;
@@ -109,6 +110,7 @@
     if (n <= 32) lg = n <= 1? 6 : __builtin_clz((uint32_t) (n - 1)) - 26;
     const int G = 1 << lg, c = lane & (G - 1), gbase = lane & ~(G - 1);
     const uint64_t gmask = G == 64? ~0ULL : (1ULL << G) - 1ULL;
+    const int lone = regroup && G < 64? G : -1;
     if (n > 64) {
         for (int32_t base = 0; base < n; base += 256) {
             int32_t kk[4], dd[4], lim[4];
@@ -123,6 +125,7 @@
                 lim[u] = (ql - dd[u] < tl? ql - dd[u] : tl) - 1;
             }
             while (__ballot(act[0] | act[1] | act[2] | act[3])) {
+                ++turns;
 #pragma unroll
                 for (int u = 0; u < 4; ++u) {
                     const int32_t r = lim[u] - kk[u];
@@ -174,7 +177,32 @@
                 const int32_t adv = gb? (first << 4) + mm : G << 4;
                 kk += act? adv : 0;
                 act = act && gb == 0;
-                if (!__ballot(act)) break;
+                ++turns;
+                const uint64_t alive = __ballot(act);
+                if (!alive) break;
+                if (ECW_RARE(__builtin_popcountll(alive) == lone)) {
+                    const int ld = __builtin_ctzll(alive);
+                    int32_t k1 = (int32_t) ecw_lane((uint32_t) kk, ld);
+                    const int32_t d1 = (int32_t) ecw_lane((uint32_t) dd, ld), l1 = (int32_t) ecw_lane((uint32_t) lim, ld), o1 = lane << 4;
+                    for (;;) {
+                        const int32_t r1 = l1 - k1 - o1;
+                        const int32_t oo1 = r1 > 0? o1 : 0;
+                        const uint32_t x1 = ecw_win16(ts, k1 + 1 + oo1) ^ ecw_win16(qs, k1 + d1 + 1 + oo1);
+                        int32_t m1 = x1? __builtin_ctz(x1) >> 1 : 16;
+                        m1 = m1 < r1? m1 : r1;
+                        m1 = r1 > 0? m1 : 0;
+                        const uint64_t gb1 = __ballot(m1 != 16);
+                        ++turns;
+                        if (gb1) {
+                            const int f1 = __builtin_ctzll(gb1);
+                            k1 += (f1 << 4) + (int32_t) ecw_lane((uint32_t) m1, f1);
+                            break;
+                        }
+                        k1 += 1024;
+                    }
+                    kk = lane == ld? k1 : kk;
+                    break;
+                }
             }
         }
         const bool reached = act0 && (kk + dd == ql - 1 || kk == tl - 1);
@@ -222,7 +250,7 @@
 
 __global__ __launch_bounds__(64) void ecw_wf_ed_kernel(const uint32_t *tw, const uint64_t *tw_off, const int32_t *tl, const uint32_t *qw, const uint64_t *qw_off,
                                                        const int32_t *bw, const int32_t *step_ql, const uint64_t *step_off, int32_t *kbuf, const uint64_t *k_off,
-                                                       int32_t *out3)
+                                                       int32_t *out3, int32_t regroup, uint32_t *turns_out)
 {
     const uint64_t j = blockIdx.x;
     const uint32_t *ts = tw + tw_off[j], *qs = qw + qw_off[j];
@@ -233,15 +261,17 @@
     if (threadIdx.x == 0) ka[0] = -1;
     ecw_sync();
     int32_t score = 0, t_end = -1, q_end = -1;
+    uint32_t turns = 0;
     for (uint64_t s = step_off[j]; s < step_off[j + 1]; ++s) {
         const int32_t ql = step_ql[s];
         for (;;) {
-            if (ecw_step(ts, tlen, qs, ql, band, wv, ka, kb, t_end, q_end)) break;
+            if (ecw_step(ts, tlen, qs, ql, band, wv, ka, kb, t_end, q_end, regroup, turns)) break;
             ++score;
             if (band >= 0 && score > band) break;
         }
         if (threadIdx.x == 0) out3[3 * s] = score, out3[3 * s + 1] = t_end + 1, out3[3 * s + 2] = q_end + 1;
     }
+    if (turns_out && threadIdx.x == 0) turns_out[j] = turns;
 }
 
 #ifdef OATK_EXPERIMENTS
@@ -321,6 +351,7 @@
     int32_t ff_cl0, ff_clp;
     int32_t mode;
     uint32_t n_reuse, n_ff;
+    uint32_t n_turns;
     __device__ __forceinline__ void reset() { src = ff_end = EC_NONE, depth = 0, ff_d = 0, ff_arc = 0, ff_cl0 = ff_clp = 0; }
 };
 
@@ -480,7 +511,7 @@
         ff_walk = false;
         for (;;) {
             ++wf_steps, wf_diag += (uint64_t) wv.n;
-            if (ecw_step(s.ts, tl, s.cs, c_len, bw, wv, s.ka, s.kb, t_end, q_end)) break;
+            if (ecw_step(s.ts, tl, s.cs, c_len, bw, wv, s.ka, s.kb, t_end, q_end, s.regroup, mm.n_turns)) break;
             ++score;
             if (ECW_RARE(score > bw)) break;
         }
@@ -548,7 +579,7 @@
 #define ECW_WPB 2
 #endif
 #ifndef ECW_BATCH
-#define ECW_BATCH 16
+#define ECW_BATCH 32
 #endif
 #define ECW_POOL_CHUNK 512
 
@@ -576,6 +607,7 @@
     int32_t batch;
     int32_t arc_budget;
     int32_t memo;
+    int32_t regroup;
     unsigned long long *memo_stat;
     uint32_t *seq_qend;
     uint32_t *seq_slots;
@@ -681,6 +713,7 @@
     EcwScratch s;
     s.cap_t = a.cap_t, s.cap_c = a.cap_c, s.cap_w = a.cap_w, s.cap_path = a.cap_path, s.cap_f = a.cap_f;
     s.arc_budget = MODE == 0? a.arc_budget : 0;
+    s.regroup = a.regroup;
     uint32_t *const p0 = BIG? (uint32_t *) (a.slabs + (uint64_t) wave * a.slab_bytes)
                             : ecw_lds + (WPB > 1? ecw_uniu(threadIdx.x >> 6) * (MODE == 2? ecw_lds_words_hybrid(a.cap_t, a.cap_c, a.cap_w)
                                                                                                       : ecw_scratch_words(a.cap_t, a.cap_c, a.cap_w, a.cap_path, a.cap_f, false)) : 0u);
@@ -699,7 +732,7 @@
     const uint64_t total = a.todo? a.n_todo : a.n_work;
     uint64_t pool_at = 0, pool_end = 0;
     EcwMemo mm;
-    mm.mode = a.memo, mm.n_reuse = mm.n_ff = 0;
+    mm.mode = a.memo, mm.n_reuse = mm.n_ff = mm.n_turns = 0;
     for (;;) {
         unsigned long long t0 = 0;
         if (lane == 0) t0 = atomicAdd(a.next, (unsigned long long) a.batch);
@@ -754,10 +787,11 @@
             ecw_sync();
         }
     }
-    if (a.memo_stat && lane == 0 && (mm.n_reuse | mm.n_ff)) {
+    if (a.memo_stat && lane == 0 && (mm.n_reuse | mm.n_ff | mm.n_turns)) {
         atomicAdd(a.memo_stat, (unsigned long long) mm.n_reuse);
         atomicAdd(a.memo_stat + 1, (unsigned long long) mm.n_ff);
-    }
-}
-
-}
+        atomicAdd(a.memo_stat + 2, (unsigned long long) mm.n_turns);
+    }
+}
+
+}
diff --git a/oatk_amd/device.py b/oatk_amd/device.py
--- a/oatk_amd/device.py
+++ b/oatk_amd/device.py
@@ -214,7 +214,17 @@
         self._check(self.L.oatk_hip_ec_stats(self.h, st.ctypes.data), "oatk_hip_ec_stats")
         return st
 
-    def wf_ed(self, jobs, wg=0):
+    def cov_runs(self, key_sorted, occ, nv, runs=True):
+        key, oc = np.ascontiguousarray(key_sorted, np.uint32), np.ascontiguousarray(occ, np.uint64)
+        cov, fwd, dl = np.zeros(nv, np.uint32), np.zeros(nv, np.uint32), np.zeros(nv, np.uint8)
+        self._check(self.L.oatk_hip_debug_cov_runs(self.h, int(bool(runs)), len(key), key.ctypes.data, oc.ctypes.data, nv, cov.ctypes.data, fwd.ctypes.data, dl.ctypes.data), "oatk_hip_debug_cov_runs")
+        return cov, fwd, dl
+
+    def wf_ed_turns(self, jobs, regroup=True):
+        turns = np.zeros(len(jobs), np.uint32)
+        return self.wf_ed(jobs, turns=turns, regroup=regroup), [int(t) for t in turns]
+
+    def wf_ed(self, jobs, wg=0, turns=None, regroup=True):
         code = np.full(256, 255, np.uint8)
         for i, ch in enumerate(b"ACGT"):
             code[ch] = code[ch + 32] = i
@@ -232,6 +242,9 @@
         if wg:
             self._check(self.L.oatk_hip_debug_wf_ed_wg(self.h, wg, len(jobs), tc.ctypes.data, t_off.ctypes.data, qc.ctypes.data, q_off.ctypes.data, bw.ctypes.data,
                                                        ql.ctypes.data, s_off.ctypes.data, out.ctypes.data), "oatk_hip_debug_wf_ed_wg")
+        elif turns is not None:
+            self._check(self.L.oatk_hip_debug_wf_ed_turns(self.h, int(bool(regroup)), len(jobs), tc.ctypes.data, t_off.ctypes.data, qc.ctypes.data, q_off.ctypes.data, bw.ctypes.data,
+                                                          ql.ctypes.data, s_off.ctypes.data, out.ctypes.data, turns.ctypes.data), "oatk_hip_debug_wf_ed_turns")
         else:
             self._check(self.L.oatk_hip_debug_wf_ed(self.h, len(jobs), tc.ctypes.data, t_off.ctypes.data, qc.ctypes.data, q_off.ctypes.data, bw.ctypes.data,
                                                     ql.ctypes.data, s_off.ctypes.data, out.ctypes.data), "oatk_hip_debug_wf_ed")
```

New measurement: 402.3, median of 6. 1.9% higher.
